# finmath/finmath-lib-cuda-extensions

Measured on AMD Instinct MI355X. Metric: Monte-Carlo path-ops/sec (fused RandomVariable stream), higher is better.
Workload: dtype f32

## Files before the change

### finmath-lib-cuda-extensions_amd/__init__.py

```python
from __future__ import annotations

import ctypes as _C

from . import _native
from ._native import FmhipError, Moments, PoolStats, ProgOp, build
from .random_variable import OP, DeviceVector, RandomVariableHip, RandomVariableHipFactory, quantiles, select_ranks_batch
from .brownian_motion import BrownianMotionHip, BrownianMotionFromMersenneRandomNumbers, TimeDiscretization, mersenne_increments
from .increments import (ExponentialLaw, GammaLaw, GammaProcess, IndependentIncrementsFromICDF, JumpProcessIncrements, NormalLaw, PoissonLaw,
                         UniformLaw, VarianceGammaProcess, host_increments, merton_increments)
from .sobol import BrownianMotionFromSobolSequence, SobolSequence, sobol_increments
from .program import Program
from .regression import MonteCarloConditionalExpectationRegression, covariance_matrix, cross_moments, solve_normal_equations
from .regression import MonteCarloConditionalExpectationLocalizedRegression, binned_cross_moments, binned_evaluate, quantile_bounds
from .regression import MonteCarloConditionalExpectationPolynomialRegression, polynomial_cross_moments, polynomial_evaluate
from .sorting import argsort, rank_scores, read_elements, sort_by_key, sorted_quantiles, spearman_matrix
from .prefix import cumulative_sums, expected_shortfall_curve, prefix_search, prefix_sums_at, prefix_sums_host, running_average
from .prefix import weighted_expected_shortfall, weighted_quantiles
from .resample import (bootstrap_resample, device_resample, effective_sample_size, multinomial_resample, resample, resample_host, stratified_resample,
                       systematic_resample)
from .selection import compress, compress_host, count_selected, device_select, expand, expand_host, gather, gather_host
from .tabulated import TabulatedFunction, table_apply, table_apply_host
from .analytic import NORMAL_CDF, NORMAL_DENSITY, NORMAL_QUANTILE, NamedFunction, function_apply, function_apply_host, normal_scores
from .analytic import bachelier_option_value, black_scholes_option_value, option_formula, option_formula_double, option_formula_host
from .analytic import (bachelier_implied_volatility, black_scholes_implied_volatility, convert_volatility, implied_volatility,
# ... 178 lines not shown
    prev = _C.c_int(0)
    _native.check(lib().fmhip_set_jit(int(mode), _C.byref(prev)))
    return prev.value


def jit_wait() -> None:
    _native.check(lib().fmhip_jit_wait())


def traffic_stats() -> tuple:
    b, l = _C.c_int64(0), _C.c_int64(0)
    _native.check(lib().fmhip_traffic_stats(_C.byref(b), _C.byref(l)))
    return b.value, l.value


def engine_stats() -> dict:
    st = _native.EngineStats()
    _native.check(lib().fmhip_engine_stats(_C.byref(st)))
    return {n: getattr(st, n) for n, _ in _native.EngineStats._fields_ if n != "size"}


def jit_stats() -> dict:
    c, f, p, s, d = _C.c_int64(0), _C.c_int64(0), _C.c_int64(0), _C.c_double(0), _C.c_int64(0)
    _native.check(lib().fmhip_jit_stats(_C.byref(c), _C.byref(f), _C.byref(p), _C.byref(s), _C.byref(d)))
    return {"compiled": c.value, "failed": f.value, "pending": p.value, "compile_seconds": s.value, "disk_cache_hits": d.value}


def graph_clone(roots, n_copies: int, leaf_from=(), leaf_to=(), scalars=None):
    import numpy as _np
    n_roots, n_map = len(roots), len(leaf_from)
    r = (_C.c_int64 * n_roots)(*[v.handle for v in roots])
    lf = (_C.c_int64 * max(1, n_map))(*[v.handle for v in leaf_from])
    lt = (_C.c_int64 * max(1, n_map * n_copies))(*[v.handle for row in leaf_to for v in row])
    sc, n_sc = None, 0
    if scalars is not None:
        a = _np.ascontiguousarray(scalars, dtype=_np.float64).reshape(n_copies, -1)
        n_sc = a.shape[1]
        sc = a.ctypes.data_as(_C.POINTER(_C.c_double))
    out = (_C.c_int64 * max(1, n_roots * n_copies))()
    _native.check(lib().fmhip_graph_clone(r, n_roots, n_copies, lf, lt, n_map, sc, n_sc, out))
    return [[DeviceVector(out[j * n_roots + k], roots[k].n) for k in range(n_roots)] for j in range(n_copies)]


def graph_scalars(roots):
    import numpy as _np
    r = (_C.c_int64 * len(roots))(*[v.handle for v in roots])
    n = _C.c_int(0)
    _native.check(lib().fmhip_graph_scalars(r, len(roots), None, 0, _C.byref(n)))
    out = _np.zeros(max(1, n.value), dtype=_np.float64)
    _native.check(lib().fmhip_graph_scalars(r, len(roots), out.ctypes.data_as(_C.POINTER(_C.c_double)), n.value, _C.byref(n)))
    return out[:n.value]


def flush() -> None:
    _native.check(lib().fmhip_flush())


def pool_stats() -> PoolStats:
    s = PoolStats()
    _native.check(lib().fmhip_pool_stats(_C.byref(s)))
    return s


def device_info():
    name = _C.create_string_buffer(256)
    cus, hbm = _C.c_int(0), _C.c_int64(0)
    _native.check(lib().fmhip_device_info(name, 256, _C.byref(cus), _C.byref(hbm)))
    return name.value.decode(), cus.value, hbm.value


def stream_ptr() -> int:
    p = _C.c_void_p(0)
    _native.check(lib().fmhip_get_stream(_C.byref(p)))
    return p.value or 0


def profile_enable(enabled: bool) -> None:
    _native.check(lib().fmhip_profile_enable(1 if enabled else 0))


def profile_read():
    ms, n = _C.c_double(0.0), _C.c_int64(0)
    _native.check(lib().fmhip_profile_read(_C.byref(ms), _C.byref(n)))
    return ms.value, n.value
```

### finmath-lib-cuda-extensions_amd/_native.py

```python
from __future__ import annotations

import ctypes as C
import os
import subprocess

_HERE = os.path.dirname(os.path.abspath(__file__))
LIB_PATH = os.path.join(_HERE, "lib", "libfmhip.so")
CSRC = os.path.join(_HERE, "csrc")

SYMBOLS = [
    "fmhip_init", "fmhip_init_devices", "fmhip_device_count", "fmhip_set_thread_engines", "fmhip_shutdown", "fmhip_is_initialized", "fmhip_abi_version", "fmhip_last_error",
    "fmhip_device_info", "fmhip_synchronize", "fmhip_get_stream",
    "fmhip_vec_create_from_double", "fmhip_vec_create_from_float", "fmhip_vec_create_filled",
    "fmhip_vec_create_uninitialized", "fmhip_vec_retain", "fmhip_vec_release", "fmhip_vec_size", "fmhip_vec_give_up_values",
    "fmhip_vec_read_double", "fmhip_vec_read_float", "fmhip_vec_device_ptr",
    "fmhip_call_v1s0", "fmhip_call_v1s1", "fmhip_call_v2s0", "fmhip_call_v2s1", "fmhip_call_v3s0",
    "fmhip_set_fusion", "fmhip_flush", "fmhip_fusion_hold", "fmhip_set_step_grouping", "fmhip_graph_clone", "fmhip_graph_scalars", "fmhip_set_math_mode",
    "fmhip_reduce_moments", "fmhip_reduce_moments_batch", "fmhip_reduce_moments_batch_device", "fmhip_reduce_moments_device",
    "fmhip_reduce_moments_batch_begin", "fmhip_reduce_moments_batch_end", "fmhip_reduce_moments_batch_devices", "fmhip_get_stream_of", "fmhip_expectation_collective",
    "fmhip_set_expectation_comm", "fmhip_expectation_world", "fmhip_expectation_combine",
    "fmhip_select_ranks_batch", "fmhip_rank_sums_batch", "fmhip_count_not_above", "fmhip_cross_moments", "fmhip_cross_moments_wide",
    "fmhip_binned_cross_moments", "fmhip_binned_cross_moments_host", "fmhip_binned_evaluate", "fmhip_binned_evaluate_host",
    "fmhip_polynomial_cross_moments", "fmhip_polynomial_evaluate", "fmhip_polynomial_cross_moments_host", "fmhip_polynomial_evaluate_host",
    "fmhip_sort_by_key", "fmhip_argsort", "fmhip_argsort_host", "fmhip_rank_scores", "fmhip_vec_read_elements",
    "fmhip_prefix_sums", "fmhip_prefix_sums_at", "fmhip_prefix_search", "fmhip_prefix_sums_host",
    "fmhip_resample", "fmhip_resample_host",
    "fmhip_compress", "fmhip_expand", "fmhip_gather", "fmhip_compress_host", "fmhip_expand_host", "fmhip_gather_host",
    "fmhip_table_build", "fmhip_table_apply", "fmhip_table_apply_host",
    "fmhip_function_apply", "fmhip_function_apply_host", "fmhip_option_formula", "fmhip_option_formula_host",
    "fmhip_implied_volatility", "fmhip_implied_volatility_host",
    "fmhip_block_moments", "fmhip_block_moments_host", "fmhip_vec_repeat",
    "fmhip_block_order_statistics", "fmhip_block_order_statistics_host", "fmhip_block_sort", "fmhip_block_sort_host",
    "fmhip_cross_order_statistics", "fmhip_cross_order_statistics_host", "fmhip_cross_select", "fmhip_cross_select_host",
    "fmhip_kernel_moments", "fmhip_kernel_moments_host",
    "fmhip_program_create", "fmhip_program_release", "fmhip_program_launch_count", "fmhip_program_shape",
    "fmhip_program_run", "fmhip_program_run_into",
    "fmhip_set_jit", "fmhip_jit_wait", "fmhip_jit_stats", "fmhip_program_tier", "fmhip_program_source",
    "fmhip_bm_generate", "fmhip_mersenne_increments", "fmhip_bm_generate_mersenne", "fmhip_bm_generate_mersenne_device", "fmhip_inverse_normal_cdf",
    "fmhip_increments_host", "fmhip_increments_generate_device",
    "fmhip_sobol_points_host", "fmhip_sobol_increments_host", "fmhip_bm_generate_sobol_device",
    "fmhip_pool_clean", "fmhip_pool_purge", "fmhip_pool_stats",
    "fmhip_profile_enable", "fmhip_profile_read", "fmhip_traffic_stats", "fmhip_engine_stats",
]

OK = 0
ERR_INVALID_HANDLE, ERR_SIZE_MISMATCH, ERR_OUT_OF_MEMORY, ERR_HIP = -1, -2, -3, -4
ERR_INVALID_ARGUMENT, ERR_NOT_INITIALIZED, ERR_UNSUPPORTED, ERR_PROGRAM_LIMIT = -5, -6, -7, -8


GATHER_FN = C.CFUNCTYPE(C.c_int, C.c_void_p, C.POINTER(C.c_double), C.c_int, C.POINTER(C.c_double))


class Moments(C.Structure):
    _fields_ = [("sum", C.c_double), ("sumsq", C.c_double), ("min", C.c_double), ("max", C.c_double)]


class ProgOp(C.Structure):
    _fields_ = [("opcode", C.c_int32), ("a", C.c_int32), ("b", C.c_int32), ("c", C.c_int32), ("scalar", C.c_double)]


class PoolStats(C.Structure):
    _fields_ = [(n, C.c_int64) for n in (
        "bytes_reserved", "bytes_in_use", "bytes_cached", "device_bytes_free", "device_bytes_total",
        "n_alloc_hits", "n_alloc_misses", "n_live_vectors", "n_kernel_launches", "n_ops_executed")]


class EngineStats(C.Structure):
    _fields_ = [(n, C.c_int64) for n in (
        "size", "kernel_launches", "specialised_launches", "interpreter_launches", "algorithmic_bytes", "algorithmic_bytes_written",
        "values_deferred", "values_deferred_now", "values_demanded", "pending_operations", "peak_bytes_reserved",
        "late_releases_while_waiting", "late_releases_at_once", "late_release_nanoseconds", "merged_launches", "merged_chains", "common_rows", "rolled_launches")]


class FmhipError(RuntimeError):
    def __init__(self, code: int, message: str):
        super().__init__(f"fmhip error {code}: {message}")
        self.code = code


def _source_hash() -> str:
    import hashlib
    h = hashlib.sha256()
    files = [os.path.join(CSRC, f) for f in sorted(os.listdir(CSRC))]
    files += [os.path.join(_HERE, "host", f) for f in sorted(os.listdir(os.path.join(_HERE, "host")))]
    files.append(os.path.join(os.path.dirname(_HERE), "include", "fmhip.h"))
    for f in files:
        if os.path.isfile(f):
            h.update(os.path.basename(f).encode())
            with open(f, "rb") as fh:
                h.update(fh.read())
    return h.hexdigest()


_HASH_PATH = LIB_PATH + ".srchash"


def build(force: bool = False) -> str:
    if force:
        subprocess.check_call(["make", "-C", CSRC, "clean"])
    subprocess.check_call(["make", "-C", CSRC, "-j4"], stdout=subprocess.DEVNULL)
    with open(_HASH_PATH, "w") as fh:
        fh.write(_source_hash())
    return LIB_PATH


def _stale() -> bool:
    if not os.path.exists(LIB_PATH):
        return True
    try:
        with open(_HASH_PATH) as fh:
            return fh.read().strip() != _source_hash()
    except OSError:
        return True


_lib = None


def lib():
    global _lib
    if _lib is not None:
        return _lib
    if _stale():
        import fcntl
        os.makedirs(os.path.dirname(LIB_PATH), exist_ok=True)
        with open(LIB_PATH + ".lock", "w") as lock:
            fcntl.flock(lock, fcntl.LOCK_EX)
            try:
                if _stale():
                    try:
                        build()
                    except Exception as e:
                        if not os.path.exists(LIB_PATH):
                            raise
                        import warnings
                        warnings.warn(f"libfmhip.so is older than its sources and rebuilding it failed ({e}); loading the existing library", RuntimeWarning)
            finally:
                fcntl.flock(lock, fcntl.LOCK_UN)
    if not os.path.exists(LIB_PATH):
        raise ImportError(f"{LIB_PATH} is missing — the HIP extension is required (no CPU fallback exists)")
    L = C.CDLL(LIB_PATH)
    vec, i64, i32, dbl, vp = C.c_int64, C.c_int64, C.c_int, C.c_double, C.c_void_p
    pv = C.POINTER(C.c_int64)
    sig = {
        "fmhip_init": [i32], "fmhip_init_devices": [C.POINTER(C.c_int), i32], "fmhip_device_count": [C.POINTER(C.c_int)], "fmhip_set_thread_engines": [i32, C.POINTER(C.c_int)], "fmhip_shutdown": [], "fmhip_is_initialized": [], "fmhip_abi_version": [],
        "fmhip_device_info": [C.c_char_p, i32, C.POINTER(i32), C.POINTER(i64)],
        "fmhip_synchronize": [], "fmhip_get_stream": [C.POINTER(vp)],
        "fmhip_vec_create_from_double": [C.POINTER(dbl), i64, pv],
        "fmhip_vec_create_from_float": [C.POINTER(C.c_float), i64, pv],
        "fmhip_vec_create_filled": [i64, dbl, pv], "fmhip_vec_create_uninitialized": [i64, pv],
        "fmhip_vec_retain": [vec], "fmhip_vec_release": [vec], "fmhip_vec_size": [vec, C.POINTER(i64)],
        "fmhip_vec_read_double": [vec, C.POINTER(dbl), i64], "fmhip_vec_read_float": [vec, C.POINTER(C.c_float), i64],
        "fmhip_vec_device_ptr": [vec, C.POINTER(vp)],
        "fmhip_call_v1s0": [i32, vec, pv], "fmhip_call_v1s1": [i32, vec, dbl, pv],
        "fmhip_call_v2s0": [i32, vec, vec, pv], "fmhip_call_v2s1": [i32, vec, vec, dbl, pv],
        "fmhip_call_v3s0": [i32, vec, vec, vec, pv],
        "fmhip_set_fusion": [i32, C.POINTER(i32)], "fmhip_flush": [], "fmhip_fusion_hold": [i32, C.POINTER(i32)], "fmhip_set_step_grouping": [i32, C.POINTER(i32)], "fmhip_set_math_mode": [i32, C.POINTER(i32)],
        "fmhip_graph_clone": [pv, i32, i32, pv, pv, i32, C.POINTER(dbl), i32, pv], "fmhip_graph_scalars": [pv, i32, C.POINTER(dbl), i32, C.POINTER(i32)],
        "fmhip_reduce_moments": [vec, dbl, C.POINTER(Moments)], "fmhip_reduce_moments_batch": [pv, i32, C.POINTER(dbl), C.POINTER(Moments)], "fmhip_reduce_moments_batch_device": [pv, i32, C.POINTER(dbl), vp], "fmhip_reduce_moments_device": [vec, dbl, vp],
        "fmhip_reduce_moments_batch_devices": [pv, i32, C.POINTER(dbl), C.POINTER(vp), i32], "fmhip_get_stream_of": [i32, C.POINTER(vp)], "fmhip_expectation_collective": [C.POINTER(i32), C.c_char_p, i32],
        "fmhip_reduce_moments_batch_begin": [pv, i32, C.POINTER(dbl), pv], "fmhip_vec_give_up_values": [pv, i32], "fmhip_reduce_moments_batch_end": [i64, C.POINTER(Moments), i32],
        "fmhip_select_ranks_batch": [pv, i32, C.POINTER(i64), i32, C.POINTER(dbl)], "fmhip_rank_sums_batch": [pv, i32, i64, i64, C.POINTER(dbl)], "fmhip_count_not_above": [vec, C.POINTER(dbl), i32, C.POINTER(i64)],
        "fmhip_cross_moments": [pv, i32, pv, i32, C.POINTER(dbl)],
        "fmhip_cross_moments_wide": [pv, i32, pv, i32, C.POINTER(dbl)],
        "fmhip_binned_cross_moments": [vec, C.POINTER(dbl), i32, pv, i32, pv, i32, C.POINTER(i64), C.POINTER(dbl)],
        "fmhip_binned_cross_moments_host": [vp, i64, C.POINTER(dbl), i32, C.POINTER(vp), i32, C.POINTER(vp), i32, C.POINTER(i64), C.POINTER(dbl)],
        "fmhip_binned_evaluate": [vec, C.POINTER(dbl), i32, pv, i32, C.POINTER(dbl), pv],
        "fmhip_binned_evaluate_host": [vp, i64, C.POINTER(dbl), i32, C.POINTER(vp), i32, C.POINTER(dbl), vp],
        "fmhip_polynomial_cross_moments": [pv, i32, C.POINTER(C.c_uint8), i32, pv, i32, pv, i32, C.POINTER(dbl)],
        "fmhip_polynomial_evaluate": [pv, i32, C.POINTER(C.c_uint8), i32, pv, i32, C.POINTER(dbl), pv],
        "fmhip_polynomial_cross_moments_host": [C.POINTER(vp), i64, i32, C.POINTER(C.c_uint8), i32, C.POINTER(vp), i32, C.POINTER(vp), i32, C.POINTER(dbl)],
        "fmhip_polynomial_evaluate_host": [C.POINTER(vp), i64, i32, C.POINTER(C.c_uint8), i32, C.POINTER(vp), i32, C.POINTER(dbl), vp],
        "fmhip_sort_by_key": [vec, pv, i32, pv, pv], "fmhip_argsort": [vec, C.POINTER(i64)], "fmhip_argsort_host": [vp, i64, C.POINTER(i64)],
        "fmhip_rank_scores": [vec, pv], "fmhip_vec_read_elements": [vec, C.POINTER(i64), i32, C.POINTER(dbl)],
        "fmhip_prefix_sums": [vec, i32, pv, C.POINTER(dbl)], "fmhip_prefix_sums_at": [vec, C.POINTER(i64), i32, C.POINTER(dbl)],
        "fmhip_prefix_search": [vec, C.POINTER(dbl), i32, i32, C.POINTER(i64), C.POINTER(dbl), C.POINTER(dbl)],
        "fmhip_prefix_sums_host": [vp, i64, C.POINTER(dbl)],
        "fmhip_resample": [vec, i32, i64, dbl, vec, pv, i32, pv, pv, C.POINTER(dbl)],
        "fmhip_resample_host": [vp, i64, i32, i64, dbl, vp, C.POINTER(vp), i32, C.POINTER(vp), C.POINTER(i64), C.POINTER(dbl)],
        "fmhip_compress": [vec, pv, i32, pv, pv, C.POINTER(i64)], "fmhip_expand": [vec, pv, i32, dbl, pv], "fmhip_gather": [vec, pv, i32, pv],
        "fmhip_compress_host": [vp, i64, C.POINTER(vp), i32, C.POINTER(vp), C.POINTER(i64), C.POINTER(i64)],
        "fmhip_expand_host": [vp, i64, C.POINTER(vp), i32, i64, dbl, C.POINTER(vp)],
        "fmhip_gather_host": [vp, i64, C.POINTER(vp), i32, i64, C.POINTER(vp)],
        "fmhip_table_build": [C.POINTER(dbl), C.POINTER(dbl), i32, i32, i32, i32, C.POINTER(dbl)],
        "fmhip_table_apply": [vec, C.POINTER(dbl), i32, C.POINTER(dbl), i32, pv],
        "fmhip_table_apply_host": [vp, i64, C.POINTER(dbl), i32, C.POINTER(dbl), i32, C.POINTER(vp)],
        "fmhip_function_apply": [vec, C.POINTER(i32), i32, pv], "fmhip_function_apply_host": [vp, i64, C.POINTER(i32), i32, C.POINTER(vp)],
        "fmhip_option_formula": [i32, vec, dbl, vec, dbl, vec, dbl, dbl, dbl, i32, pv],
        "fmhip_option_formula_host": [i32, vp, dbl, vp, dbl, vp, dbl, i64, dbl, dbl, i32, C.POINTER(vp)],
        "fmhip_implied_volatility": [i32, vec, dbl, vec, dbl, vec, dbl, dbl, dbl, i32, pv],
        "fmhip_implied_volatility_host": [i32, vp, dbl, vp, dbl, vp, dbl, i64, dbl, dbl, i32, C.POINTER(vp)],
        "fmhip_block_moments": [pv, i32, i64, C.c_uint32, pv], "fmhip_block_moments_host": [vp, i64, i64, C.c_uint32, vp],
        "fmhip_vec_repeat": [vec, i64, i64, pv],
        "fmhip_block_order_statistics": [pv, i32, i64, C.POINTER(i64), i32, C.POINTER(i64), C.POINTER(i64), i32, pv],
        "fmhip_block_order_statistics_host": [vp, i64, i64, C.POINTER(i64), i32, C.POINTER(i64), C.POINTER(i64), i32, vp],
        "fmhip_block_sort": [vec, i64, pv], "fmhip_block_sort_host": [vp, i64, i64, vp],
        "fmhip_cross_order_statistics": [pv, i32, C.POINTER(C.c_int32), i32, i32, pv],
        "fmhip_cross_order_statistics_host": [C.POINTER(vp), i32, i64, C.POINTER(C.c_int32), i32, i32, C.POINTER(vp)],
        "fmhip_cross_select": [vec, pv, i32, pv], "fmhip_cross_select_host": [vp, C.POINTER(vp), i32, i64, vp],
        "fmhip_kernel_moments": [vec, C.POINTER(dbl), C.POINTER(dbl), i32, i32, i32, pv, i32, C.POINTER(dbl)],
        "fmhip_kernel_moments_host": [vp, i64, C.POINTER(dbl), C.POINTER(dbl), i32, i32, i32, C.POINTER(vp), i32, C.POINTER(dbl)],
        "fmhip_program_create": [C.POINTER(ProgOp), i32, i32, C.POINTER(C.c_int32), i32, C.POINTER(C.c_int32), i32, pv],
        "fmhip_program_release": [i64], "fmhip_program_launch_count": [i64, C.POINTER(i32)],
        "fmhip_program_shape": [i64, C.POINTER(i32), C.POINTER(i32), C.POINTER(i32)],
        "fmhip_set_expectation_comm": [i32, i32, GATHER_FN, vp], "fmhip_expectation_world": [C.POINTER(i32), C.POINTER(i32)],
        "fmhip_expectation_combine": [C.POINTER(Moments), i32, i32, C.POINTER(Moments)],
        "fmhip_program_run": [i64, i32, pv, pv, C.POINTER(dbl), C.POINTER(Moments), vp],
        "fmhip_program_run_into": [i64, i32, pv, pv, C.POINTER(dbl), C.POINTER(Moments), vp],
        "fmhip_bm_generate": [i64, i32, i32, i64, i64, C.POINTER(dbl), pv],
        "fmhip_mersenne_increments": [C.c_int32, i32, i32, i64, C.POINTER(dbl), C.POINTER(dbl)],
        "fmhip_bm_generate_mersenne": [C.c_int32, i32, i32, i64, C.POINTER(dbl), pv],
# ... 31 lines not shown
```

### finmath-lib-cuda-extensions_amd/csrc/abi.cpp

```cpp
#include "runtime.hpp"
#include "sharded.hpp"
#include "order_stats.hpp"
#include <cmath>

#include <chrono>
#include <cstdlib>
#include <algorithm>
#include <cstring>
#include <functional>
#include <string>
#include <thread>
#include <vector>

namespace fm { void mersenne_increments(int32_t, int, int, int64_t, const double*, double*); double inverse_normal_cdf(double); }

using fm::Engine;
using fm::Error;

static thread_local std::string g_last_error;
namespace fm { void set_last_error(const std::string& message) { g_last_error = message; } }
namespace front = fm::front;
#define FRONT(call) do { if (fm::front_active()) return front::call; } while (0)

namespace te {
// ... 404 lines not shown
    return guarded([&] {
        Engine& e = Engine::get();
        e.require_init();
        if (previous) *previous = e.fusion ? 1 : 0;
        if (e.fusion && !enabled) e.flush_all();
        e.fusion = enabled != 0;
    });
}
int fmhip_fusion_hold(int hold, int* previous) {
    FRONT(set_int(1, hold, previous));
    return guarded([&] {
        Engine& e = Engine::get();
        e.require_init();
        if (previous) *previous = e.fusion_hold;
        e.fusion_hold = hold == 2 ? 2 : (hold != 0 ? 1 : 0);
    });
}
int fmhip_set_step_grouping(int steps, int* previous) {
    FRONT(set_int(2, steps, previous));
    TE_ALL(mine, fmhip_set_step_grouping(steps, mine ? previous : nullptr));
    return guarded([&] {
        Engine& e = Engine::get();
        e.require_init();
        if (steps < 0) throw Error(FMHIP_ERR_INVALID_ARGUMENT, "negative number of time steps");
        if (previous) *previous = e.group_steps;
        e.group_steps = steps;
    });
}
int fmhip_graph_clone(const fmhip_vec* roots, int n_roots, int n_copies, const fmhip_vec* leaf_from, const fmhip_vec* leaf_to, int n_map,
                      const double* scalars, int n_scalars, fmhip_vec* out) {
    FRONT(graph_clone(roots, n_roots, n_copies, leaf_from, leaf_to, n_map, scalars, n_scalars, out));
    if (te::active()) {
        const int te_rc = te::status_of([&]() -> int {
            te::ensure();
            bool any = false;
            for (int i = 0; leaf_from && i < n_map; ++i) any |= te::foreign(leaf_from[i]);
            for (int i = 0; leaf_to && i < n_map * n_copies; ++i) any |= te::foreign(leaf_to[i]);
            if (!any) return te::NOT_MINE_TO_HANDLE;
            te::Localized from(leaf_from, n_map), to(leaf_to, n_map * n_copies);
            te::Inside nested;
            return fmhip_graph_clone(roots, n_roots, n_copies, from.local.data(), to.local.data(), n_map, scalars, n_scalars, out);
        });
        if (te_rc != te::NOT_MINE_TO_HANDLE) return te_rc;
    }
    return guarded([&] { Engine::get().graph_clone(roots, n_roots, n_copies, leaf_from, leaf_to, n_map, scalars, n_scalars, out); });
}
int fmhip_graph_scalars(const fmhip_vec* roots, int n_roots, double* scalars_out, int capacity, int* n_scalars) {
    FRONT(graph_scalars(roots, n_roots, scalars_out, capacity, n_scalars));
    return guarded([&] {
        if (!n_scalars) throw Error(FMHIP_ERR_INVALID_ARGUMENT, "null count pointer");
        *n_scalars = Engine::get().graph_scalars(roots, n_roots, scalars_out, capacity);
    });
}
int fmhip_set_math_mode(int mode, int* previous) {
    FRONT(set_int(3, mode, previous));
    TE_ALL(mine, fmhip_set_math_mode(mode, mine ? previous : nullptr));
    return guarded([&] {
        Engine& e = Engine::get();
        e.require_init();
        if (mode != FMHIP_MATH_EXACT && mode != FMHIP_MATH_FAST) throw Error(FMHIP_ERR_INVALID_ARGUMENT, "unknown math mode");
        if (previous) *previous = e.math_mode;
        if (e.math_mode != mode) e.flush_all();
        e.math_mode = mode;
    });
}
int fmhip_flush(void) { FRONT(flush()); return guarded([&] { Engine::get().flush_all(); Engine::get().end_step_group(); }); }

static void combine_moments(const fmhip_moments* gathered, int world, int count, fmhip_moments* out) {
    for (int k = 0; k < count; ++k) {
        fmhip_moments m = gathered[k];
        for (int r = 1; r < world; ++r) {
            const fmhip_moments& g = gathered[(size_t)r * count + k];
            m.sum += g.sum; m.sumsq += g.sumsq;
            m.min = (m.min != m.min || g.min != g.min) ? std::nan("") : (g.min < m.min || (g.min == m.min && std::signbit(g.min))) ? g.min : m.min;
            m.max = (m.max != m.max || g.max != g.max) ? std::nan("") : (g.max > m.max || (g.max == m.max && !std::signbit(g.max))) ? g.max : m.max;
        }
        out[k] = m;
    }
}
static void exchange_moments(Engine& e, fmhip_moments* inout, int count) {
    if (e.comm_world <= 1 || !e.comm_gather) return;
    std::vector<fmhip_moments> all((size_t)e.comm_world * count);
    const int st = e.comm_gather(e.comm_context, reinterpret_cast<const double*>(inout), count * 4, reinterpret_cast<double*>(all.data()));
    if (st != 0) throw Error(FMHIP_ERR_HIP, "the expectation communicator's gather failed with status " + std::to_string(st));
    combine_moments(all.data(), e.comm_world, count, inout);
}
int fmhip_set_expectation_comm(int world, int rank, fmhip_gather_fn gather, void* context) {
    if (fm::front_active()) {
        if (world > 1) return front::unsupported("fmhip_set_expectation_comm");
        if (world < 1 || rank != 0) { g_last_error = "bad communicator: world " + std::to_string(world) + ", rank " + std::to_string(rank); return FMHIP_ERR_INVALID_ARGUMENT; }
        return FMHIP_OK;
    }
    return guarded([&] {
        Engine& e = Engine::get();
        if (world < 1 || rank < 0 || rank >= world) throw Error(FMHIP_ERR_INVALID_ARGUMENT, "bad communicator: world " + std::to_string(world) + ", rank " + std::to_string(rank));
        if (world > 1 && !gather) throw Error(FMHIP_ERR_INVALID_ARGUMENT, "a communicator of more than one rank needs a gather function");
        e.comm_world = gather ? world : 1; e.comm_rank = gather ? rank : 0; e.comm_gather = gather; e.comm_context = context;
    });
}
int fmhip_expectation_world(int* world, int* rank) {
    if (fm::front_active()) { if (world) *world = 1; if (rank) *rank = 0; return FMHIP_OK; }
    return guarded([&] { Engine& e = Engine::get(); if (world) *world = e.comm_world; if (rank) *rank = e.comm_rank; });
}
int fmhip_expectation_combine(const fmhip_moments* gathered, int world, int count, fmhip_moments* out) {
    return guarded([&] {
        need(gathered, "gathered"); need(out, "out");
// ... 754 lines not shown
```

### finmath-lib-cuda-extensions_amd/csrc/runtime.cpp

```cpp
#include "runtime.hpp"
#include "kernels.h"

#include <algorithm>
#include <cfloat>
#include <cmath>
#include <cstdio>
#include <cstdlib>
#include <cstring>
#include <array>
#include <functional>
#include <map>
#include <sstream>
#include <thread>
#include <chrono>
#include <unordered_set>
#if defined(__x86_64__)
#include <immintrin.h>
#endif

namespace fm {
static std::atomic<uint64_t> g_te_malloc_ns{ 0 }, g_te_malloc_calls{ 0 }, g_te_init_ns{ 0 };

void EngineMutex::lock_slow(uint64_t me) {
    for (unsigned spins = 0;; ++spins) {
// ... 117 lines not shown
        if (!all_free(sl)) { kept.push_back(sl); continue; }
        std::unordered_set<void*>& fs = free_set[sl.cap];
        for (size_t i = 0; i < sl.blocks; ++i) fs.erase((char*)sl.base + i * sl.cap);
        cached -= (int64_t)(sl.blocks * sl.cap);
        free_set[sl.parent_cap].insert(sl.base);
        cached += (int64_t)sl.parent_cap;
    }
    slabs_.swap(kept);
    kept.clear();
    size_t given_back = 0;
    for (size_t k = slabs_.size(); k-- > 0;) {
        const Slab& sl = slabs_[k];
        if (sl.parent_cap || given_back >= need || !all_free(sl)) { kept.push_back(sl); continue; }
        std::unordered_set<void*>& fs = free_set[sl.cap];
        for (size_t i = 0; i < sl.blocks; ++i) fs.erase((char*)sl.base + i * sl.cap);
        (void)hipFree(sl.base);
        reserved -= (int64_t)(sl.blocks * sl.cap); cached -= (int64_t)(sl.blocks * sl.cap);
        given_back += sl.blocks * sl.cap;
    }
    std::reverse(kept.begin(), kept.end());
    slabs_.swap(kept);
    free_.clear();
    for (auto& kv : free_set) if (!kv.second.empty()) free_[kv.first].assign(kv.second.begin(), kv.second.end());
    for (auto it = slab_blocks_.begin(); it != slab_blocks_.end();) {
        bool any = false;
        for (const Slab& sl : slabs_) any |= sl.cap == it->first && !sl.parent_cap;
        it = any ? std::next(it) : slab_blocks_.erase(it);
    }
}


static thread_local Engine* tls_engine = nullptr;
Engine& Engine::get() {
    if (tls_engine) { if (!tls_engine->retired.load(std::memory_order_acquire)) return *tls_engine; tls_engine = nullptr; }
    static Engine* e = new Engine();
    return *e;
}
Engine* Engine::create() { return new Engine(); }
void Engine::bind_thread(Engine* e) { tls_engine = e; }
bool Engine::thread_is_bound() { if (tls_engine && tls_engine->retired.load(std::memory_order_acquire)) tls_engine = nullptr; return tls_engine != nullptr; }

void Engine::require_init() const {
    if (!initialized_) throw Error(FMHIP_ERR_NOT_INITIALIZED, "fmhip_init has not been called");
    static thread_local int bound_device = -1;
    if (bound_device != device_) { hip_check(hipSetDevice(device_), "hipSetDevice"); bound_device = device_; }
}

void fusion_max_weight_override(int v);
HostProfile g_host_profile;
void HostProfile::report() const {
    static const char* names[N_SLOTS] = { "call (record one method)", "release", "flush_all (total)", "  build_dag", "  run_dags (total)", "    launch (total)",
                                          "      kernel launch API", "      row table upload", "reduce / reduce_batch (total)",
                                          "  flush: roots + components", "  build_big (walk, schedule, sign)", "  run_big_group (total)",
                                          "graph_clone (total)" };
    std::fprintf(stderr, "[fmhip host profile]\n");
    for (int i = 0; i < N_SLOTS; ++i)
        std::fprintf(stderr, "  %-32s %10lld calls %9.3f s %9.2f us/call\n", names[i], count[i], seconds[i], count[i] ? seconds[i] / count[i] * 1e6 : 0.0);
}

void Engine::init(int device_index) {
    const auto ti0 = std::chrono::steady_clock::now();
    struct Ti { std::chrono::steady_clock::time_point t0; ~Ti() { g_te_init_ns += (uint64_t)std::chrono::duration_cast<std::chrono::nanoseconds>(std::chrono::steady_clock::now() - t0).count(); } } ti{ ti0 };
    if (device_index < 0) {
        const char* e = std::getenv("FMHIP_DEVICE_INDEX");
        if (!e) e = std::getenv("LOCAL_RANK");
        device_index = e ? std::atoi(e) : 0;
    }
    int count = 0;
    hip_check(hipGetDeviceCount(&count), "hipGetDeviceCount");
    if (count <= 0) throw Error(FMHIP_ERR_HIP, "no HIP device visible");
    if (device_index >= count) device_index = device_index % count;
    if (initialized_) {
        if (device_index != device_) throw Error(FMHIP_ERR_INVALID_ARGUMENT, "already initialised on another device");
        return;
    }
    hip_check(hipSetDevice(device_index), "hipSetDevice");
    hip_check(hipStreamCreateWithFlags(&stream_, hipStreamNonBlocking), "hipStreamCreate");
    ring_cap_ = size_t(32) << 20;
    if (const char* e = std::getenv("FMHIP_RING_BYTES")) {
        const long long v = std::atoll(e);
        if (v >= 4096) ring_cap_ = ((size_t)v + 255) & ~size_t(255);
    }
    hip_check(hipHostMalloc(&ring_host_, ring_cap_, hipHostMallocDefault), "hipHostMalloc(ring)");
    hip_check(hipMalloc(&ring_dev_, ring_cap_ + 256), "hipMalloc(ring)");
    hip_check(hipMalloc(&dump_dev_, FM_DUMP_BYTES), "hipMalloc(dump)");
    hip_check(hipHostMalloc((void**)&result_slots_, (size_t)RESULT_SLOTS * 128, hipHostMallocDefault), "hipHostMalloc(result slots)");
    ARENA_BYTES = size_t(16) << 20;
    if (const char* e = std::getenv("FMHIP_ARENA_BYTES")) { const long long v = std::atoll(e); if (v >= 1024) ARENA_BYTES = ((size_t)v + 31) & ~size_t(31); }
    hip_check(hipHostMalloc((void**)&moments_arena_, ARENA_BYTES, hipHostMallocDefault), "hipHostMalloc(moments arena)");
    arena_off_ = 0; arena_outstanding_.clear();
    free_slots_.clear();
    for (int i = RESULT_SLOTS; i-- > 0;) free_slots_.push_back(i);
    { const char* e = std::getenv("FMHIP_UNIT_WORKGROUPS"); unit_workgroups_ = e ? std::atoll(e) : 512; }
    hip_check(hipMalloc((void**)&counters_dev_, FM_COUNTER_PLANES * FM_COUNTER_PLANE * sizeof(uint32_t)), "hipMalloc(counters)");
    hip_check(hipMemsetAsync(counters_dev_, 0, FM_COUNTER_PLANES * FM_COUNTER_PLANE * sizeof(uint32_t), stream_), "hipMemset(counters)");
    hip_check(hipStreamSynchronize(stream_), "init sync");
    hip_check(preload_kernels(), "loading the device code");
    ring_off_ = 0;
    device_ = device_index;
    if (const char* e = std::getenv("FMHIP_JIT")) {
        const std::string v(e);
        if (v == "off" || v == "0") jit_mode = FMHIP_JIT_OFF;
        else if (v == "sync" || v == "2") jit_mode = FMHIP_JIT_SYNC;
        else if (v == "auto" || v == "1") jit_mode = FMHIP_JIT_AUTO;
    }
    if (!jit_shared_) jit_.start(device_index);
    { static std::once_flag once; std::call_once(once, [] { g_host_profile.on = std::getenv("FMHIP_HOST_PROFILE") != nullptr; }); }
// ... 736 lines not shown
            throw;
        }
        return id;
    }
    return nd->id;
}

void Engine::step_boundary(const Node* inc) {
    if (group_last_by_bm_.size() > 64) group_last_by_bm_.clear();
    auto known = group_last_by_bm_.find(inc->bm_id);
    const int32_t last_of_this = known == group_last_by_bm_.end() ? -1 : known->second;
    if (inc->bm_step == last_of_this) { group_bm_id_ = inc->bm_id; group_last_step_ = inc->bm_step; return; }
    const bool restart = inc->bm_step == 0 || inc->bm_step < last_of_this;
    const bool same_time_index = !restart && inc->bm_id != group_bm_id_ && inc->bm_step == group_last_step_;
    group_last_by_bm_[inc->bm_id] = inc->bm_step;
    group_bm_id_ = inc->bm_id; group_last_step_ = inc->bm_step;
    if (same_time_index) return;
    ops_since_boundary_ = 0;
    if (restart) group_steps_pending_ = 0;
    if (group_steps_pending_ == 0) group_hold_ = true;
    if (++group_steps_pending_ > group_steps) { flush_all(); group_steps_pending_ = 1; }
    if (inc->bm_step == inc->bm_steps - 1) { group_steps_pending_ = 0; group_last_step_ = -1; group_bm_id_ = 0; group_hold_ = false; group_last_by_bm_.erase(inc->bm_id); }
}


void Engine::collect_pending(const fmhip_vec* roots, int n_roots, std::vector<Node*>& graph) {
    if (n_roots <= 0 || !roots) throw Error(FMHIP_ERR_INVALID_ARGUMENT, "no roots");
    if (!replicas_.empty())
        for (int r = 0; r < n_roots; ++r) { Node* root = node(roots[r]); if (!root->buf && root->rep_copy) if (ReplicaGroup* g = replica_of(root)) expand_replicas(g); }
    const uint64_t ep = ++epoch_;
    std::vector<Node*> stack;
    for (int r = 0; r < n_roots; ++r) {
        Node* root = node(roots[r]);
        if (root->buf || root->mark == ep) continue;
        root->mark = ep; stack.push_back(root);
        while (!stack.empty()) {
            Node* nd = stack.back(); stack.pop_back();
            graph.push_back(nd);
            for (int k = 0; k < nd->n_in; ++k) { Node* c = nd->in[k]; if (!c->buf && c->mark != ep) { c->mark = ep; stack.push_back(c); } }
        }
    }
    std::sort(graph.begin(), graph.end(), [](const Node* a, const Node* b) { return a->id < b->id; });
}

int Engine::graph_scalars(const fmhip_vec* roots, int n_roots, double* out, int capacity) {
    require_init();
    std::vector<Node*> graph;
    collect_pending(roots, n_roots, graph);
    int count = 0;
    for (Node* nd : graph) if (op_info(nd->opcode).scalar) { if (out && count < capacity) out[count] = nd->scalar; ++count; }
    return count;
}

template <class RootNode, class IdOf, class ScalarOf, class LeafTo>
static void clone_nodes_impl(std::vector<Node*>& graph, uint64_t ep_graph, uint64_t ep_leaf, int n_copies, RootNode root_node, IdOf id_of, ScalarOf scalar_of, LeafTo leaf_to,
                             std::vector<Node*>& node_pool, std::vector<std::vector<Node*>>& copies, const std::function<void(Node*)>& pend_insert)
{
    copies.assign((size_t)n_copies, std::vector<Node*>(graph.size(), nullptr));
    for (int j = 0; j < n_copies; ++j) {
        std::vector<Node*>& copy = copies[(size_t)j];
        for (size_t i = 0; i < graph.size(); ++i) {
            const Node* src = graph[i];
            Node* nd = root_node(j, i);
            const bool fresh = nd == nullptr;
            if (fresh) {
                if (!node_pool.empty()) { nd = node_pool.back(); node_pool.pop_back(); *nd = Node(); } else nd = new Node();
                nd->id = id_of(j, i); nd->n = src->n;
            }
            nd->opcode = src->opcode; nd->n_in = src->n_in; nd->weight = src->weight;
            nd->scalar = scalar_of(j, i, src);
            for (int k = 0; k < src->n_in; ++k) {
                Node* c = src->in[k];
                Node* m = c->mark == ep_graph ? copy[(size_t)c->tmp_id] : (c->mark == ep_leaf ? leaf_to(j, c->tmp_id) : c);
                nd->in[k] = m; m->refs_int++;
            }
            if (fresh) pend_insert(nd);
            copy[i] = nd;
        }
    }
}

static const bool REPLICAS = knob_on("FMHIP_REPLICAS");

void Engine::graph_clone(const fmhip_vec* roots, int n_roots, int n_copies, const fmhip_vec* leaf_from, const fmhip_vec* leaf_to, int n_map,
                         const double* scalars, int n_scalars, fmhip_vec* out) {
    HostTimer timer(HostProfile::CLONE);
    require_init();
    if (n_copies < 0 || n_map < 0 || !out || (n_map > 0 && (!leaf_from || !leaf_to))) throw Error(FMHIP_ERR_INVALID_ARGUMENT, "bad graph replication request");
    std::vector<Node*> graph;
    collect_pending(roots, n_roots, graph);
    const uint64_t ep_graph = ++epoch_;
    int count_scalars = 0;
    for (size_t i = 0; i < graph.size(); ++i) { graph[i]->mark = ep_graph; graph[i]->tmp_id = (int)i; count_scalars += op_info(graph[i]->opcode).scalar ? 1 : 0; }
    if (scalars && n_scalars != count_scalars)
        throw Error(FMHIP_ERR_INVALID_ARGUMENT, "the graph has " + std::to_string(count_scalars) + " scalar operands, the caller supplied " + std::to_string(n_scalars));
    const uint64_t ep_leaf = ++epoch_;
    std::vector<Node*> from((size_t)n_map);
    for (int i = 0; i < n_map; ++i) {
        Node* l = node(leaf_from[i]);
        touch(l);
        if (l->mark == ep_graph) throw Error(FMHIP_ERR_INVALID_ARGUMENT, "a substituted operand lies inside the graph to be replicated");
        l->mark = ep_leaf; l->tmp_id = i;
        from[(size_t)i] = l;
    }
    std::vector<Node*> root_nodes((size_t)n_roots);
    for (int r = 0; r < n_roots; ++r) { root_nodes[(size_t)r] = node(roots[r]); touch(root_nodes[(size_t)r]); }
// ... 1141 lines not shown
```

### finmath-lib-cuda-extensions_amd/csrc/runtime.hpp

```cpp
#pragma once
#include <hip/hip_runtime_api.h>
#include <array>
#include <atomic>
#include <chrono>
#include <cstdint>
#include <cstdlib>
#include <memory>
#include <mutex>
#include <stdexcept>
#include <string>
#include <unordered_map>
#include <unordered_set>
#include <vector>

#include "../../include/fmhip.h"
#include "fm_program.h"
#include "jit.hpp"

namespace fm {

struct Error : std::runtime_error {
    int code;
    Error(int c, const std::string& m) : std::runtime_error(m), code(c) {}
};
// ... 186 lines not shown
    std::vector<ForeignDone> take_foreign_done();
    void release_exported(fmhip_vec h, hipEvent_t done);
    static void bind_thread(Engine* e);
    static bool thread_is_bound();
    EngineMutex mu;
    static size_t late_eager() { static const size_t v = [] { const char* e = std::getenv("FMHIP_LATE_EAGER"); return e ? (size_t)std::atoll(e) : (size_t(1) << 17); }(); return v; }
    static size_t late_portion() { static const size_t v = [] { const char* e = std::getenv("FMHIP_LATE_PORTION"); return e ? (size_t)std::atoll(e) : (size_t)48; }(); return v; }
    void note_driver() { driver_seq_.store(driver_seq_.load(std::memory_order_relaxed) + 1, std::memory_order_relaxed); }
    uint64_t driver_seq() const { return driver_seq_.load(std::memory_order_relaxed); }
    void release_later(const fmhip_vec* hs, size_t count) {
        std::lock_guard<std::mutex> lock(late_mu_);
        late_.insert(late_.end(), hs, hs + count);
        late_count_.store(late_.size() - late_pos_, std::memory_order_release);
    }
    bool has_late() const { return late_count_.load(std::memory_order_acquire) != 0; }
    size_t late_count() const { return late_count_.load(std::memory_order_relaxed); }
    void drain_late(size_t at_most = ~size_t(0));
    std::atomic<int> waits_in_flight{ 0 };

    void init(int device_index);
    void shutdown();
    bool initialized() const { return initialized_; }
    int device_index() const { return device_; }
    void require_init() const;
    void synchronize();
    hipStream_t stream() const { return stream_; }
    void device_info(char* name, int len, int* cus, int64_t* hbm);

    Node* node(fmhip_vec h);
    fmhip_vec create_from_host(const void* src, bool is_double, int64_t n);
    fmhip_vec create_filled(int64_t n, float v);
    fmhip_vec create_uninitialized(int64_t n);
    void retain(fmhip_vec h);
    void release(fmhip_vec h);
    void read(fmhip_vec h, void* dst, bool as_double, int64_t n);
    void* device_ptr(fmhip_vec h);

    fmhip_vec call(int opcode, int n_in, const fmhip_vec* in, double scalar, bool has_scalar);
    bool fusion = false;
    int fusion_hold = 0;
    int math_mode = FMHIP_MATH_EXACT;
    int comm_world = 1, comm_rank = 0;
    fmhip_gather_fn comm_gather = nullptr;
    void* comm_context = nullptr;
    int group_steps = 4;
    int64_t unit_workgroups_ = 512;
    bool unit_launch(int64_t n, int64_t batch) const;
    void end_step_group() { group_hold_ = false; group_steps_pending_ = 0; }
    void flush_all();
    void materialize(const std::vector<Node*>& targets);
    void graph_clone(const fmhip_vec* roots, int n_roots, int n_copies, const fmhip_vec* leaf_from, const fmhip_vec* leaf_to, int n_map,
                     const double* scalars, int n_scalars, fmhip_vec* out);
    int graph_scalars(const fmhip_vec* roots, int n_roots, double* out, int capacity);

    struct RedLaunch { void* partials = nullptr; size_t partials_cap = 0; void* results = nullptr; size_t results_cap = 0; void* dev_moments = nullptr;
                       bool on_host = false; volatile uint64_t* poll_flag = nullptr; uint64_t done_value = 0; int slot = -1;
                       bool pending = false; int batch = 0, n_red = 0; fmhip_moments* host = nullptr; };
    void reduce(fmhip_vec h, double shift, fmhip_moments* host_out, void* dev_out, RedLaunch* hand_over = nullptr);
    static bool red_poll(const RedLaunch& red);
    void red_complete(RedLaunch& red, bool arrived);
    void reduce_batch(const fmhip_vec* hs, int count, const double* shifts, fmhip_moments* host_out, void* dev_out);
    struct MomentsTicket { void* host = nullptr; size_t cap = 0; hipEvent_t event = nullptr; int count = 0;
                           std::vector<volatile uint64_t*> slots; std::vector<fmhip_moments> ready; };
    int64_t reduce_batch_begin(const fmhip_vec* hs, int count, const double* shifts);
    int64_t reduce_batch_begin_from_launches(const fmhip_vec* hs, int count);
    void reduce_batch_device(const fmhip_vec* hs, int count, const double* shifts, void* dev_out);
    void reduce_batch_device_from_launches(const fmhip_vec* hs, int count, void* dev_out);
    void give_up_values(const fmhip_vec* hs, int count);
    MomentsTicket ticket_take(int64_t id);
    void ticket_retire(MomentsTicket& t);

    int64_t pass_size(const fmhip_vec* hs, int count, const char* what);
    int64_t os_size(const fmhip_vec* hs, int count);
    void os_hist_pass(const fmhip_vec* hs, int count, int S, const uint32_t* slots, uint32_t shift, uint64_t* hist_out);
    void os_sum_pass(const fmhip_vec* hs, int count, const uint32_t* keys, double* sums_out);
    void os_count_pass(fmhip_vec h, const double* ascending_bounds, int m, uint64_t* counts_out);

    void xmom_pass(const fmhip_vec* x, int n_x, const fmhip_vec* y, int n_y, double* sums_out);
    void xmom_wide_pass(const fmhip_vec* x, int n_x, const fmhip_vec* y, int n_y, double* sums_out);
    void xmom_poly_pass(const fmhip_vec* states, int n_states, const uint8_t* exponents, int n_terms, const fmhip_vec* extra_x, int n_extra, const fmhip_vec* y, int n_y, double* sums_out);
    void poly_eval(const fmhip_vec* states, int n_states, const uint8_t* exponents, int n_terms, const fmhip_vec* extra_x, int n_extra, const double* coefficients, fmhip_vec* out);

    void binned_xmom_pass(fmhip_vec key, const double* bounds, int n_bins, const fmhip_vec* x, int n_x, const fmhip_vec* y, int n_y, int64_t* counts_out, double* sums_out);
    void binned_eval(fmhip_vec key, const double* bounds, int n_bins, const fmhip_vec* x, int n_x, const double* coefficients, fmhip_vec* out);

    void sort_by_key(fmhip_vec key, const fmhip_vec* values, int n_values, fmhip_vec* sorted_key_out, fmhip_vec* sorted_values_out);
    void argsort(fmhip_vec key, int64_t* permutation_out);
    void rank_scores(fmhip_vec key, fmhip_vec* out);
    void read_elements(fmhip_vec v, const int64_t* positions, int count, double* out);

    void prefix_sums(fmhip_vec v, int mode, fmhip_vec* out, double* total_out);
    void prefix_sums_at(fmhip_vec v, const int64_t* positions, int count, double* sums_out);
    void prefix_search(fmhip_vec v, const double* thresholds, int count, int relative, int64_t* positions_out, double* sums_out, double* total_out);

    void resample(fmhip_vec weights, int scheme, int64_t m, double offset, fmhip_vec uniforms, const fmhip_vec* values, int n_values, fmhip_vec* values_out,
                  fmhip_vec* ancestors_out, double* total_out);

    void compress(fmhip_vec mask, const fmhip_vec* values, int n_values, fmhip_vec* values_out, fmhip_vec* positions_out, int64_t* count_out);
    void expand(fmhip_vec mask, const fmhip_vec* values, int n_values, double fill, fmhip_vec* values_out);
    void gather(fmhip_vec index, const fmhip_vec* values, int n_values, fmhip_vec* values_out);

    void table_apply(fmhip_vec x, const double* knots, int count, const double* coefficients, int n_tables, fmhip_vec* out);

    void function_apply(fmhip_vec x, const int* kinds, int n_functions, fmhip_vec* out);
    void option_formula(int model, fmhip_vec forward, double forward_scalar, fmhip_vec volatility, double volatility_scalar, fmhip_vec payoff_unit,
                        double payoff_unit_scalar, double maturity, double strike, int outputs, fmhip_vec* out);
// ... 296 lines not shown
    const SmallMatch* match_small(const Dag& d);
    int merge_shape_index(const std::string& desc);
    std::vector<std::string> merge_shapes_;
    std::vector<RolledBody> merge_shape_bodies_;
    std::unordered_map<std::string, SmallMatch> small_match_;
    std::unordered_map<std::string, std::shared_ptr<JitSlot>> merged_kernels_;
    int64_t n_merged_launches_ = 0, n_merged_chains_ = 0;
    std::unordered_map<uint32_t, ReplicaGroup*> replicas_;
    uint32_t next_replica_id_ = 1;
    uint32_t next_bm_id_ = 1, group_bm_id_ = 0;
    int32_t  group_last_step_ = -1;
    std::unordered_map<uint32_t, int32_t> group_last_by_bm_;
    int      group_steps_pending_ = 0;
    bool     group_hold_ = false;
    void step_boundary(const Node* increment);
    ReplicaGroup* replica_of(const Node* nd) const { if (!nd->rep_id) return nullptr; auto it = replicas_.find(nd->rep_id); return it == replicas_.end() ? nullptr : it->second; }
    void expand_replicas(ReplicaGroup* g);
    void expand_replicas_below(const std::vector<Node*>& targets);
    void replica_roots_done(ReplicaGroup* g, const std::vector<int>& roots);
    void destroy_replica_group(ReplicaGroup* g);
    void replicas_after_failure(const std::vector<std::pair<ReplicaGroup*, std::vector<int>>>& done);
    struct ReplicaView;
    std::unordered_map<uint64_t, BigPlan> plan_cache_;
    bool build_dag(const std::vector<Node*>& roots, Dag& dag);
    bool run_dags_plain(std::vector<Dag>& dags, const Dag* proto);
    bool run_dags(std::vector<Dag>& dags, const double* reduce_shift = nullptr, fmhip_moments* host_moments = nullptr, void* dev_moments = nullptr, const Dag* proto = nullptr);
    template <class K, class T> struct OrderedGroups {
        std::unordered_map<K, size_t> index; std::vector<std::vector<T>> lists;
        std::vector<T>& operator[](const K& key) { auto it = index.find(key); if (it == index.end()) { it = index.emplace(key, lists.size()).first; lists.emplace_back(); } return lists[it->second]; }
    };
    struct ReplicaLaunch;
    struct BigGroups;
    bool pending_roots(std::vector<Node*>& roots);
    Node* any_live_pending();
    void pending_components(const std::vector<Node*>& roots, OrderedGroups<int, Node*>& comps);
    bool small_groups(OrderedGroups<int, Node*>& comps, OrderedGroups<std::string, Dag>& groups, std::vector<Node*>& leftovers);
    void run_small_group(std::vector<Dag>& g, std::vector<SmallGroup>& waiting, std::vector<Node*>& leftovers);
    void run_small(SmallGroup& sg, std::vector<Node*>* leftovers);
    void run_parked(std::vector<SmallGroup>& waiting);
    bool big_groups(OrderedGroups<int, Node*>& comps, const std::vector<Node*>& leftovers, BigGroups& big);
    void run_big_groups(BigGroups& big, std::vector<SmallGroup>& waiting);
    bool expand_unless_whole(uint32_t rep_id, bool uniform, const std::vector<Node*>& nodes, const std::vector<char>* escapes, const std::vector<Node*>& roots);
    template <class D> void members_with_copies(std::vector<D>& originals, std::vector<D>& members, ReplicaLaunch& launch);
    std::vector<int> replicated_roots(Dag& d, ReplicaGroup* g);
    std::vector<int> replicated_roots(BigDag& b, ReplicaGroup* g);
    Dag replica_member(const Dag& d, ReplicaGroup* g, int copy);
    BigDag replica_member(const BigDag& b, ReplicaGroup* g, int copy);
    ReplicaGroup* clean_replica_group(uint32_t rep_id, bool uniform) const { if (!rep_id || !uniform) return nullptr; auto it = replicas_.find(rep_id); return it == replicas_.end() ? nullptr : it->second; }
};

void hip_check(hipError_t e, const char* what);

struct HostProfile {
    enum Slot { CALL, RELEASE, FLUSH, BUILD_DAG, RUN_DAGS, LAUNCH, LAUNCH_API, ROW_UPLOAD, REDUCE, FLUSH_COMPONENTS, BUILD_BIG, RUN_BIG, CLONE, N_SLOTS };
    bool on = false;
    double seconds[N_SLOTS] = { 0 };
    long long count[N_SLOTS] = { 0 };
    void report() const;
};
extern HostProfile g_host_profile;
struct HostTimer {
    HostProfile::Slot slot; bool on; std::chrono::steady_clock::time_point t0;
    explicit HostTimer(HostProfile::Slot s) : slot(s), on(g_host_profile.on) { if (on) t0 = std::chrono::steady_clock::now(); }
    ~HostTimer() { if (on) { g_host_profile.seconds[slot] += std::chrono::duration<double>(std::chrono::steady_clock::now() - t0).count(); g_host_profile.count[slot]++; } }
};

void xmom_check_counts(const fmhip_vec* x, int n_x, const fmhip_vec* y, int n_y, const double* sums_out);
void xmom_wide_check_counts(const fmhip_vec* x, int n_x, const fmhip_vec* y, int n_y, const double* sums_out);
void mt_bm_check(int n_steps, int n_factors, int64_t n_paths, int64_t path_offset, const double* dt, const fmhip_vec* out);
void mt_increments_check_only(int n_steps, int n_factors, int64_t n_paths, int64_t path_offset, const int32_t* kinds, const double* a, const double* b, const fmhip_vec* out);
void increments_host(int32_t seed, int n_steps, int n_factors, int64_t n_paths, const int32_t* kinds, const double* a, const double* b, double* host_out);
void sobol_check(int randomize, int construction, int n_steps, int n_factors, int64_t n_paths, int64_t path_offset, const double* dt, const fmhip_vec* out);
void sobol_increments_host(int32_t seed, int randomize, int construction, int n_steps, int n_factors, int64_t n_paths, int64_t path_offset, const double* dt, double* host_out);
void sobol_points_host(int n_dims, int64_t first_index, int64_t count, int32_t seed, int randomize, double* u_out);
void sort_check_by_key(fmhip_vec key, const fmhip_vec* values, int n_values, const fmhip_vec* sorted_key_out, const fmhip_vec* sorted_values_out);
void sort_check_read_elements(fmhip_vec v, const int64_t* positions, int count, const double* out);
void sort_argsort_host_checked(const float* key, int64_t n, int64_t* permutation_out);
void prefix_check_sums(fmhip_vec v, int mode, const fmhip_vec* out);
void prefix_check_queries(fmhip_vec v, const void* queries, int count, const void* sums_out, const char* what);
void prefix_sums_host_checked(const float* v, int64_t n, double* prefix_out);
void resample_check(fmhip_vec weights, int scheme, int64_t m, double offset, fmhip_vec uniforms, const fmhip_vec* values, int n_values, const fmhip_vec* values_out,
                    const fmhip_vec* ancestors_out);
void resample_check_sizes(int64_t n, int64_t m, int64_t n_uniforms, bool want_ancestors);
void resample_host_checked(const float* weights, int64_t n, int scheme, int64_t m, double offset, const float* uniforms, const float* const* values, int n_values,
                           float* const* values_out, int64_t* ancestors_out, double* total_out);
void select_check_compress(fmhip_vec mask, const fmhip_vec* values, int n_values, const fmhip_vec* values_out, const fmhip_vec* positions_out, const int64_t* count_out);
void select_check_expand(fmhip_vec mask, const fmhip_vec* values, int n_values, const fmhip_vec* values_out);
void select_check_gather(fmhip_vec index, const fmhip_vec* values, int n_values, const fmhip_vec* values_out);
void select_check_mask_size(const char* what, int64_t n, bool want_positions);
void compress_host_checked(const float* mask, int64_t n, const float* const* values, int n_values, float* const* values_out, int64_t* positions_out, int64_t* count_out);
void expand_host_checked(const float* mask, int64_t n, const float* const* values, int n_values, int64_t n_value_elements, double fill, float* const* values_out);
void gather_host_checked(const float* index, int64_t m, const float* const* values, int n_values, int64_t n, float* const* values_out);
void table_check_apply(fmhip_vec x, const double* knots, int count, const double* coefficients, int n_tables, const fmhip_vec* out);
void table_build_checked(const double* knots, const double* values, int count, int interpolation, int extrapolation, int derivative, double* coefficients_out);
void table_apply_host_checked(const float* x, int64_t n, const double* knots, int count, const double* coefficients, int n_tables, float* const* out);
void analytic_check_function(fmhip_vec x, const int* kinds, int n_functions, const fmhip_vec* out);
void analytic_check_formula(int model, fmhip_vec forward, fmhip_vec volatility, fmhip_vec payoff_unit, double maturity, double strike, int outputs, const fmhip_vec* out);
void function_apply_host_checked(const float* x, int64_t n, const int* kinds, int n_functions, float* const* out);
void option_formula_host_checked(int model, const float* forward, double forward_scalar, const float* volatility, double volatility_scalar, const float* payoff_unit,
                                 double payoff_unit_scalar, int64_t n, double maturity, double strike, int outputs, float* const* out);
void implied_check(int model, fmhip_vec price, fmhip_vec forward, fmhip_vec payoff_unit, double maturity, double strike, int outputs, const fmhip_vec* out);
void implied_volatility_host_checked(int model, const float* price, double price_scalar, const float* forward, double forward_scalar, const float* payoff_unit,
                                     double payoff_unit_scalar, int64_t n, double maturity, double strike, int outputs, float* const* out);
void nested_check_moments(const fmhip_vec* vs, int n_vs, int64_t block, uint32_t mask, const fmhip_vec* outs);
void nested_check_repeat(fmhip_vec v, int64_t each, int64_t times, const fmhip_vec* out);
void block_moments_host_checked(const float* v, int64_t n, int64_t block, uint32_t mask, float* outs);
void block_order_check_statistics(const fmhip_vec* vs, int n_vs, int64_t block, const int64_t* ranks, int n_ranks, const int64_t* range_from, const int64_t* range_to,
// ... 22 lines not shown
```

### finmath-lib-cuda-extensions_amd/csrc/sharded.cpp

```cpp
#include "sharded.hpp"
#include "runtime.hpp"
#include "kernels.h"
#include "order_stats.hpp"

#include <dlfcn.h>
#include <rccl/rccl.h>

#include <atomic>
#include <chrono>
#include <cmath>
#include <condition_variable>
#include <cstring>
#include <deque>
#include <functional>
#include <memory>
#include <mutex>
#include <string>
#include <thread>
#include <unordered_map>
#include <vector>

namespace fm {

void set_last_error(const std::string& message);
// ... 416 lines not shown
        Cmd& x = s.slot();
        x.kind = Cmd::CALL; x.has_scalar = has_scalar; x.last = false; x.target = -1; x.opcode = opcode; x.n_in = n_in; x.scalar = scalar;
        x.a0 = a[0]; x.a1 = a[1]; x.a2 = a[2]; x.id = id;
        s.pushed();
        *out = id;
    });
}

int set_int(int what, int value, int* previous) {
    return fronted([&](Shards& s) {
        int* mirror = what == 0 ? &s.fusion : what == 1 ? &s.hold : what == 2 ? &s.group_steps : what == 3 ? &s.math_mode : &s.jit_mode;
        if (what == 2 && value < 0) throw Error(FMHIP_ERR_INVALID_ARGUMENT, "negative number of time steps");
        if (what == 3 && value != FMHIP_MATH_EXACT && value != FMHIP_MATH_FAST) throw Error(FMHIP_ERR_INVALID_ARGUMENT, "unknown math mode");
        if (what == 4 && value != FMHIP_JIT_OFF && value != FMHIP_JIT_AUTO && value != FMHIP_JIT_SYNC) throw Error(FMHIP_ERR_INVALID_ARGUMENT, "unknown JIT mode");
        if (previous) *previous = *mirror;
        *mirror = what == 0 ? (value != 0) : what == 1 ? (value == 2 ? 2 : (value != 0 ? 1 : 0)) : value;
        s.post([=](Worker& w) {
            w.ok(what == 0 ? fmhip_set_fusion(value, nullptr) : what == 1 ? fmhip_fusion_hold(value, nullptr) : what == 2 ? fmhip_set_step_grouping(value, nullptr)
                 : what == 3 ? fmhip_set_math_mode(value, nullptr) : fmhip_set_jit(value, nullptr));
        });
    });
}

int flush() { return fronted([&](Shards& s) { s.post([](Worker& w) { w.ok(fmhip_flush()); }); s.check(); }); }

int graph_clone(const fmhip_vec* roots, int n_roots, int n_copies, const fmhip_vec* leaf_from, const fmhip_vec* leaf_to, int n_map, const double* scalars, int n_scalars, fmhip_vec* out) {
    return fronted([&](Shards& s) {
        if (n_roots <= 0 || !roots) throw Error(FMHIP_ERR_INVALID_ARGUMENT, "no roots");
        if (n_copies < 0 || n_map < 0 || !out || (n_map > 0 && (!leaf_from || !leaf_to))) throw Error(FMHIP_ERR_INVALID_ARGUMENT, "bad graph replication request");
        std::vector<int64_t> root_n;
        for (int r = 0; r < n_roots; ++r) root_n.push_back(s.vec(roots[r]).n);
        for (int i = 0; i < n_map; ++i) { const int64_t n = s.vec(leaf_from[i]).n; for (int j = 0; j < n_copies; ++j) if (s.vec(leaf_to[(size_t)j * n_map + i]).n != n) throw Error(FMHIP_ERR_SIZE_MISMATCH, "a substituted operand differs in size"); }
        auto r = std::make_shared<std::vector<fmhip_vec>>(roots, roots + n_roots);
        auto lf = std::make_shared<std::vector<fmhip_vec>>(leaf_from, leaf_from + n_map);
        auto lt = std::make_shared<std::vector<fmhip_vec>>(leaf_to, leaf_to + (size_t)n_map * n_copies);
        auto sc = std::make_shared<std::vector<double>>();
        if (scalars) sc->assign(scalars, scalars + (size_t)n_scalars * n_copies);
        const bool with_scalars = scalars != nullptr;
        std::vector<fmhip_vec> ids((size_t)n_roots * n_copies);
        for (int j = 0; j < n_copies; ++j) for (int k = 0; k < n_roots; ++k) ids[(size_t)j * n_roots + k] = s.fresh(root_n[(size_t)k]);
        auto idv = std::make_shared<std::vector<fmhip_vec>>(ids);
        s.post([=](Worker& w) {
            std::vector<fmhip_vec> lr, lfrom, lto, got(idv->size(), 0);
            for (fmhip_vec h : *r) lr.push_back(w.at(h));
            for (fmhip_vec h : *lf) lfrom.push_back(w.at(h));
            for (fmhip_vec h : *lt) lto.push_back(w.at(h));
            if (w.ok(fmhip_graph_clone(lr.data(), n_roots, n_copies, lfrom.data(), lto.data(), n_map, with_scalars ? sc->data() : nullptr, n_scalars, got.data())))
                for (size_t i = 0; i < got.size(); ++i) w.bind((*idv)[i], got[i]);
        });
        std::memcpy(out, ids.data(), ids.size() * sizeof(fmhip_vec));
    });
}

int graph_scalars(const fmhip_vec* roots, int n_roots, double* scalars_out, int capacity, int* n_scalars) {
    return fronted([&](Shards& s) {
        if (!n_scalars) throw Error(FMHIP_ERR_INVALID_ARGUMENT, "null count pointer");
        if (n_roots <= 0 || !roots) throw Error(FMHIP_ERR_INVALID_ARGUMENT, "no roots");
        for (int r = 0; r < n_roots; ++r) (void)s.vec(roots[r]);
        std::vector<fmhip_vec> r(roots, roots + n_roots);
        s.post([&](Worker& w) {
            std::vector<fmhip_vec> lr; for (fmhip_vec h : r) lr.push_back(w.at(h));
            w.ok(fmhip_graph_scalars(lr.data(), n_roots, scalars_out, capacity, n_scalars));
        }, 0);
        s.wait();
    });
}

int reduce_moments_batch(const fmhip_vec* vectors, int count, const double* shifts, fmhip_moments* out) {
    return fronted([&](Shards& s) {
        need(vectors, "vectors"); need(out, "out");
        if (count <= 0) throw Error(FMHIP_ERR_INVALID_ARGUMENT, "count must be positive");
        for (int i = 0; i < count; ++i) if (s.vec(vectors[i]).n != s.vec(vectors[0]).n) throw Error(FMHIP_ERR_SIZE_MISMATCH, "batched reduction over vectors of different size");
        std::vector<std::vector<fmhip_moments>> per((size_t)s.D(), std::vector<fmhip_moments>((size_t)count));
        s.post([&](Worker& w) {
            std::vector<fmhip_vec> l; for (int i = 0; i < count; ++i) l.push_back(w.at(vectors[i]));
            w.ok(count == 1 ? fmhip_reduce_moments(l[0], shifts ? shifts[0] : 0.0, per[(size_t)w.shard].data()) : fmhip_reduce_moments_batch(l.data(), count, shifts, per[(size_t)w.shard].data()));
        });
        s.wait();
        combine(per, count, out);
    });
}

int reduce_moments_batch_begin(const fmhip_vec* vectors, int count, const double* shifts, fmhip_ticket* ticket_out) {
    return fronted([&](Shards& s) {
        need(vectors, "vectors"); need(ticket_out, "ticket_out");
        if (count <= 0) throw Error(FMHIP_ERR_INVALID_ARGUMENT, "count must be positive");
        for (int i = 0; i < count; ++i) if (s.vec(vectors[i]).n != s.vec(vectors[0]).n) throw Error(FMHIP_ERR_SIZE_MISMATCH, "batched reduction over vectors of different size");
        auto v = std::make_shared<std::vector<fmhip_vec>>(vectors, vectors + count);
        auto sh = std::make_shared<std::vector<double>>();
        if (shifts) sh->assign(shifts, shifts + count);
        const bool shifted = shifts != nullptr;
        const int64_t id = s.next_other++;
        s.tickets[id] = count;
        s.post([=](Worker& w) {
            std::vector<fmhip_vec> l; for (fmhip_vec h : *v) l.push_back(w.at(h));
            fmhip_ticket t = 0;
            if (w.ok(fmhip_reduce_moments_batch_begin(l.data(), count, shifted ? sh->data() : nullptr, &t))) w.tickets[id] = t;
        });
        *ticket_out = id;
    });
}

int reduce_moments_batch_end(fmhip_ticket ticket, fmhip_moments* out, int count) {
    return fronted([&](Shards& s) {
        need(out, "out");
        auto it = s.tickets.find(ticket);
// ... 770 lines not shown
```

### finmath-lib-cuda-extensions_amd/csrc/sharded.hpp

```cpp
#pragma once
#include <cstdint>
#include <functional>
#include "../../include/fmhip.h"

namespace fm {
bool front_active();
void shard_range(int64_t n, int shards, int shard, int64_t* offset, int64_t* count);
int os_local_hist(const fmhip_vec* v, int count, int S, const uint32_t* slots, uint32_t shift, uint64_t* hist);
int os_local_sum(const fmhip_vec* v, int count, const uint32_t* keys, double* sums);
int os_local_count(fmhip_vec v, const double* ascending, int m, uint64_t* counts);
int xmom_local(const fmhip_vec* x, int n_x, const fmhip_vec* y, int n_y, double* sums);
int xmom_wide_local(const fmhip_vec* x, int n_x, const fmhip_vec* y, int n_y, double* sums);
int xmom_poly_local(const fmhip_vec* states, int n_states, const uint8_t* exponents, int n_terms, const fmhip_vec* extra_x, int n_extra, const fmhip_vec* y, int n_y, double* sums);
int binned_xmom_local(fmhip_vec key, const double* bounds, int n_bins, const fmhip_vec* x, int n_x, const fmhip_vec* y, int n_y, int64_t* counts, double* sums);
int kernel_moments_local(fmhip_vec key, const double* points, const double* bandwidths, int n_points, int kernel, int order, const fmhip_vec* y, int n_y, double* sums);
void os_counts_from_passes(const double* bounds, int n_bounds, int64_t* counts_out, const std::function<void(const double*, int, uint64_t*)>& pass);
namespace front {
int init_devices(const int* devices, int count);
int shutdown();
int device_info(char* name_buf, int name_buf_len, int* n_compute_units, int64_t* hbm_bytes);
int device_count(int* count);
int synchronize();
int vec_create_from_host(const void* host_values, bool is_double, int64_t n, fmhip_vec* out);
int vec_create_filled(int64_t n, double value, bool initialised, fmhip_vec* out);
int vec_retain(fmhip_vec v);
int vec_release(fmhip_vec v);
int vec_size(fmhip_vec v, int64_t* n_out);
int vec_read(fmhip_vec v, void* host_out, bool as_double, int64_t n);
int call(int opcode, int n_in, const fmhip_vec* in, double scalar, bool has_scalar, fmhip_vec* out);
int set_int(int what, int value, int* previous);
int flush();
int graph_clone(const fmhip_vec* roots, int n_roots, int n_copies, const fmhip_vec* leaf_from, const fmhip_vec* leaf_to, int n_map, const double* scalars, int n_scalars, fmhip_vec* out);
int graph_scalars(const fmhip_vec* roots, int n_roots, double* scalars_out, int capacity, int* n_scalars);
int reduce_moments_batch(const fmhip_vec* vectors, int count, const double* shifts, fmhip_moments* out);
int reduce_moments_batch_begin(const fmhip_vec* vectors, int count, const double* shifts, fmhip_ticket* ticket_out);
int reduce_moments_batch_end(fmhip_ticket ticket, fmhip_moments* out, int count);
int reduce_moments_batch_devices(const fmhip_vec* vectors, int count, const double* shifts, void* const* device_out, int n_devices);
int get_stream_of(int shard, void** stream_out);
int expectation_collective(int* kind, char* why, int why_len);
int vec_give_up_values(const fmhip_vec* vectors, int count);
int select_ranks_batch(const fmhip_vec* vectors, int count, const int64_t* ranks, int n_ranks, double* values_out);
int rank_sums_batch(const fmhip_vec* vectors, int count, int64_t rank_from, int64_t rank_to, double* sums_out);
int count_not_above(fmhip_vec v, const double* bounds, int n_bounds, int64_t* counts_out);
int cross_moments(const fmhip_vec* x, int n_x, const fmhip_vec* y, int n_y, double* sums_out);
int cross_moments_wide(const fmhip_vec* x, int n_x, const fmhip_vec* y, int n_y, double* sums_out);
int binned_cross_moments(fmhip_vec key, const double* bounds, int n_bins, const fmhip_vec* x, int n_x, const fmhip_vec* y, int n_y, int64_t* counts_out, double* sums_out);
int binned_evaluate(fmhip_vec key, const double* bounds, int n_bins, const fmhip_vec* x, int n_x, const double* coefficients, fmhip_vec* out);
int sort_by_key(fmhip_vec key, const fmhip_vec* values, int n_values, fmhip_vec* sorted_key_out, fmhip_vec* sorted_values_out);
int argsort(fmhip_vec key, int64_t* permutation_out);
int rank_scores(fmhip_vec key, fmhip_vec* out);
int vec_read_elements(fmhip_vec v, const int64_t* positions, int count, double* out);
int prefix_sums(fmhip_vec v, int mode, fmhip_vec* out, double* total_out);
int prefix_sums_at(fmhip_vec v, const int64_t* positions, int count, double* sums_out);
int resample(fmhip_vec weights, int scheme, int64_t m, double offset, fmhip_vec uniforms, const fmhip_vec* values, int n_values, fmhip_vec* values_out,
             fmhip_vec* ancestors_out, double* total_out);
int compress(fmhip_vec mask, const fmhip_vec* values, int n_values, fmhip_vec* values_out, fmhip_vec* positions_out, int64_t* count_out);
int expand(fmhip_vec mask, const fmhip_vec* values, int n_values, double fill, fmhip_vec* values_out);
int gather(fmhip_vec index, const fmhip_vec* values, int n_values, fmhip_vec* values_out);
int table_apply(fmhip_vec x, const double* knots, int count, const double* coefficients, int n_tables, fmhip_vec* out);
int function_apply(fmhip_vec x, const int* kinds, int n_functions, fmhip_vec* out);
int option_formula(int model, fmhip_vec forward, double forward_scalar, fmhip_vec volatility, double volatility_scalar, fmhip_vec payoff_unit,
                   double payoff_unit_scalar, double maturity, double strike, int outputs, fmhip_vec* out);
int implied_volatility(int model, fmhip_vec price, double price_scalar, fmhip_vec forward, double forward_scalar, fmhip_vec payoff_unit,
                       double payoff_unit_scalar, double maturity, double strike, int outputs, fmhip_vec* out);
int prefix_search(fmhip_vec v, const double* thresholds, int count, int relative, int64_t* positions_out, double* sums_out, double* total_out);
int block_moments(const fmhip_vec* vs, int n_vs, int64_t block, uint32_t mask, fmhip_vec* outs);
int vec_repeat(fmhip_vec v, int64_t each, int64_t times, fmhip_vec* out);
int block_order_statistics(const fmhip_vec* vs, int n_vs, int64_t block, const int64_t* ranks, int n_ranks, const int64_t* range_from, const int64_t* range_to,
                           int n_ranges, fmhip_vec* outs);
int block_sort(fmhip_vec v, int64_t block, fmhip_vec* out);
int cross_order_statistics(const fmhip_vec* vs, int n_vs, const int* ranks, int n_ranks, int outputs, fmhip_vec* outs);
int cross_select(fmhip_vec index, const fmhip_vec* vs, int n_vs, fmhip_vec* out);
int kernel_moments(fmhip_vec key, const double* points, const double* bandwidths, int n_points, int kernel, int order, const fmhip_vec* y, int n_y, double* sums_out);
int polynomial_cross_moments(const fmhip_vec* states, int n_states, const uint8_t* exponents, int n_terms, const fmhip_vec* extra_x, int n_extra, const fmhip_vec* y, int n_y, double* sums_out);
int polynomial_evaluate(const fmhip_vec* states, int n_states, const uint8_t* exponents, int n_terms, const fmhip_vec* extra_x, int n_extra, const double* coefficients, fmhip_vec* out);
int program_create(const fmhip_prog_op* ops, int n_ops, int n_inputs, const int32_t* out_values, int n_outputs, const int32_t* reduce_values, int n_reduce, fmhip_program* out);
int program_release(fmhip_program p);
int program_shape(fmhip_program p, int* n_inputs, int* n_outputs, int* n_reduce);
int program_tier(fmhip_program p, int* tier, int* vgprs);
int program_run(fmhip_program p, int batch, const fmhip_vec* inputs, fmhip_vec* outputs, bool into, const double* reduce_shift, fmhip_moments* moments);
int jit_wait();
int jit_stats(int64_t* compiled, int64_t* failed, int64_t* pending, double* compile_seconds, int64_t* disk_cache_hits);
int bm_generate(int64_t seed, int n_steps, int n_factors, int64_t n_paths, int64_t path_offset, const double* dt, fmhip_vec* out);
int bm_generate_mersenne_device(int32_t seed, int n_steps, int n_factors, int64_t n_paths, int64_t path_offset, const double* dt, fmhip_vec* out);
int increments_generate_device(int32_t seed, int n_steps, int n_factors, int64_t n_paths, int64_t path_offset, const int32_t* kinds, const double* a, const double* b, fmhip_vec* out);
int bm_generate_sobol_device(int32_t seed, int randomize, int construction, int n_steps, int n_factors, int64_t n_paths, int64_t path_offset, const double* dt, fmhip_vec* out);
// ... 10 lines not shown
```

### finmath-lib-cuda-extensions_amd/host/hip_backend.hpp

```cpp
#pragma once
#include <cstdlib>
#include <cstring>
#include <memory>
#include "lmm.hpp"

namespace fmhost {

class BrownianMotionFromMersenneRandomNumbersHip final : public BrownianMotion {
public:
    BrownianMotionFromMersenneRandomNumbersHip(TimeDiscretization td, int numberOfFactors, int64_t numberOfPaths, int seed, int64_t pathOffset = 0)
        : td_(std::move(td)), factors_(numberOfFactors), paths_(numberOfPaths), offset_(pathOffset), seed_(seed) {}
    RV getBrownianIncrement(int timeIndex, int factor) const override {
        std::call_once(generated_, [this] { generate(); });
        return inc_.at((size_t)timeIndex * factors_ + factor);
    }
    const TimeDiscretization& getTimeDiscretization() const override { return td_; }
    int getNumberOfFactors() const override { return factors_; }
    int64_t getNumberOfPaths() const override { return paths_; }
    int getSeed() const { return seed_; }
    RV getRandomVariableForConstant(double value) const override { return RandomVariableHip::of(-std::numeric_limits<double>::infinity(), value); }
private:
    void generate() const {
        const int steps = td_.getNumberOfTimeSteps();
        std::vector<double> dt((size_t)steps);
        for (int i = 0; i < steps; ++i) dt[(size_t)i] = td_.getTimeStep(i);
        std::vector<fmhip_vec> h((size_t)steps * factors_);
        check(fmhip_bm_generate_mersenne_device(seed_, steps, factors_, paths_, offset_, dt.data(), h.data()));
        inc_.reserve(h.size());
        for (int i = 0; i < steps; ++i)
            for (int f = 0; f < factors_; ++f)
                inc_.push_back(RandomVariableHip::of(td_.getTime(i + 1), DeviceVector(h[(size_t)i * factors_ + f]), paths_));
    }
    TimeDiscretization td_;
    int factors_;
    int64_t paths_, offset_;
    int seed_;
    mutable std::vector<RV> inc_;
    mutable std::once_flag generated_;
};

inline lmm::Backend makeHipBackend(const RandomVariableFactory* factory, const BrownianMotion* brownianMotion, int chunk = 0, int stepsPerLaunch = 0, int jacobianBatch = 0) {
    lmm::Backend be;
    be.factory = factory;
    be.brownianMotion = brownianMotion;
    if (!(std::getenv("FMHIP_LMM_FLUSH") && std::getenv("FMHIP_LMM_FLUSH")[0] == '0'))
        be.flush = [] { check(fmhip_flush()); };
    if (!(std::getenv("FMHIP_LMM_HOLD") && std::getenv("FMHIP_LMM_HOLD")[0] == '0'))
        be.hold = [](bool h) { check(fmhip_fusion_hold(h ? 1 : 0, nullptr)); };
    if (chunk > 0) be.chunk = chunk;
    if (stepsPerLaunch > 0) be.stepsPerLaunch = stepsPerLaunch;
    be.jacobianBatch = jacobianBatch > 0 ? jacobianBatch : 8;
    if (!(std::getenv("FMHIP_LMM_CLONE") && std::getenv("FMHIP_LMM_CLONE")[0] == '0')) {
        auto handleOf = [](const RV& x) {
            auto p = dynamic_cast<const RandomVariableHip*>(x.get());
            if (!p || p->isDeterministic()) throw std::runtime_error("graph replication over a value that is not a device vector");
            return p->deviceVector().handle();
        };
        be.clone = [handleOf](const std::vector<RV>& roots, const std::vector<RV>& leafFrom, const std::vector<std::vector<RV>>& leafTo,
                              const std::vector<std::vector<double>>* scalars) {
            const int nRoots = (int)roots.size(), nMap = (int)leafFrom.size(), nCopies = (int)leafTo.size();
            std::vector<fmhip_vec> r, lf, lt, out((size_t)nRoots * nCopies);
            for (const RV& x : roots) r.push_back(handleOf(x));
            for (const RV& x : leafFrom) lf.push_back(handleOf(x));
            for (const auto& row : leafTo) { if ((int)row.size() != nMap) throw std::runtime_error("graph replication: ragged operand map"); for (const RV& x : row) lt.push_back(handleOf(x)); }
            std::vector<double> sc;
            int nScalars = 0;
            if (scalars) { nScalars = (int)(*scalars)[0].size(); for (const auto& row : *scalars) { if ((int)row.size() != nScalars) throw std::runtime_error("graph replication: ragged scalar lists"); sc.insert(sc.end(), row.begin(), row.end()); } }
            check(fmhip_graph_clone(r.data(), nRoots, nCopies, lf.data(), lt.data(), nMap, scalars ? sc.data() : nullptr, nScalars, out.data()));
            std::vector<std::vector<RV>> copies((size_t)nCopies);
            for (int c = 0; c < nCopies; ++c)
                for (int k = 0; k < nRoots; ++k)
                    copies[(size_t)c].push_back(RandomVariableHip::of(roots[(size_t)k]->getFiltrationTime(), DeviceVector(out[(size_t)c * nRoots + k]), roots[(size_t)k]->size()));
            return copies;
        };
        be.recordedScalars = [handleOf](const std::vector<RV>& roots) {
            std::vector<fmhip_vec> r;
            for (const RV& x : roots) r.push_back(handleOf(x));
            int n = 0;
            check(fmhip_graph_scalars(r.data(), (int)r.size(), nullptr, 0, &n));
            std::vector<double> sc((size_t)n);
            check(fmhip_graph_scalars(r.data(), (int)r.size(), sc.data(), n, &n));
            return sc;
        };
    }
    if (!(std::getenv("FMHIP_LMM_DISCARD") && std::getenv("FMHIP_LMM_DISCARD")[0] == '0'))
        be.valuesNotNeeded = [](const std::vector<RV>& v) {
            std::vector<fmhip_vec> h;
            for (const RV& x : v) { auto p = dynamic_cast<const RandomVariableHip*>(x.get()); if (p && !p->isDeterministic()) h.push_back(p->deviceVector().handle()); }
            if (!h.empty()) check(fmhip_vec_give_up_values(h.data(), (int)h.size()));
        };
    be.launches = [] { fmhip_engine_stats_t s; check(fmhip_engine_stats(&s)); return (long long)s.kernel_launches; };
    be.averages = [](const std::vector<RV>& v) { return getAverages(v); };
    if (!(std::getenv("FMHIP_LMM_ASYNC") && std::getenv("FMHIP_LMM_ASYNC")[0] == '0'))
        be.expectationsRunPending = true;
    if (!(std::getenv("FMHIP_LMM_ASYNC") && std::getenv("FMHIP_LMM_ASYNC")[0] == '0'))
        be.averagesAsync = [](const std::vector<RV>& v) -> std::function<std::vector<double>()> {
            std::vector<fmhip_vec> h;
            int64_t n = 0;
            for (const RV& x : v) {
                auto p = dynamic_cast<const RandomVariableHip*>(x.get());
                if (!p || p->isDeterministic()) { const std::vector<double> now = getAverages(v); return [now] { return now; }; }
                h.push_back(p->deviceVector().handle()); n = p->size();
            }
            const int count = (int)h.size();
            fmhip_ticket ticket = 0;
            check(fmhip_reduce_moments_batch_begin(h.data(), count, nullptr, &ticket));
            struct Owner { fmhip_ticket t = 0; int count = 0; bool ended = false;
                           Owner() = default; Owner(const Owner&) = delete; Owner& operator=(const Owner&) = delete;
                           ~Owner() { if (!ended && t) { std::vector<fmhip_moments> drop((size_t)count); (void)fmhip_reduce_moments_batch_end(t, drop.data(), count); } } };
            auto owner = std::make_shared<Owner>();
            owner->t = ticket; owner->count = count;
            return [owner, count, n] {
                std::vector<fmhip_moments> m((size_t)count);
                owner->ended = true;
                check(fmhip_reduce_moments_batch_end(owner->t, m.data(), count));
                std::vector<double> out((size_t)count);
                for (int k = 0; k < count; ++k) out[(size_t)k] = m[(size_t)k].sum / (double)n;
                return out;
            };
        };
    return be;
}

}
```

### finmath-lib-cuda-extensions_amd/host/lmm.hpp

```cpp
#pragma once
#include <algorithm>
#include <chrono>
#include <cmath>
#include <cstdio>
#include <atomic>
#include <thread>
#include <cstdlib>
#include <functional>
#include <string>
#include <vector>

#include "random_variable.hpp"

namespace fmhost { namespace lmm {


inline const std::vector<double>& atmNormalVolatilities() {
    static const std::vector<double> v = {
        0.00151, 0.00169, 0.0021, 0.00248, 0.00291, 0.00329, 0.00365, 0.004, 0.00437, 0.00466, 0.00527, 0.00571,
        0.00604, 0.00625, 0.0016, 0.00174, 0.00217, 0.00264, 0.00314, 0.00355, 0.00398, 0.00433, 0.00469,
        0.00493, 0.00569, 0.00607, 0.00627, 0.00645, 0.00182, 0.00204, 0.00238, 0.00286, 0.00339, 0.00384,
        0.00424, 0.00456, 0.00488, 0.0052, 0.0059, 0.00623, 0.0064, 0.00654, 0.00205, 0.00235, 0.00272, 0.0032,
        0.00368, 0.00406, 0.00447, 0.00484, 0.00515, 0.00544, 0.00602, 0.00629, 0.0064, 0.00646, 0.00279,
        0.00319, 0.0036, 0.00396, 0.00436, 0.00469, 0.00503, 0.0053, 0.00557, 0.00582, 0.00616, 0.00628,
        0.00638, 0.00641, 0.00379, 0.00406, 0.00439, 0.00472, 0.00504, 0.00532, 0.0056, 0.00582, 0.00602,
        0.00617, 0.0063, 0.00636, 0.00638, 0.00639, 0.00471, 0.00489, 0.00511, 0.00539, 0.00563, 0.00583, 0.006,
        0.00618, 0.0063, 0.00644, 0.00641, 0.00638, 0.00635, 0.00634, 0.00544, 0.00557, 0.00572, 0.00591,
        0.00604, 0.00617, 0.0063, 0.00641, 0.00651, 0.00661, 0.00645, 0.00634, 0.00627, 0.00624, 0.00625,
        0.00632, 0.00638, 0.00644, 0.0065, 0.00655, 0.00661, 0.00667, 0.00672, 0.00673, 0.00634, 0.00614,
        0.00599, 0.00593, 0.00664, 0.00671, 0.00675, 0.00676, 0.00676, 0.00675, 0.00676, 0.00674, 0.00672,
        0.00669, 0.00616, 0.00586, 0.00569, 0.00558, 0.00647, 0.00651, 0.00651, 0.00651, 0.00652, 0.00649,
        0.00645, 0.0064, 0.00637, 0.00631, 0.00576, 0.00534, 0.00512, 0.00495, 0.00615, 0.0062, 0.00618,
        0.00613, 0.0061, 0.00607, 0.00602, 0.00596, 0.00591, 0.00586, 0.00536, 0.00491, 0.00469, 0.0045,
        0.00578, 0.00583, 0.00579, 0.00574, 0.00567, 0.00562, 0.00556, 0.00549, 0.00545, 0.00538, 0.00493,
        0.00453, 0.00435, 0.0042, 0.00542, 0.00547, 0.00539, 0.00532, 0.00522, 0.00516, 0.0051, 0.00504, 0.005,
        0.00495, 0.00454, 0.00418, 0.00404, 0.00394 };
    return v;
}
inline const std::vector<double>& atmExpiryYears() { static const std::vector<double> v = { 1.0 / 12, 0.25, 0.5, 1, 2, 3, 4, 5, 7, 10, 15, 20, 25, 30 }; return v; }
inline const std::vector<double>& atmTenorYears()  { static const std::vector<double> v = { 1, 2, 3, 4, 5, 6, 7, 8, 9, 10, 15, 20, 25, 30 }; return v; }

struct DiscountCurve {
    std::vector<double> t{ 0.0 }, logdf{ 0.0 };
    double df(double time) const {
        if (time <= 0.0) return 1.0;
        if (time >= t.back()) return std::exp(logdf.back());
        const size_t k = (size_t)(std::upper_bound(t.begin(), t.end(), time) - t.begin());
        const double w = (time - t[k - 1]) / (t[k] - t[k - 1]);
        return std::exp(logdf[k - 1] + w * (logdf[k] - logdf[k - 1]));
    }
    double forward(double fixing, double period) const { return (df(fixing) / df(fixing + period) - 1.0) / period; }
    static DiscountCurve bootstrap() {
        const double maturities[] = { 0.5, 1, 2, 3, 4, 5, 6, 7, 8, 9, 10, 11, 12, 15, 20, 25, 30, 35, 40, 45, 50 };
        const double rates[] = { -0.00216, -0.00208, -0.00222, -0.00216, -0.0019, -0.0014, -0.00072, 0.00011, 0.00103, 0.00196, 0.00285,
                                 0.00367, 0.0044, 0.00604, 0.00733, 0.00767, 0.00773, 0.00765, 0.00752, 0.007138, 0.007 };
        DiscountCurve c;
        for (int i = 0; i < 21; ++i) {
            const double M = maturities[i], r = rates[i];
            c.t.push_back(M); c.logdf.push_back(c.logdf.back());
            auto swapValue = [&](double ld) {
                c.logdf.back() = ld;
// ... 32 lines not shown
                for (int p = 0; p <= s.numberOfPeriods; ++p) s.swapTenor.push_back(exercise + p * 0.5);
                double floating = 0.0, annuity = 0.0;
                for (int p = 0; p < s.numberOfPeriods; ++p) {
                    const double d = curve.df(s.swapTenor[p + 1]);
                    floating += curve.forward(s.swapTenor[p], 0.5) * 0.5 * d; annuity += 0.5 * d;
                }
                s.swaprate = floating / annuity; s.annuity = annuity;
                s.targetVolatility = vols[e * atmTenorYears().size() + k];
                swaptions.push_back(std::move(s));
            }
    }
    int numberOfLibors() const { return timeDiscretization.getNumberOfTimeSteps(); }
};

struct VolatilityModel {
    std::vector<double> grid{ 0.0, 1.0, 2.0, 5.0, 10.0, 20.0, 30.0, 40.0 };
    std::vector<double> parameter = std::vector<double>(64, 0.50 / 100);
    int bin(double x) const { int k = 0; while (k < 7 && grid[(size_t)k] < x - 1e-12) ++k; return k; }
    int parameterIndex(double time, double maturity) const { return bin(time) * 8 + bin(maturity - time); }
    double volatility(double time, double maturity) const { return maturity <= time + 1e-12 ? 0.0 : parameter[(size_t)parameterIndex(time, maturity)]; }
    std::vector<int> activeParameters(const Market& m) const {
        std::vector<char> used(64, 0);
        const auto& td = m.timeDiscretization;
        for (int i = 0; i < td.getNumberOfTimeSteps(); ++i)
            for (int j = i + 1; j < m.numberOfLibors(); ++j) used[(size_t)parameterIndex(td.getTime(i), td.getTime(j))] = 1;
        std::vector<int> idx;
        for (int k = 0; k < 64; ++k) if (used[(size_t)k]) idx.push_back(k);
        return idx;
    }
};


struct Simulation {
    std::vector<std::vector<RV>> libor;
    std::vector<RV> numeraire;
};

struct Backend {
    const RandomVariableFactory* factory = nullptr;
    const BrownianMotion* brownianMotion = nullptr;
    std::function<void()> flush = [] {};
    std::function<void(bool)> hold = [](bool) {};
    std::function<long long()> launches = [] { return 0LL; };
    std::function<std::vector<double>(const std::vector<RV>&)> averages = [](const std::vector<RV>& v) {
        std::vector<double> a; for (const RV& x : v) a.push_back(x->getAverage()); return a; };
    std::function<std::function<std::vector<double>()>(const std::vector<RV>&)> averagesAsync;
    bool expectationsRunPending = false;
    std::function<void(const std::vector<RV>&)> valuesNotNeeded;
    int chunk = 7;
    int stepsPerLaunch = 4;
    std::function<std::vector<std::vector<RV>>(const std::vector<RV>& roots, const std::vector<RV>& leafFrom, const std::vector<std::vector<RV>>& leafTo,
                                               const std::vector<std::vector<double>>* scalars)> clone;
    std::function<std::vector<double>(const std::vector<RV>& roots)> recordedScalars;
    int jacobianBatch = 1;
    bool keepAllStates = false;
    int threads = 1;
};

inline std::vector<Simulation> simulateMany(const Market& m, const std::vector<const VolatilityModel*>& vols, const Backend& be, int lastTimeIndex,
                                            const std::vector<char>* keep = nullptr) {
    const auto& td = m.timeDiscretization;
    const int n = m.numberOfLibors();
    const double delta = m.dt;
    const size_t K = vols.size();
    std::vector<Simulation> sims(K);
    for (Simulation& sim : sims) {
        sim.libor.resize((size_t)lastTimeIndex + 1);
        sim.numeraire.resize((size_t)lastTimeIndex + 1);
        sim.libor[0].resize((size_t)n);
        for (int j = 0; j < n; ++j) sim.libor[0][(size_t)j] = be.factory->createRandomVariable(0.0, m.curve.forward(td.getTime(j), delta));
        sim.numeraire[0] = be.factory->createRandomVariable(0.0, 1.0);
    }
    std::vector<RV> factorSum(K);
    const int S = std::max(1, be.stepsPerLaunch);
    static int cloneChecks = 0;
    for (int i0 = 0; i0 < lastTimeIndex;) {
        int i1 = std::min(i0 + S, lastTimeIndex);
        static const bool endAtKept = std::getenv("FMHIP_LMM_GROUPS_END_AT_KEPT") && std::getenv("FMHIP_LMM_GROUPS_END_AT_KEPT")[0] == '1';
        if (keep && endAtKept) for (int s2 = i0 + 1; s2 < i1; ++s2) if ((*keep)[(size_t)s2]) { i1 = s2; break; }
        const bool cloning = K > 1 && S > 1 && keep && be.clone && i0 >= 2;
        const size_t Krec = cloning ? 1 : K;
        if (S > 1) be.hold(true);
        for (int i = i0; i < i1; ++i) {
            const double t = td.getTime(i), dt = td.getTimeStep(i);
            const RV dW = be.brownianMotion->getBrownianIncrement(i, 0);
            for (size_t k = 0; k < Krec; ++k) {
                auto& cur = sims[k].libor[(size_t)i];
                auto& nxt = sims[k].libor[(size_t)i + 1];
                nxt.resize((size_t)n);
                for (int j = 0; j <= i && j < n; ++j) nxt[(size_t)j] = cur[(size_t)j];
                factorSum[k] = nullptr;
            }
            for (int j0 = i + 1; j0 < n; j0 += be.chunk) {
                const int j1 = std::min(n, j0 + be.chunk);
                for (size_t k = 0; k < Krec; ++k) {
                    auto& cur = sims[k].libor[(size_t)i];
                    auto& nxt = sims[k].libor[(size_t)i + 1];
                    for (int j = j0; j < j1; ++j) {
                        const double lambda = vols[k]->volatility(t, td.getTime(j));
                        const RV& L = cur[(size_t)j];
                        const RV transform = be.factory->createRandomVariable(lambda * delta)->discount(L, delta);
                        factorSum[k] = factorSum[k] ? factorSum[k]->add(transform) : transform;
                        const RV drift = factorSum[k]->mult(lambda);
                        nxt[(size_t)j] = L->addProduct(drift, dt)->addProduct(dW, lambda);
                    }
                }
                if (S == 1 && j1 - j0 == be.chunk) be.flush();
            }
            for (size_t k = 0; k < Krec; ++k)
                sims[k].numeraire[(size_t)i + 1] = sims[k].numeraire[(size_t)i]->accrue(sims[k].libor[(size_t)i][(size_t)i], delta);
            for (size_t k = 0; k < Krec; ++k) factorSum[k] = nullptr;
        }
        if (cloning) {
            std::vector<RV> roots, leafFrom;
            for (int j = i0 + 1; j < n; ++j) roots.push_back(sims[0].libor[(size_t)i1][(size_t)j]);
            for (int i = i0; i < i1; ++i) roots.push_back(sims[0].numeraire[(size_t)i + 1]);
            for (int s2 = i0 + 1; s2 < i1; ++s2)
                if (!keep || (*keep)[(size_t)s2]) for (int j = s2; j < n; ++j) roots.push_back(sims[0].libor[(size_t)s2][(size_t)j]);
            for (int j = i0; j < n; ++j) leafFrom.push_back(sims[0].libor[(size_t)i0][(size_t)j]);
            leafFrom.push_back(sims[0].numeraire[(size_t)i0]);
            auto scalarsOf = [&](const VolatilityModel& vol) {
                std::vector<double> sc;
                for (int i = i0; i < i1; ++i) {
                    const double t = td.getTime(i), dt = td.getTimeStep(i);
                    for (int j = i + 1; j < n; ++j) {
                        const double lambda = vol.volatility(t, td.getTime(j));
                        sc.push_back(delta); sc.push_back(1.0); sc.push_back(lambda * delta); sc.push_back(lambda); sc.push_back(dt); sc.push_back(lambda);
                    }
                    sc.push_back(delta);
                }
                return sc;
            };
            if (cloneChecks < 64 && be.recordedScalars) {
                ++cloneChecks;
                if (be.recordedScalars(roots) != scalarsOf(*vols[0])) throw std::runtime_error("lmm: the scalar list of the replicated Euler steps does not match the recording");
            }
            std::vector<std::vector<RV>> leafTo(K - 1);
            std::vector<std::vector<double>> scalars(K - 1);
            for (size_t k = 1; k < K; ++k) {
                for (int j = i0; j < n; ++j) leafTo[k - 1].push_back(sims[k].libor[(size_t)i0][(size_t)j]);
                leafTo[k - 1].push_back(sims[k].numeraire[(size_t)i0]);
                scalars[k - 1] = scalarsOf(*vols[k]);
            }
            const std::vector<std::vector<RV>> copies = be.clone(roots, leafFrom, leafTo, &scalars);
            for (size_t k = 1; k < K; ++k) {
                auto& nxt = sims[k].libor[(size_t)i1];
                nxt.resize((size_t)n);
                for (int j = 0; j <= i0 && j < n; ++j) nxt[(size_t)j] = sims[k].libor[(size_t)i0][(size_t)j];
                size_t r = 0;
                for (int j = i0 + 1; j < n; ++j) nxt[(size_t)j] = copies[k - 1][r++];
                for (int i = i0; i < i1; ++i) sims[k].numeraire[(size_t)i + 1] = copies[k - 1][r++];
                for (int s2 = i0 + 1; s2 < i1; ++s2)
                    if (!keep || (*keep)[(size_t)s2]) { auto& mid = sims[k].libor[(size_t)s2]; mid.resize((size_t)n); for (int j = s2; j < n; ++j) mid[(size_t)j] = copies[k - 1][r++]; }
            }
        }
        if (keep)
            for (int i = i0; i < i1; ++i)
                if (!(*keep)[(size_t)i])
                    for (size_t k = 0; k < K; ++k) { sims[k].libor[(size_t)i].clear(); sims[k].libor[(size_t)i].shrink_to_fit(); }
        if (S > 1) be.hold(false);
        be.flush();
        i0 = i1;
    }
    return sims;
}

inline Simulation simulate(const Market& m, const VolatilityModel& vol, const Backend& be, int lastTimeIndex) {
    return std::move(simulateMany(m, { &vol }, be, lastTimeIndex)[0]);
}

inline RV swaptionValue(const Market& m, const Simulation& sim, const Swaption& s) {
    const auto& td = m.timeDiscretization;
    const int exerciseIndex = td.getTimeIndex(s.exercise);
    RV value;
    for (int p = s.numberOfPeriods - 1; p >= 0; --p) {
        const int j = td.getTimeIndex(s.swapTenor[(size_t)p]);
        const RV& libor = sim.libor[(size_t)exerciseIndex][(size_t)j];
        const RV payoff = libor->sub(s.swaprate)->mult(s.swapPeriodLength);
        value = (value ? value->add(payoff) : payoff)->discount(libor, s.swapPeriodLength);
    }
    return value->floor(0.0)->div(sim.numeraire[(size_t)exerciseIndex]);
}
inline double bachelierAtmImpliedVolatility(double optionValue, double optionMaturity, double annuity) {
    return optionValue * std::sqrt(2.0 * 3.14159265358979323846) / (annuity * std::sqrt(optionMaturity));
}

struct Valuation { std::vector<double> modelVolatility; double seconds_simulation = 0, seconds_valuation = 0; long long launches_simulation = 0, launches_valuation = 0; };

struct PendingValuations {
    std::vector<std::function<std::vector<double>()>> expectations;
    std::vector<Valuation> out;
};

inline std::vector<Valuation> evaluateManyFinish(const Market& m, PendingValuations& p) {
    for (size_t k = 0; k < p.out.size(); ++k) {
        const std::vector<double> optionValues = p.expectations[k]();
        for (size_t q = 0; q < m.swaptions.size(); ++q)
            p.out[k].modelVolatility.push_back(bachelierAtmImpliedVolatility(optionValues[q], m.swaptions[q].exercise, m.swaptions[q].annuity));
    }
    return std::move(p.out);
}

inline PendingValuations evaluateManyBegin(const Market& m, const std::vector<const VolatilityModel*>& vols, const Backend& be) {
    using clk = std::chrono::steady_clock;
    const size_t K = vols.size();
    PendingValuations pending;
    std::vector<Valuation>& out = pending.out;
    out.resize(K);
    int lastIndex = 0;
    for (const Swaption& s : m.swaptions) lastIndex = std::max(lastIndex, m.timeDiscretization.getTimeIndex(s.exercise));
    const auto t0 = clk::now();
    const long long l0 = be.launches();
    std::vector<char> keep((size_t)lastIndex + 1, 0);
    for (const Swaption& s : m.swaptions) keep[(size_t)m.timeDiscretization.getTimeIndex(s.exercise)] = 1;
    const std::vector<Simulation> sims = simulateMany(m, vols, be, lastIndex, be.keepAllStates ? nullptr : &keep);
    const auto t1 = clk::now();
    const long long l1 = be.launches();
    std::vector<std::vector<RV>> values(K);
    if (K > 1 && be.clone) {
        be.hold(true);
        values[0].reserve(m.swaptions.size());
        for (const Swaption& s : m.swaptions) values[0].push_back(swaptionValue(m, sims[0], s));
        std::vector<RV> leafFrom;
        std::vector<std::vector<RV>> leafTo(K - 1);
        for (int e = 0; e <= lastIndex; ++e) {
            if (!keep[(size_t)e]) continue;
            for (size_t k = 0; k < K; ++k) {
                std::vector<RV>& dst = k == 0 ? leafFrom : leafTo[k - 1];
                for (int j = e; j < m.numberOfLibors(); ++j) dst.push_back(sims[k].libor[(size_t)e][(size_t)j]);
                dst.push_back(sims[k].numeraire[(size_t)e]);
            }
        }
        const std::vector<std::vector<RV>> copies = be.clone(values[0], leafFrom, leafTo, nullptr);
        for (size_t k = 1; k < K; ++k) values[k] = copies[k - 1];
        be.hold(false);
        if (!(be.averagesAsync && be.expectationsRunPending)) be.flush();
    } else
    for (size_t k = 0; k < K; ++k) {
        be.hold(true);
        values[k].reserve(m.swaptions.size());
        for (const Swaption& s : m.swaptions) values[k].push_back(swaptionValue(m, sims[k], s));
        be.hold(false);
        if (!(be.averagesAsync && be.expectationsRunPending)) be.flush();
    }
    if (be.valuesNotNeeded) for (size_t k = 0; k < K; ++k) be.valuesNotNeeded(values[k]);
    for (size_t k = 0; k < K; ++k) {
        if (be.averagesAsync) pending.expectations.push_back(be.averagesAsync(values[k]));
        else { const std::vector<double> now = be.averages(values[k]); pending.expectations.push_back([now] { return now; }); }
    }
    const auto t2 = clk::now();
    for (size_t k = 0; k < K; ++k) {
        out[k].launches_simulation = (l1 - l0) / (long long)K; out[k].launches_valuation = (be.launches() - l1) / (long long)K;
        out[k].seconds_simulation = std::chrono::duration<double>(t1 - t0).count() / (double)K;
        out[k].seconds_valuation = std::chrono::duration<double>(t2 - t1).count() / (double)K;
    }
    return pending;
}

inline std::vector<Valuation> evaluateMany(const Market& m, const std::vector<const VolatilityModel*>& vols, const Backend& be) {
    PendingValuations p = evaluateManyBegin(m, vols, be);
    return evaluateManyFinish(m, p);
}

inline Valuation evaluate(const Market& m, const VolatilityModel& vol, const Backend& be) {
    return std::move(evaluateMany(m, { &vol }, be)[0]);
}


struct CalibrationResult {
    VolatilityModel model; int iterations = 0, evaluations = 0;
    double meanDeviation = 0, rmsDeviation = 0, initialRms = 0, seconds = 0, seconds_simulation = 0, seconds_valuation = 0;
    std::vector<double> modelVolatility;
};

inline bool solveSymmetric(std::vector<double> A, std::vector<double> b, int n, std::vector<double>& x) {
    for (int c = 0; c < n; ++c) {
        int piv = c;
        for (int r = c + 1; r < n; ++r) if (std::fabs(A[(size_t)r * n + c]) > std::fabs(A[(size_t)piv * n + c])) piv = r;
        if (std::fabs(A[(size_t)piv * n + c]) < 1e-300) return false;
        if (piv != c) { for (int k = 0; k < n; ++k) std::swap(A[(size_t)c * n + k], A[(size_t)piv * n + k]); std::swap(b[(size_t)c], b[(size_t)piv]); }
        for (int r = c + 1; r < n; ++r) {
            const double f = A[(size_t)r * n + c] / A[(size_t)c * n + c];
            for (int k = c; k < n; ++k) A[(size_t)r * n + k] -= f * A[(size_t)c * n + k];
            b[(size_t)r] -= f * b[(size_t)c];
        }
    }
    x.assign((size_t)n, 0.0);
    for (int r = n - 1; r >= 0; --r) { double s = b[(size_t)r]; for (int k = r + 1; k < n; ++k) s -= A[(size_t)r * n + k] * x[(size_t)k]; x[(size_t)r] = s / A[(size_t)r * n + r]; }
    return true;
}

inline CalibrationResult calibrate(const Market& m, const Backend& be, int maxIterations = 200, double accuracy = 1e-7,
                                   double lambda = 0.1, double parameterStep = 1e-4, bool verbose = false) {
    using clk = std::chrono::steady_clock;
// ... 122 lines not shown
```

### finmath-lib-cuda-extensions_amd/host/lmm_hip_main.cpp

```cpp
#include <fstream>
#include <thread>
#include <csignal>
#include <execinfo.h>
#include <unistd.h>
#include <rccl/rccl.h>
#include "lmm_main_common.hpp"
#include "hip_backend.hpp"
using namespace fmhost;

static void ncclCheck(ncclResult_t r, const char* what) {
    if (r != ncclSuccess) throw std::runtime_error(std::string(what) + ": " + ncclGetErrorString(r));
}

static void fatalSignal(int sig) {
    void* frames[64];
    const int n = backtrace(frames, 64);
    const char msg[] = "lmm_hip: fatal signal, call stack:\n";
    (void)!write(2, msg, sizeof msg - 1);
    backtrace_symbols_fd(frames, n, 2);
    signal(sig, SIG_DFL);
    raise(sig);
}

int main(int argc, char** argv) {
    if (std::getenv("FMHIP_BACKTRACE")) { signal(SIGABRT, fatalSignal); signal(SIGSEGV, fatalSignal); signal(SIGBUS, fatalSignal); }
    const lmm::Options o = lmm::parseOptions(argc, argv);
    try {
        if (!o.devices.empty()) check(fmhip_init_devices(o.devices.data(), (int)o.devices.size()));
        else check(fmhip_init(-1));
        check(fmhip_set_fusion(1, nullptr));
        RandomVariableHipFactory factory;
        lmm::Market m;
        const int64_t pathOffset = o.pathOffset + (int64_t)o.rank * o.paths;
        BrownianMotionHip philox(m.timeDiscretization, 1, o.paths, o.seed, pathOffset);
        BrownianMotionFromMersenneRandomNumbers mersenne(m.timeDiscretization, 1, o.paths, (int)o.seed, &factory);
        if (o.brownian == "mersenne" && o.world > 1) throw std::runtime_error("--brownian mersenne is a sequential stream: not available with --world > 1 (mersenne-device is)");
        BrownianMotionFromMersenneRandomNumbersHip mersenneDevice(m.timeDiscretization, 1, o.paths, (int)o.seed, pathOffset);
        lmm::Backend be = makeHipBackend(&factory, (o.brownian == "mersenne") ? static_cast<const BrownianMotion*>(&mersenne)
                                                 : (o.brownian == "mersenne-device") ? static_cast<const BrownianMotion*>(&mersenneDevice) : &philox,
                                         o.chunk, o.stepsPerLaunch, o.jacobianBatch);

        if (o.finmathLike) {
            be.flush = [] {}; be.hold = [](bool) {}; be.clone = nullptr; be.recordedScalars = nullptr; be.averagesAsync = nullptr; be.expectationsRunPending = false;
            be.averages = [](const std::vector<RV>& v) { std::vector<double> a; for (const RV& x : v) a.push_back(x->getAverage()); return a; };
            be.jacobianBatch = 1; be.stepsPerLaunch = 1; be.chunk = 1 << 30; be.keepAllStates = true;
            if (o.threads > 1) {
                if (!o.devices.empty() || o.world > 1) throw std::runtime_error("--threads: one device, one process");
                check(fmhip_set_thread_engines(1, nullptr));
                be.threads = o.threads;
            }
        } else if (o.threads > 1) throw std::runtime_error("--threads belongs to --finmath-like (the native driver batches its Jacobian columns instead)");
        if (o.releaseLagMs > 0.0 || o.releaseLagBytes > 0) ReleaseLag::instance().start(o.releaseLagMs, (size_t)o.releaseLagBytes);
        ncclComm_t comm = nullptr;
        std::vector<std::pair<double*, hipEvent_t>> sparePinned;
        fmhip_vec sums = 0;
        long long collectives = 0;
        double collective_seconds = 0.0;
        if (o.world > 1 || !o.ncclIdFile.empty()) {
            if (o.ncclIdFile.empty()) throw std::runtime_error("--world needs --nccl-id-file");
            struct IdFile { uint64_t magic, nonce; ncclUniqueId id; } rec{};
            const uint64_t MAGIC = 0x464d4e43434c4944ull;
            if (o.rank == 0) {
                std::remove(o.ncclIdFile.c_str());
                rec.magic = MAGIC; rec.nonce = (uint64_t)o.ncclNonce;
                ncclCheck(ncclGetUniqueId(&rec.id), "ncclGetUniqueId");
                { std::ofstream f(o.ncclIdFile + ".tmp", std::ios::binary); f.write((const char*)&rec, sizeof rec); }
                std::rename((o.ncclIdFile + ".tmp").c_str(), o.ncclIdFile.c_str());
            } else {
                for (int tries = 0; ; ++tries) {
                    std::ifstream f(o.ncclIdFile, std::ios::binary);
                    if (f && f.read((char*)&rec, sizeof rec) && f.gcount() == (std::streamsize)sizeof rec && rec.magic == MAGIC && rec.nonce == (uint64_t)o.ncclNonce) break;
                    if (tries > 6000) throw std::runtime_error("timed out waiting for " + o.ncclIdFile);
                    std::this_thread::sleep_for(std::chrono::milliseconds(10));
                }
            }
            const ncclUniqueId id = rec.id;
            ncclCheck(ncclCommInitRank(&comm, o.world, id, o.rank), "ncclCommInitRank");
            if (o.rank == 0) std::remove(o.ncclIdFile.c_str());
            const int count = (int)m.swaptions.size();
            check(fmhip_vec_create_uninitialized((int64_t)count * 8 * o.world, &sums));
            void* stream = nullptr; check(fmhip_get_stream(&stream));
            const int64_t totalPaths = (int64_t)o.world * o.paths;
            const int world = o.world, rank = o.rank;
            struct Flight {
                fmhip_vec dev = 0; double* host = nullptr; hipEvent_t ev = nullptr;
                std::vector<std::pair<double*, hipEvent_t>>* spare = nullptr;
                ~Flight() { if (dev) fmhip_vec_release(dev); if (host && ev && spare) spare->push_back({ host, ev }); }
            };
            std::vector<std::pair<double*, hipEvent_t>>* const spare = &sparePinned;
            { const char* e = std::getenv("FMHIP_LMM_SHARDED_FROM_LAUNCHES"); be.expectationsRunPending = !(e && e[0] == '0'); }
            be.averagesAsync = [=, &collectives, &collective_seconds](const std::vector<RV>& v) -> std::function<std::vector<double>()> {
                std::vector<fmhip_vec> h;
                for (const RV& x : v) {
                    auto p = dynamic_cast<const RandomVariableHip*>(x.get());
                    if (!p || p->isDeterministic()) throw std::runtime_error("sharded expectation of a non-device value");
                    h.push_back(p->deviceVector().handle());
                }
                if ((int)h.size() != count) throw std::runtime_error("sharded expectation: unexpected product count");
                auto f = std::make_shared<Flight>();
                const size_t doubles = (size_t)count * 4 * (size_t)world;
                check(fmhip_vec_create_uninitialized((int64_t)doubles * 2, &f->dev));
                f->spare = spare;
                if (!spare->empty()) { f->host = spare->back().first; f->ev = spare->back().second; spare->pop_back(); }
                else if (hipHostMalloc((void**)&f->host, doubles * 8, hipHostMallocDefault) != hipSuccess || hipEventCreateWithFlags(&f->ev, hipEventDisableTiming) != hipSuccess)
                    throw std::runtime_error("pinned memory / event for a sharded expectation");
// ... 40 lines not shown
                    for (int r = 0; r < world; ++r) { double s; std::memcpy(&s, &raw[((size_t)r * count + k) * 8], 8); total += s; }
                    out[(size_t)k] = total / (double)totalPaths;
                }
                return out;
            };
        }

        if (o.mode == "evaluate" && o.warmupEvaluations > 0) {
            lmm::VolatilityModel vol;
            (void)lmm::evaluateMany(m, std::vector<const lmm::VolatilityModel*>((size_t)o.warmupEvaluations, &vol), be);
            check(fmhip_jit_wait());
        }
        fmhip_pool_stats_t s0; check(fmhip_pool_stats(&s0));
        int64_t bytes0 = 0; check(fmhip_traffic_stats(&bytes0, nullptr));
        if (o.profile) check(fmhip_profile_enable(1));
        auto extra = [&] {
            fmhip_pool_stats_t s; check(fmhip_pool_stats(&s));
            char name[128] = { 0 }; int cus = 0; int64_t hbm = 0; fmhip_device_info(name, 128, &cus, &hbm);
            int64_t jc = 0, jf = 0, jp = 0, jd = 0; double js = 0.0; fmhip_jit_stats(&jc, &jf, &jp, &js, &jd);
            int64_t bytes1 = 0, jl = 0; fmhip_traffic_stats(&bytes1, &jl);
            std::string prof;
            if (o.profile) {
                double ms = 0.0; int64_t nl = 0; fmhip_profile_read(&ms, &nl);
                char pb[256];
                std::snprintf(pb, sizeof pb, ", \"profiled_launches\": %lld, \"kernel_ms_total\": %.3f, \"achieved_GBps\": %.1f",
                              (long long)nl, ms, ms > 0 ? (double)(bytes1 - bytes0) / (ms * 1e-3) / 1e9 : 0.0);
                prof = pb;
            }
            char buf[768];
            std::snprintf(buf, sizeof buf, ", \"kernel_launches\": %lld, \"path_ops\": %.6e, \"device_bytes_reserved\": %lld, \"device\": \"%s\", "
                          "\"world\": %d, \"rank\": %d, \"total_paths\": %lld, \"rccl_collectives\": %lld, \"rccl_collective_seconds\": %.6f, "
                          "\"specialised_kernels\": %lld, \"specialisations_from_disk_cache\": %lld, \"specialisations_pending\": %lld, \"specialisation_seconds\": %.3f, "
                          "\"algorithmic_bytes\": %lld, \"specialised_launches\": %lld",
                          (long long)(s.n_kernel_launches - s0.n_kernel_launches), (double)(s.n_ops_executed - s0.n_ops_executed) * (double)o.paths,
                          (long long)s.bytes_reserved, name, o.world, o.rank, (long long)o.world * (long long)o.paths, collectives, collective_seconds,
                          (long long)jc, (long long)jd, (long long)jp, js, (long long)(bytes1 - bytes0), (long long)jl);
            std::string lag;
            if (ReleaseLag::instance().on()) {
                const ReleaseLag::Stats ls = ReleaseLag::instance().stats();
                char lb[384];
                std::snprintf(lb, sizeof lb, ", \"release_lag\": {\"collect_every_ms\": %.3f, \"collect_at_bytes\": %lld, \"handles_queued\": %lld, \"handles_released\": %lld, "
                              "\"collections\": %lld, \"collections_forced_by_out_of_memory\": %lld, \"peak_dead_handles\": %lld}",
                              o.releaseLagMs, o.releaseLagBytes, ls.queued, ls.released, ls.collections, ls.forcedCollections, ls.peakQueue);
                lag = lb;
            }
            fmhip_engine_stats_t es; check(fmhip_engine_stats(&es));
            char eb[768];
            std::snprintf(eb, sizeof eb, ", \"engine\": {\"interpreter_launches\": %lld, \"algorithmic_bytes_written\": %lld, \"values_deferred\": %lld, \"values_deferred_now\": %lld, "
                          "\"values_demanded\": %lld, \"peak_bytes_reserved\": %lld, \"late_releases_while_waiting\": %lld, \"late_releases_at_once\": %lld, \"late_release_seconds\": %.3f, "
                          "\"merged_launches\": %lld, \"merged_chains\": %lld, \"common_rows\": %lld, \"rolled_launches\": %lld}",
                          (long long)es.interpreter_launches, (long long)es.algorithmic_bytes_written, (long long)es.values_deferred, (long long)es.values_deferred_now,
                          (long long)es.values_demanded, (long long)es.peak_bytes_reserved, (long long)es.late_releases_while_waiting, (long long)es.late_releases_at_once, (double)es.late_release_nanoseconds * 1e-9,
                          (long long)es.merged_launches, (long long)es.merged_chains, (long long)es.common_rows, (long long)es.rolled_launches);
            return std::string(buf) + prof + lag + eb;
        };
        if (o.rank == 0) lmm::runAndReport(o, be, "hip", extra);
        else { lmm::Options quiet = o; quiet.verbose = false; lmm::runAndReport(quiet, be, "hip", extra); }
        if (sums) fmhip_vec_release(sums);
        ReleaseLag::instance().stop();
        be = lmm::Backend();
        for (auto& pe : sparePinned) { (void)hipHostFree(pe.first); (void)hipEventDestroy(pe.second); }
        if (comm) ncclCommDestroy(comm);
        check(fmhip_shutdown());
    } catch (const std::exception& e) { std::fprintf(stderr, "lmm_hip[rank %d]: %s\n", o.rank, e.what()); return 1; }
    return 0;
}
```

### include/fmhip.h

```cpp
#ifndef FMHIP_H
#define FMHIP_H

#include <stdint.h>
#include <stddef.h>

#ifdef __cplusplus
extern "C" {
#endif

#define FMHIP_ABI_VERSION 1

typedef int64_t fmhip_vec;
typedef int64_t fmhip_program;

typedef enum fmhip_status {
    FMHIP_OK                  =  0,
    FMHIP_ERR_INVALID_HANDLE  = -1,
    FMHIP_ERR_SIZE_MISMATCH   = -2,
    FMHIP_ERR_OUT_OF_MEMORY   = -3,
    FMHIP_ERR_HIP             = -4,
    FMHIP_ERR_INVALID_ARGUMENT= -5,
    FMHIP_ERR_NOT_INITIALIZED = -6,
    FMHIP_ERR_UNSUPPORTED     = -7,
    FMHIP_ERR_PROGRAM_LIMIT   = -8
// ... 44 lines not shown
typedef struct fmhip_pool_stats_t {
    int64_t bytes_reserved;
    int64_t bytes_in_use;
    int64_t bytes_cached;
    int64_t device_bytes_free;
    int64_t device_bytes_total;
    int64_t n_alloc_hits;
    int64_t n_alloc_misses;
    int64_t n_live_vectors;
    int64_t n_kernel_launches;
    int64_t n_ops_executed;
} fmhip_pool_stats_t;


int fmhip_init(int device_index);
int fmhip_init_devices(const int* devices, int count);
int fmhip_device_count(int* count);
int fmhip_set_thread_engines(int enabled, int* previous);
int fmhip_shutdown(void);
int fmhip_is_initialized(void);
int fmhip_abi_version(void);
const char* fmhip_last_error(void);
int fmhip_device_info(char* name_buf, int name_buf_len, int* n_compute_units, int64_t* hbm_bytes);
int fmhip_synchronize(void);
int fmhip_get_stream(void** stream_out);


int fmhip_vec_create_from_double(const double* host_values, int64_t n, fmhip_vec* out);
int fmhip_vec_create_from_float(const float* host_values, int64_t n, fmhip_vec* out);
int fmhip_vec_create_filled(int64_t n, double value, fmhip_vec* out);
int fmhip_vec_create_uninitialized(int64_t n, fmhip_vec* out);
int fmhip_vec_retain(fmhip_vec v);
int fmhip_vec_release(fmhip_vec v);
int fmhip_vec_size(fmhip_vec v, int64_t* n_out);
int fmhip_vec_read_double(fmhip_vec v, double* host_out, int64_t n);
int fmhip_vec_read_float(fmhip_vec v, float* host_out, int64_t n);
int fmhip_vec_device_ptr(fmhip_vec v, void** device_ptr_out);


int fmhip_call_v1s0(int opcode, fmhip_vec a, fmhip_vec* out);
int fmhip_call_v1s1(int opcode, fmhip_vec a, double s, fmhip_vec* out);
int fmhip_call_v2s0(int opcode, fmhip_vec a, fmhip_vec b, fmhip_vec* out);
int fmhip_call_v2s1(int opcode, fmhip_vec a, fmhip_vec b, double s, fmhip_vec* out);
int fmhip_call_v3s0(int opcode, fmhip_vec a, fmhip_vec b, fmhip_vec c, fmhip_vec* out);

int fmhip_set_fusion(int enabled, int* previous);
int fmhip_flush(void);
int fmhip_fusion_hold(int hold, int* previous);
int fmhip_set_step_grouping(int steps, int* previous);
int fmhip_graph_clone(const fmhip_vec* roots, int n_roots, int n_copies,
                      const fmhip_vec* leaf_from, const fmhip_vec* leaf_to, int n_map,
                      const double* scalars, int n_scalars, fmhip_vec* out);
int fmhip_graph_scalars(const fmhip_vec* roots, int n_roots, double* scalars_out, int capacity, int* n_scalars);

#define FMHIP_MATH_EXACT 0
#define FMHIP_MATH_FAST  1
int fmhip_set_math_mode(int mode, int* previous);


int fmhip_reduce_moments(fmhip_vec v, double shift, fmhip_moments* out);
int fmhip_reduce_moments_device(fmhip_vec v, double shift, void* device_out_4_doubles);

int fmhip_reduce_moments_batch(const fmhip_vec* vectors, int count, const double* shifts, fmhip_moments* out);
int fmhip_reduce_moments_batch_device(const fmhip_vec* vectors, int count, const double* shifts, void* device_out);
int fmhip_reduce_moments_batch_devices(const fmhip_vec* vectors, int count, const double* shifts, void* const* device_out, int n_devices);
int fmhip_get_stream_of(int shard, void** stream_out);
int fmhip_expectation_collective(int* kind, char* why, int why_len);
typedef int64_t fmhip_ticket;
int fmhip_reduce_moments_batch_begin(const fmhip_vec* vectors, int count, const double* shifts, fmhip_ticket* ticket_out);
int fmhip_reduce_moments_batch_end(fmhip_ticket ticket, fmhip_moments* out, int count);
int fmhip_vec_give_up_values(const fmhip_vec* vectors, int count);

int fmhip_select_ranks_batch(const fmhip_vec* vectors, int count, const int64_t* ranks, int n_ranks, double* values_out);
int fmhip_rank_sums_batch(const fmhip_vec* vectors, int count, int64_t rank_from, int64_t rank_to, double* sums_out);
int fmhip_count_not_above(fmhip_vec v, const double* bounds, int n_bounds, int64_t* counts_out);

int fmhip_cross_moments(const fmhip_vec* x, int n_x, const fmhip_vec* y, int n_y, double* sums_out);

int fmhip_cross_moments_wide(const fmhip_vec* x, int n_x, const fmhip_vec* y, int n_y, double* sums_out);

int fmhip_binned_cross_moments(fmhip_vec key, const double* bounds, int n_bins, const fmhip_vec* x, int n_x, const fmhip_vec* y, int n_y,
                               int64_t* counts_out, double* sums_out);
int fmhip_binned_cross_moments_host(const float* key, int64_t n, const double* bounds, int n_bins, const float* const* x, int n_x,
                                    const float* const* y, int n_y, int64_t* counts_out, double* sums_out);
int fmhip_binned_evaluate(fmhip_vec key, const double* bounds, int n_bins, const fmhip_vec* x, int n_x, const double* coefficients, fmhip_vec* out);
int fmhip_binned_evaluate_host(const float* key, int64_t n, const double* bounds, int n_bins, const float* const* x, int n_x,
                               const double* coefficients, float* out);

int fmhip_sort_by_key(fmhip_vec key, const fmhip_vec* values, int n_values, fmhip_vec* sorted_key_out, fmhip_vec* sorted_values_out);
int fmhip_argsort(fmhip_vec key, int64_t* permutation_out);
int fmhip_argsort_host(const float* key, int64_t n, int64_t* permutation_out);
int fmhip_rank_scores(fmhip_vec key, fmhip_vec* out);
int fmhip_vec_read_elements(fmhip_vec v, const int64_t* positions, int count, double* out);

#define FMHIP_PREFIX_SUM  0
#define FMHIP_PREFIX_MEAN 1
int fmhip_prefix_sums(fmhip_vec v, int mode, fmhip_vec* out, double* total_out);
int fmhip_prefix_sums_at(fmhip_vec v, const int64_t* positions, int count, double* sums_out);
int fmhip_prefix_search(fmhip_vec v, const double* thresholds, int count, int relative,
                        int64_t* positions_out, double* sums_out, double* total_out);
int fmhip_prefix_sums_host(const float* v, int64_t n, double* prefix_out);

#define FMHIP_RESAMPLE_SYSTEMATIC  0
#define FMHIP_RESAMPLE_STRATIFIED  1
#define FMHIP_RESAMPLE_MULTINOMIAL 2
int fmhip_resample(fmhip_vec weights , int scheme, int64_t m, double offset,
// ... 186 lines not shown
```

### java/net/finmath/hip/Native.java

```java
package net.finmath.hip;

final class Native {

	static {
		System.loadLibrary("fmhip_jni");
	}

	private Native() { }

	static native int init(int deviceIndex);
	static native int initDevices(int[] devices);
	static native int deviceCount(int[] count);
	static native int    setThreadEngines(int enabled, int[] previous);
	static native int shutdown();
	static native int isInitialized();
	static native int abiVersion();
	static native String lastError();
	static native int deviceInfo(String[] name, int[] computeUnits, long[] hbmBytes);
	static native int synchronize();
	static native int getStream(long[] stream);

	static native long vecCreateFromDouble(double[] values);
	static native long vecCreateFromFloat(float[] values);
	static native long vecCreateFilled(long n, double value);
	static native long vecCreateUninitialized(long n);
	static native int vecRetain(long vector);
	static native int vecRelease(long vector);
	static native int vecSize(long vector, long[] size);
	static native int vecReadDouble(long vector, double[] out);
	static native int vecReadFloat(long vector, float[] out);
	static native int vecDevicePtr(long vector, long[] devicePointer);

	static native long callV1s0(int opcode, long a);
	static native long callV1s1(int opcode, long a, double s);
	static native long callV2s0(int opcode, long a, long b);
	static native long callV2s1(int opcode, long a, long b, double s);
	static native long callV3s0(int opcode, long a, long b, long c);

	static native int setFusion(int enabled, int[] previous);
	static native int flush();
	static native int fusionHold(int hold, int[] previous);
	static native int setStepGrouping(int steps, int[] previous);
	static native int graphClone(long[] roots, int nCopies, long[] leafFrom, long[] leafTo, double[] scalarsOrNull, int nScalars, long[] out);
	static native int graphScalars(long[] roots, double[] scalarsOutOrNull, int[] count);
	static native int setMathMode(int mode, int[] previous);

	static native int reduceMoments(long vector, double shift, double[] moments4);
	static native int reduceMomentsDevice(long vector, double shift, long deviceOut4Doubles);
	static native int reduceMomentsBatch(long[] vectors, double[] shiftsOrNull, double[] moments4PerVector);
	static native int reduceMomentsBatchDevice(long[] vectors, double[] shiftsOrNull, long deviceOut);
	static native int selectRanksBatch(long[] vectors, long[] ranks, double[] valuesOut);
	static native int rankSumsBatch(long[] vectors, long rankFrom, long rankTo, double[] sumsOut);
	static native int countNotAbove(long vector, double[] bounds, long[] countsOut);
	static native int crossMoments(long[] x, long[] y, double[] sumsOut);
	static native int crossMomentsWide(long[] x, long[] y, double[] sumsOut);
	static native int binnedCrossMoments(long key, double[] bounds, long[] x, long[] y, long[] countsOut, double[] sumsOut);
	static native int binnedCrossMomentsHost(float[] key, double[] bounds, float[] xColumns, int nX, int onesMask, float[] yColumns, int nY, long[] countsOut, double[] sumsOut);
	static native int binnedEvaluate(long key, double[] bounds, long[] x, double[] coefficients, long[] out);
	static native int binnedEvaluateHost(float[] key, double[] bounds, float[] xColumns, int nX, int onesMask, double[] coefficients, float[] out);
	static native int sortByKey(long key, long[] values, long[] sortedKeyOut, long[] sortedValuesOut);
	static native int argsort(long key, long[] permutationOut);
	static native int argsortHost(float[] key, long[] permutationOut);
	static native int rankScores(long key, long[] out);
	static native int vecReadElements(long v, long[] positions, double[] out);
	static native int prefixSums(long v, int mode, long[] out, double[] totalOutOrNull);
	static native int prefixSumsAt(long v, long[] positions, double[] sumsOut);
	static native int prefixSearch(long v, double[] thresholds, boolean relative, long[] positionsOut, double[] sumsOut, double[] totalOutOrNull);
	static native int prefixSumsHost(float[] v, double[] prefixOut);
	static native int resample(long weights, int scheme, long m, double offset, long uniforms, long[] values, long[] valuesOut, long[] ancestorsOutOrNull, double[] totalOutOrNull);
	static native int resampleHost(float[] weightsOrNull, long n, int scheme, long m, double offset, float[] uniformsOrNull, float[] valueColumns, int nValues, float[] outColumns, long[] ancestorsOutOrNull, double[] totalOutOrNull);
	static native int compress(long mask, long[] valuesOrNull, long[] valuesOutOrNull, long[] positionsOutOrNull, long[] countOutOrNull);
	static native int expand(long mask, long[] values, double fill, long[] valuesOut);
	static native int gather(long index, long[] values, long[] valuesOut);
	static native int compressHost(float[] mask, float[] valueColumns, int nValues, float[] outColumns, long[] positionsOutOrNull, long[] countOutOrNull);
	static native int expandHost(float[] mask, float[] valueColumns, int nValues, long nValueElements, double fill, float[] outColumns);
	static native int gatherHost(float[] index, float[] valueColumns, int nValues, long n, float[] outColumns);
	static native int tableBuild(double[] knots, double[] values, int interpolation, int extrapolation, int derivative, double[] coefficientsOut);
	static native int tableApply(long x, double[] knots, double[] coefficients, int nTables, long[] out);
	static native int tableApplyHost(float[] x, double[] knots, double[] coefficients, int nTables, float[] outColumns);
	static native int functionApply(long x, int[] kinds, long[] out);
	static native int functionApplyHost(float[] x, int[] kinds, float[] outColumns);
	static native int optionFormula(int model, long forward, double forwardScalar, long volatility, double volatilityScalar, long payoffUnit, double payoffUnitScalar, double maturity, double strike, int outputs, long[] out);
	static native int optionFormulaHost(int model, float[] forwardOrNull, double forwardScalar, float[] volatilityOrNull, double volatilityScalar, float[] payoffUnitOrNull, double payoffUnitScalar, int n, double maturity, double strike, int outputs, float[] outColumns);
	static native int impliedVolatility(int model, long price, double priceScalar, long forward, double forwardScalar, long payoffUnit, double payoffUnitScalar, double maturity, double strike, int outputs, long[] out);
	static native int impliedVolatilityHost(int model, float[] priceOrNull, double priceScalar, float[] forwardOrNull, double forwardScalar, float[] payoffUnitOrNull, double payoffUnitScalar, int n, double maturity, double strike, int outputs, float[] outColumns);
	static native int blockMoments(long[] vs, long block, int mask, long[] outs);
	static native int blockMomentsHost(float[] v, long block, int mask, float[] outColumns);
	static native int vecRepeat(long v, long each, long times, long[] out);
	static native int blockOrderStatistics(long[] vs, long block, long[] ranks, long[] rangeFrom, long[] rangeTo, long[] outs);
	static native int blockOrderStatisticsHost(float[] v, long block, long[] ranks, long[] rangeFrom, long[] rangeTo, float[] outColumns);
	static native int blockSort(long v, long block, long[] out);
	static native int blockSortHost(float[] v, long block, float[] out);
	static native int crossOrderStatistics(long[] vs, int[] ranks, int outputs, long[] outs);
	static native int crossOrderStatisticsHost(float[] vsColumns, int nVs, int[] ranks, int outputs, float[] outColumns);
	static native int crossSelect(long index, long[] vs, long[] out);
	static native int crossSelectHost(float[] index, float[] vsColumns, int nVs, float[] out);
	static native int kernelMoments(long key, double[] points, double[] bandwidths, int kernel, int order, long[] y, double[] sumsOut);
// ... 70 lines not shown
```

### src/jni/fmhip_jni.cpp

```cpp
#include <jni.h>
#include <cstdint>
#include <string>
#include <vector>
#include "fmhip.h"

namespace {

template <typename T> struct ArrayOps;
template <> struct ArrayOps<jint>    { static jint*    get(JNIEnv* e, jarray a) { return e->GetIntArrayElements((jintArray)a, nullptr); }       static void put(JNIEnv* e, jarray a, jint* p, jint m)    { e->ReleaseIntArrayElements((jintArray)a, p, m); } };
template <> struct ArrayOps<jlong>   { static jlong*   get(JNIEnv* e, jarray a) { return e->GetLongArrayElements((jlongArray)a, nullptr); }     static void put(JNIEnv* e, jarray a, jlong* p, jint m)   { e->ReleaseLongArrayElements((jlongArray)a, p, m); } };
template <> struct ArrayOps<jdouble> { static jdouble* get(JNIEnv* e, jarray a) { return e->GetDoubleArrayElements((jdoubleArray)a, nullptr); } static void put(JNIEnv* e, jarray a, jdouble* p, jint m) { e->ReleaseDoubleArrayElements((jdoubleArray)a, p, m); } };
template <> struct ArrayOps<jfloat>  { static jfloat*  get(JNIEnv* e, jarray a) { return e->GetFloatArrayElements((jfloatArray)a, nullptr); }   static void put(JNIEnv* e, jarray a, jfloat* p, jint m)  { e->ReleaseFloatArrayElements((jfloatArray)a, p, m); } };
template <typename T>
struct Pin {
    JNIEnv* env; jarray arr; T* p; jint mode; jsize len;
    Pin(JNIEnv* e, jarray a, jint release_mode = 0) : env(e), arr(a), p(nullptr), mode(release_mode), len(a ? e->GetArrayLength(a) : 0) { if (a) p = ArrayOps<T>::get(e, a); }
    ~Pin() { if (arr && p) ArrayOps<T>::put(env, arr, p, mode); }
    jsize length() const { return len; }
};
bool program_ops(JNIEnv* env, jintArray opcode, jintArray a, jintArray b, jintArray c, jdoubleArray scalar, std::vector<fmhip_prog_op>& ops) {
    const jsize n = opcode ? env->GetArrayLength(opcode) : 0;
    ops.assign((size_t)n, fmhip_prog_op{});
    if (n == 0) return true;
    Pin<jint> po(env, opcode, JNI_ABORT), pa(env, a, JNI_ABORT), pb(env, b, JNI_ABORT), pc(env, c, JNI_ABORT);
    Pin<jdouble> ps(env, scalar, JNI_ABORT);
    if (!po.p || !pa.p || !pb.p || !pc.p || pa.length() < n || pb.length() < n || pc.length() < n || (ps.p && ps.length() < n)) return false;
    for (jsize i = 0; i < n; ++i) ops[(size_t)i] = { po.p[i], pa.p[i], pb.p[i], pc.p[i], ps.p ? ps.p[i] : 0.0 };
    return true;
}

inline void set1(JNIEnv* env, jintArray arr, jint v) { if (arr && env->GetArrayLength(arr) > 0) env->SetIntArrayRegion(arr, 0, 1, &v); }
inline void set1(JNIEnv* env, jlongArray arr, jlong v) { if (arr && env->GetArrayLength(arr) > 0) env->SetLongArrayRegion(arr, 0, 1, &v); }

}

#define FMJ(ret, name) extern "C" JNIEXPORT ret JNICALL Java_net_finmath_hip_Native_##name

FMJ(jint, init)(JNIEnv*, jclass, jint deviceIndex) { return fmhip_init(deviceIndex); }
FMJ(jint, initDevices)(JNIEnv* env, jclass, jintArray devices) {
    Pin<jint> pd(env, devices, JNI_ABORT);
    if (!pd.p) return FMHIP_ERR_INVALID_ARGUMENT;
    return fmhip_init_devices((const int*)pd.p, pd.length());
}
FMJ(jint, deviceCount)(JNIEnv* env, jclass, jintArray count) {
    if (!count || env->GetArrayLength(count) < 1) return FMHIP_ERR_INVALID_ARGUMENT;
    int c = 0;
    const int st = fmhip_device_count(&c);
    if (st == FMHIP_OK) { const jint v = c; env->SetIntArrayRegion(count, 0, 1, &v); }
    return st;
}
FMJ(jint, setThreadEngines)(JNIEnv* env, jclass, jint enabled, jintArray previous) {
    int prev = 0;
    const int st = fmhip_set_thread_engines(enabled, &prev);
// ... 22 lines not shown
}

FMJ(jlong, vecCreateFromDouble)(JNIEnv* env, jclass, jdoubleArray values) {
    Pin<jdouble> p(env, values, JNI_ABORT);
    fmhip_vec out = 0;
    return fmhip_vec_create_from_double(p.p, p.length(), &out) == FMHIP_OK ? (jlong)out : 0;
}
FMJ(jlong, vecCreateFromFloat)(JNIEnv* env, jclass, jfloatArray values) {
    Pin<jfloat> p(env, values, JNI_ABORT);
    fmhip_vec out = 0;
    return fmhip_vec_create_from_float(p.p, p.length(), &out) == FMHIP_OK ? (jlong)out : 0;
}
FMJ(jlong, vecCreateFilled)(JNIEnv*, jclass, jlong n, jdouble value) { fmhip_vec out = 0; return fmhip_vec_create_filled(n, value, &out) == FMHIP_OK ? (jlong)out : 0; }
FMJ(jlong, vecCreateUninitialized)(JNIEnv*, jclass, jlong n) { fmhip_vec out = 0; return fmhip_vec_create_uninitialized(n, &out) == FMHIP_OK ? (jlong)out : 0; }
FMJ(jint, vecRetain)(JNIEnv*, jclass, jlong v) { return fmhip_vec_retain(v); }
FMJ(jint, vecRelease)(JNIEnv*, jclass, jlong v) { return fmhip_vec_release(v); }
FMJ(jint, vecSize)(JNIEnv* env, jclass, jlong v, jlongArray size) {
    int64_t n = 0;
    const int st = fmhip_vec_size(v, &n);
    if (st == FMHIP_OK) set1(env, size, (jlong)n);
    return st;
}
FMJ(jint, vecReadDouble)(JNIEnv* env, jclass, jlong v, jdoubleArray out) { Pin<jdouble> p(env, out); return fmhip_vec_read_double(v, p.p, p.length()); }
FMJ(jint, vecReadFloat)(JNIEnv* env, jclass, jlong v, jfloatArray out) { Pin<jfloat> p(env, out); return fmhip_vec_read_float(v, p.p, p.length()); }
FMJ(jint, vecDevicePtr)(JNIEnv* env, jclass, jlong v, jlongArray devicePointer) {
    void* ptr = nullptr;
    const int st = fmhip_vec_device_ptr(v, &ptr);
    if (st == FMHIP_OK) set1(env, devicePointer, (jlong)(intptr_t)ptr);
    return st;
}

FMJ(jlong, callV1s0)(JNIEnv*, jclass, jint opcode, jlong a) { fmhip_vec out = 0; return fmhip_call_v1s0(opcode, a, &out) == FMHIP_OK ? (jlong)out : 0; }
FMJ(jlong, callV1s1)(JNIEnv*, jclass, jint opcode, jlong a, jdouble s) { fmhip_vec out = 0; return fmhip_call_v1s1(opcode, a, s, &out) == FMHIP_OK ? (jlong)out : 0; }
FMJ(jlong, callV2s0)(JNIEnv*, jclass, jint opcode, jlong a, jlong b) { fmhip_vec out = 0; return fmhip_call_v2s0(opcode, a, b, &out) == FMHIP_OK ? (jlong)out : 0; }
FMJ(jlong, callV2s1)(JNIEnv*, jclass, jint opcode, jlong a, jlong b, jdouble s) { fmhip_vec out = 0; return fmhip_call_v2s1(opcode, a, b, s, &out) == FMHIP_OK ? (jlong)out : 0; }
FMJ(jlong, callV3s0)(JNIEnv*, jclass, jint opcode, jlong a, jlong b, jlong c) { fmhip_vec out = 0; return fmhip_call_v3s0(opcode, a, b, c, &out) == FMHIP_OK ? (jlong)out : 0; }

FMJ(jint, setFusion)(JNIEnv* env, jclass, jint enabled, jintArray previous) { int prev = 0; const int st = fmhip_set_fusion(enabled, &prev); if (st == FMHIP_OK) set1(env, previous, prev); return st; }
FMJ(jint, flush)(JNIEnv*, jclass) { return fmhip_flush(); }
FMJ(jint, setStepGrouping)(JNIEnv* env, jclass, jint steps, jintArray previous) { int prev = 0; const int st = fmhip_set_step_grouping(steps, &prev); if (st == FMHIP_OK) set1(env, previous, prev); return st; }
FMJ(jint, fusionHold)(JNIEnv* env, jclass, jint hold, jintArray previous) { int prev = 0; const int st = fmhip_fusion_hold(hold, &prev); if (st == FMHIP_OK) set1(env, previous, prev); return st; }
FMJ(jint, graphClone)(JNIEnv* env, jclass, jlongArray roots, jint nCopies, jlongArray leafFrom, jlongArray leafTo, jdoubleArray scalars, jint nScalars, jlongArray out) {
    Pin<jlong> pr(env, roots, JNI_ABORT), pf(env, leafFrom, JNI_ABORT), pt(env, leafTo, JNI_ABORT), po(env, out); Pin<jdouble> ps(env, scalars, JNI_ABORT);
    if (nCopies < 0 || nScalars < 0 || !pr.p || !po.p || (int64_t)pt.length() < (int64_t)pf.length() * nCopies || (int64_t)po.length() < (int64_t)pr.length() * nCopies ||
        (ps.p && (int64_t)ps.length() < (int64_t)nScalars * nCopies)) return FMHIP_ERR_INVALID_ARGUMENT;
    return fmhip_graph_clone((const fmhip_vec*)pr.p, pr.length(), nCopies, (const fmhip_vec*)pf.p, (const fmhip_vec*)pt.p, pf.length(), ps.p, nScalars, (fmhip_vec*)po.p);
}
FMJ(jint, graphScalars)(JNIEnv* env, jclass, jlongArray roots, jdoubleArray scalarsOut, jintArray count) {
    int n = 0, st;
    { Pin<jlong> pr(env, roots, JNI_ABORT); Pin<jdouble> ps(env, scalarsOut); st = fmhip_graph_scalars((const fmhip_vec*)pr.p, pr.length(), ps.p, ps.length(), &n); }
    if (st == FMHIP_OK) set1(env, count, n);
    return st;
}
FMJ(jint, setMathMode)(JNIEnv* env, jclass, jint mode, jintArray previous) { int prev = 0; const int st = fmhip_set_math_mode(mode, &prev); if (st == FMHIP_OK) set1(env, previous, prev); return st; }

FMJ(jint, reduceMoments)(JNIEnv* env, jclass, jlong v, jdouble shift, jdoubleArray moments4) {
    fmhip_moments m;
    const int st = fmhip_reduce_moments(v, shift, &m);
    if (st == FMHIP_OK && moments4 && env->GetArrayLength(moments4) >= 4) { const jdouble d[4] = { m.sum, m.sumsq, m.min, m.max }; env->SetDoubleArrayRegion(moments4, 0, 4, d); }
    return st;
}
FMJ(jint, reduceMomentsDevice)(JNIEnv*, jclass, jlong v, jdouble shift, jlong deviceOut) { return fmhip_reduce_moments_device(v, shift, (void*)(intptr_t)deviceOut); }
FMJ(jint, reduceMomentsBatch)(JNIEnv* env, jclass, jlongArray vectors, jdoubleArray shifts, jdoubleArray moments4PerVector) {
    Pin<jlong> pv(env, vectors, JNI_ABORT); Pin<jdouble> ps(env, shifts, JNI_ABORT); Pin<jdouble> pm(env, moments4PerVector);
    static_assert(sizeof(fmhip_moments) == 4 * sizeof(double), "moments travel as 4 doubles");
    if (!pv.p || !pm.p || (int64_t)pm.length() < 4 * (int64_t)pv.length() || (ps.p && ps.length() < pv.length())) return FMHIP_ERR_INVALID_ARGUMENT;
    return fmhip_reduce_moments_batch((const fmhip_vec*)pv.p, pv.length(), ps.p, (fmhip_moments*)pm.p);
}
FMJ(jint, selectRanksBatch)(JNIEnv* env, jclass, jlongArray vectors, jlongArray ranks, jdoubleArray valuesOut) {
    Pin<jlong> pv(env, vectors, JNI_ABORT); Pin<jlong> pr(env, ranks, JNI_ABORT); Pin<jdouble> po(env, valuesOut);
    static_assert(sizeof(jlong) == sizeof(int64_t), "ranks travel as 64-bit integers");
    if (!pv.p || !pr.p || !po.p || (int64_t)po.length() < (int64_t)pv.length() * (int64_t)pr.length()) return FMHIP_ERR_INVALID_ARGUMENT;
    return fmhip_select_ranks_batch((const fmhip_vec*)pv.p, pv.length(), (const int64_t*)pr.p, pr.length(), po.p);
}
FMJ(jint, rankSumsBatch)(JNIEnv* env, jclass, jlongArray vectors, jlong rankFrom, jlong rankTo, jdoubleArray sumsOut) {
    Pin<jlong> pv(env, vectors, JNI_ABORT); Pin<jdouble> po(env, sumsOut);
    if (!pv.p || !po.p || po.length() < pv.length()) return FMHIP_ERR_INVALID_ARGUMENT;
    return fmhip_rank_sums_batch((const fmhip_vec*)pv.p, pv.length(), rankFrom, rankTo, po.p);
}
FMJ(jint, countNotAbove)(JNIEnv* env, jclass, jlong v, jdoubleArray bounds, jlongArray countsOut) {
    Pin<jdouble> pb(env, bounds, JNI_ABORT); Pin<jlong> po(env, countsOut);
    if (!pb.p || !po.p || po.length() < pb.length()) return FMHIP_ERR_INVALID_ARGUMENT;
    return fmhip_count_not_above(v, pb.p, pb.length(), (int64_t*)po.p);
}
FMJ(jint, crossMoments)(JNIEnv* env, jclass, jlongArray x, jlongArray y, jdoubleArray sumsOut) {
    Pin<jlong> px(env, x, JNI_ABORT); Pin<jlong> py(env, y, JNI_ABORT); Pin<jdouble> po(env, sumsOut);
    if (!px.p || !po.p) return FMHIP_ERR_INVALID_ARGUMENT;
    const int64_t nx = px.length(), ny = py.p ? py.length() : 0;
    if ((int64_t)po.length() < nx * (nx + 1) / 2 + nx * ny) return FMHIP_ERR_INVALID_ARGUMENT;
    return fmhip_cross_moments((const fmhip_vec*)px.p, (int)nx, ny ? (const fmhip_vec*)py.p : nullptr, (int)ny, po.p);
}
FMJ(jint, crossMomentsWide)(JNIEnv* env, jclass, jlongArray x, jlongArray y, jdoubleArray sumsOut) {
    Pin<jlong> px(env, x, JNI_ABORT); Pin<jlong> py(env, y, JNI_ABORT); Pin<jdouble> po(env, sumsOut);
    if (!px.p || !po.p) return FMHIP_ERR_INVALID_ARGUMENT;
    const int64_t nx = px.length(), ny = py.p ? py.length() : 0;
    if ((int64_t)po.length() < nx * (nx + 1) / 2 + nx * ny) return FMHIP_ERR_INVALID_ARGUMENT;
    return fmhip_cross_moments_wide((const fmhip_vec*)px.p, (int)nx, ny ? (const fmhip_vec*)py.p : nullptr, (int)ny, po.p);
}
FMJ(jint, binnedCrossMoments)(JNIEnv* env, jclass, jlong key, jdoubleArray bounds, jlongArray x, jlongArray y, jlongArray countsOut, jdoubleArray sumsOut) {
    Pin<jdouble> pb(env, bounds, JNI_ABORT); Pin<jlong> px(env, x, JNI_ABORT); Pin<jlong> py(env, y, JNI_ABORT); Pin<jlong> pc(env, countsOut); Pin<jdouble> po(env, sumsOut);
    if (!px.p || !pc.p || !po.p) return FMHIP_ERR_INVALID_ARGUMENT;
    const int64_t nb = (pb.p ? pb.length() : 0) + 1, nx = px.length(), ny = py.p ? py.length() : 0;
    if ((int64_t)pc.length() < nb || (int64_t)po.length() < nb * (nx * (nx + 1) / 2 + nx * ny)) return FMHIP_ERR_INVALID_ARGUMENT;
    return fmhip_binned_cross_moments(key, pb.p, (int)nb, (const fmhip_vec*)px.p, (int)nx, ny ? (const fmhip_vec*)py.p : nullptr, (int)ny, (int64_t*)pc.p, po.p);
}
static bool binned_columns(const jfloat* flat, int64_t flatLength, int64_t n, int count, int onesMask, std::vector<const float*>& out) {
// ... 664 lines not shown
```

Baseline: 4242 billion.

## Record whole operation lists in one call instead of per-method calls

Adds fmhip_record_ops, which takes a topologically ordered list of operations over leaves and inserts all of the nodes into the pending fusion graph in one batch. It also adds fmhip_graph_ops to capture an existing graph as such a list. The LMM host driver records swaption product graphs via captured lists and replays them per simulation. The aim is to cut the per-operation host cost of calling, handle allocation and bookkeeping when building large fused graphs, at the price of extra validation code and a second path that has to match the per-call semantics.

```diff
diff --git a/finmath-lib-cuda-extensions_amd/__init__.py b/finmath-lib-cuda-extensions_amd/__init__.py
--- a/finmath-lib-cuda-extensions_amd/__init__.py
+++ b/finmath-lib-cuda-extensions_amd/__init__.py
@@ -254,6 +254,35 @@
     return out[:n.value]
 
 
+def record_ops(ops, leaves, wanted):
+    arr = (_native.Op * max(1, len(ops)))()
+    for i, (opcode, operands, scalar) in enumerate(ops):
+        arr[i].opcode, arr[i].n_in, arr[i].scalar = int(opcode), len(operands), float(scalar)
+        for k, r in enumerate(operands[:3]):
+            arr[i].operands[k] = int(r)
+    lv = (_C.c_int64 * max(1, len(leaves)))(*[v.handle for v in leaves])
+    w = (_C.c_int32 * max(1, len(wanted)))(*[int(x) for x in wanted])
+    out = (_C.c_int64 * max(1, len(wanted)))()
+    _native.check(lib().fmhip_record_ops(arr, len(ops), lv, len(leaves), w, len(wanted), out))
+    sizes = []
+    for opcode, operands, _ in ops:
+        r = operands[0]
+        sizes.append(sizes[r] if r >= 0 else leaves[-1 - r].n)
+    return [DeviceVector(out[k], sizes[wanted[k]]) for k in range(len(wanted))]
+
+
+def graph_ops(roots):
+    r = (_C.c_int64 * len(roots))(*[v.handle for v in roots])
+    n, nl = _C.c_int(0), _C.c_int(0)
+    _native.check(lib().fmhip_graph_ops(r, len(roots), None, 0, _C.byref(n), None, 0, _C.byref(nl), None))
+    arr = (_native.Op * max(1, n.value))()
+    lv = (_C.c_int64 * max(1, nl.value))()
+    entry = (_C.c_int32 * len(roots))()
+    _native.check(lib().fmhip_graph_ops(r, len(roots), arr, n.value, _C.byref(n), lv, nl.value, _C.byref(nl), entry))
+    ops = [(arr[i].opcode, [arr[i].operands[k] for k in range(arr[i].n_in)], arr[i].scalar) for i in range(n.value)]
+    return ops, [lv[i] for i in range(nl.value)], [entry[i] for i in range(len(roots))]
+
+
 def flush() -> None:
     _native.check(lib().fmhip_flush())
 
diff --git a/finmath-lib-cuda-extensions_amd/_native.py b/finmath-lib-cuda-extensions_amd/_native.py
--- a/finmath-lib-cuda-extensions_amd/_native.py
+++ b/finmath-lib-cuda-extensions_amd/_native.py
@@ -15,7 +15,7 @@
     "fmhip_vec_create_uninitialized", "fmhip_vec_retain", "fmhip_vec_release", "fmhip_vec_size", "fmhip_vec_give_up_values",
     "fmhip_vec_read_double", "fmhip_vec_read_float", "fmhip_vec_device_ptr",
     "fmhip_call_v1s0", "fmhip_call_v1s1", "fmhip_call_v2s0", "fmhip_call_v2s1", "fmhip_call_v3s0",
-    "fmhip_set_fusion", "fmhip_flush", "fmhip_fusion_hold", "fmhip_set_step_grouping", "fmhip_graph_clone", "fmhip_graph_scalars", "fmhip_set_math_mode",
+    "fmhip_set_fusion", "fmhip_flush", "fmhip_fusion_hold", "fmhip_set_step_grouping", "fmhip_graph_clone", "fmhip_graph_scalars", "fmhip_record_ops", "fmhip_graph_ops", "fmhip_set_math_mode",
     "fmhip_reduce_moments", "fmhip_reduce_moments_batch", "fmhip_reduce_moments_batch_device", "fmhip_reduce_moments_device",
     "fmhip_reduce_moments_batch_begin", "fmhip_reduce_moments_batch_end", "fmhip_reduce_moments_batch_devices", "fmhip_get_stream_of", "fmhip_expectation_collective",
     "fmhip_set_expectation_comm", "fmhip_expectation_world", "fmhip_expectation_combine",
@@ -57,6 +57,10 @@
 
 class ProgOp(C.Structure):
     _fields_ = [("opcode", C.c_int32), ("a", C.c_int32), ("b", C.c_int32), ("c", C.c_int32), ("scalar", C.c_double)]
+
+
+class Op(C.Structure):
+    _fields_ = [("opcode", C.c_int32), ("n_in", C.c_int32), ("operands", C.c_int32 * 3), ("reserved", C.c_int32), ("scalar", C.c_double)]
 
 
 class PoolStats(C.Structure):
@@ -157,6 +161,8 @@
         "fmhip_call_v3s0": [i32, vec, vec, vec, pv],
         "fmhip_set_fusion": [i32, C.POINTER(i32)], "fmhip_flush": [], "fmhip_fusion_hold": [i32, C.POINTER(i32)], "fmhip_set_step_grouping": [i32, C.POINTER(i32)], "fmhip_set_math_mode": [i32, C.POINTER(i32)],
         "fmhip_graph_clone": [pv, i32, i32, pv, pv, i32, C.POINTER(dbl), i32, pv], "fmhip_graph_scalars": [pv, i32, C.POINTER(dbl), i32, C.POINTER(i32)],
+        "fmhip_record_ops": [C.POINTER(Op), i32, pv, i32, C.POINTER(C.c_int32), i32, pv],
+        "fmhip_graph_ops": [pv, i32, C.POINTER(Op), i32, C.POINTER(i32), pv, i32, C.POINTER(i32), C.POINTER(C.c_int32)],
         "fmhip_reduce_moments": [vec, dbl, C.POINTER(Moments)], "fmhip_reduce_moments_batch": [pv, i32, C.POINTER(dbl), C.POINTER(Moments)], "fmhip_reduce_moments_batch_device": [pv, i32, C.POINTER(dbl), vp], "fmhip_reduce_moments_device": [vec, dbl, vp],
         "fmhip_reduce_moments_batch_devices": [pv, i32, C.POINTER(dbl), C.POINTER(vp), i32], "fmhip_get_stream_of": [i32, C.POINTER(vp)], "fmhip_expectation_collective": [C.POINTER(i32), C.c_char_p, i32],
         "fmhip_reduce_moments_batch_begin": [pv, i32, C.POINTER(dbl), pv], "fmhip_vec_give_up_values": [pv, i32], "fmhip_reduce_moments_batch_end": [i64, C.POINTER(Moments), i32],
diff --git a/finmath-lib-cuda-extensions_amd/csrc/abi.cpp b/finmath-lib-cuda-extensions_amd/csrc/abi.cpp
--- a/finmath-lib-cuda-extensions_amd/csrc/abi.cpp
+++ b/finmath-lib-cuda-extensions_amd/csrc/abi.cpp
@@ -480,6 +480,19 @@
         *n_scalars = Engine::get().graph_scalars(roots, n_roots, scalars_out, capacity);
     });
 }
+int fmhip_record_ops(const fmhip_op* ops, int n_ops, const fmhip_vec* leaves, int n_leaves, const int32_t* wanted, int n_wanted, fmhip_vec* out) {
+    FRONT(record_ops(ops, n_ops, leaves, n_leaves, wanted, n_wanted, out));
+    TE_LOCAL(leaves, n_leaves, L, fmhip_record_ops(ops, n_ops, L, n_leaves, wanted, n_wanted, out));
+    return guarded([&] { Engine::get().record_ops(ops, n_ops, leaves, n_leaves, wanted, n_wanted, out); });
+}
+int fmhip_graph_ops(const fmhip_vec* roots, int n_roots, fmhip_op* ops_out, int capacity, int* n_ops, fmhip_vec* leaves_out, int leaf_capacity, int* n_leaves, int32_t* root_entry_out) {
+    FRONT(unsupported("fmhip_graph_ops"));
+    return guarded([&] {
+        need(n_ops, "n_ops"); need(n_leaves, "n_leaves");
+        if (capacity < 0 || leaf_capacity < 0) throw Error(FMHIP_ERR_INVALID_ARGUMENT, "negative capacity");
+        Engine::get().graph_ops(roots, n_roots, ops_out, capacity, n_ops, leaves_out, leaf_capacity, n_leaves, root_entry_out);
+    });
+}
 int fmhip_set_math_mode(int mode, int* previous) {
     FRONT(set_int(3, mode, previous));
     TE_ALL(mine, fmhip_set_math_mode(mode, mine ? previous : nullptr));
diff --git a/finmath-lib-cuda-extensions_amd/csrc/runtime.cpp b/finmath-lib-cuda-extensions_amd/csrc/runtime.cpp
--- a/finmath-lib-cuda-extensions_amd/csrc/runtime.cpp
+++ b/finmath-lib-cuda-extensions_amd/csrc/runtime.cpp
@@ -193,7 +193,7 @@
     static const char* names[N_SLOTS] = { "call (record one method)", "release", "flush_all (total)", "  build_dag", "  run_dags (total)", "    launch (total)",
                                           "      kernel launch API", "      row table upload", "reduce / reduce_batch (total)",
                                           "  flush: roots + components", "  build_big (walk, schedule, sign)", "  run_big_group (total)",
-                                          "graph_clone (total)" };
+                                          "graph_clone (total)", "record_ops (a list of methods)" };
     std::fprintf(stderr, "[fmhip host profile]\n");
     for (int i = 0; i < N_SLOTS; ++i)
         std::fprintf(stderr, "  %-32s %10lld calls %9.3f s %9.2f us/call\n", names[i], count[i], seconds[i], count[i] ? seconds[i] / count[i] * 1e6 : 0.0);
@@ -1036,6 +1036,145 @@
     return count;
 }
 
+
+void Engine::graph_ops(const fmhip_vec* roots, int n_roots, fmhip_op* ops_out, int capacity, int* n_ops, fmhip_vec* leaves_out, int leaf_capacity, int* n_leaves,
+                       int32_t* root_entry_out) {
+    require_init();
+    std::vector<Node*> graph;
+    collect_pending(roots, n_roots, graph);
+    const uint64_t ep_graph = ++epoch_;
+    for (size_t i = 0; i < graph.size(); ++i) { graph[i]->mark = ep_graph; graph[i]->tmp_id = (int)i; }
+    const uint64_t ep_leaf = ++epoch_;
+    int leaves = 0;
+    auto leaf_index = [&](Node* l) {
+        if (l->mark != ep_leaf) { l->mark = ep_leaf; l->tmp_id = leaves; if (leaves_out && leaves < leaf_capacity) leaves_out[leaves] = l->id; ++leaves; }
+        return l->tmp_id;
+    };
+    for (size_t i = 0; i < graph.size(); ++i) {
+        const Node* nd = graph[i];
+        fmhip_op op{};
+        op.opcode = nd->opcode; op.n_in = nd->n_in; op.scalar = op_info(nd->opcode).scalar ? nd->scalar : 0.0;
+        for (int k = 0; k < nd->n_in; ++k) { Node* c = nd->in[k]; op.in[k] = c->mark == ep_graph ? c->tmp_id : -1 - leaf_index(c); }
+        if (ops_out && (int)i < capacity) ops_out[i] = op;
+    }
+    if (root_entry_out)
+        for (int r = 0; r < n_roots; ++r) { Node* root = node(roots[r]); root_entry_out[r] = root->mark == ep_graph ? root->tmp_id : -1 - leaf_index(root); }
+    if (n_ops) *n_ops = (int)graph.size();
+    if (n_leaves) *n_leaves = leaves;
+}
+
+void Engine::record_ops(const fmhip_op* ops, int n_ops, const fmhip_vec* leaves, int n_leaves, const int32_t* wanted, int n_wanted, fmhip_vec* out) {
+    HostTimer timer(HostProfile::RECORD_OPS);
+    require_init();
+    if (n_ops < 0 || n_leaves < 0 || n_wanted < 0 || (n_ops > 0 && !ops) || (n_leaves > 0 && !leaves) || (n_wanted > 0 && (!wanted || !out)))
+        throw Error(FMHIP_ERR_INVALID_ARGUMENT, "bad operation list");
+    std::vector<Node*> lf((size_t)n_leaves);
+    for (int i = 0; i < n_leaves; ++i) lf[(size_t)i] = node(leaves[i]);
+    std::vector<int64_t> size((size_t)n_ops);
+    std::vector<char> leaf_used((size_t)n_leaves, 0);
+    for (int i = 0; i < n_ops; ++i) {
+        const fmhip_op& op = ops[i];
+        const OpInfo inf = op_info(op.opcode);
+        if (inf.n_vec == 0) throw Error(FMHIP_ERR_INVALID_ARGUMENT, "entry " + std::to_string(i) + ": unknown opcode " + std::to_string(op.opcode));
+        if (inf.n_vec != op.n_in) throw Error(FMHIP_ERR_INVALID_ARGUMENT, "entry " + std::to_string(i) + ": opcode " + std::to_string(op.opcode) + " does not take " + std::to_string(op.n_in) + " operands");
+        for (int k = 0; k < op.n_in; ++k) {
+            const int32_t r = op.in[k];
+            int64_t n;
+            if (r >= 0) {
+                if (r >= i) throw Error(FMHIP_ERR_INVALID_ARGUMENT, "entry " + std::to_string(i) + " refers to entry " + std::to_string(r) + ", which is not before it");
+                n = size[(size_t)r];
+            } else {
+                const int64_t l = -1 - (int64_t)r;
+                if (l >= n_leaves) throw Error(FMHIP_ERR_INVALID_ARGUMENT, "entry " + std::to_string(i) + " refers to leaf " + std::to_string(l) + " of " + std::to_string(n_leaves));
+                const Node* leaf = lf[(size_t)l];
+                if (leaf->discarded && !leaf->buf) throw Error(FMHIP_ERR_INVALID_ARGUMENT, "the value of an operand does not exist: it was given up (fmhip_vec_give_up_values), or lost in a launch that failed");
+                leaf_used[(size_t)l] = 1;
+                n = leaf->n;
+            }
+            if (k == 0) size[(size_t)i] = n;
+            else if (n != size[(size_t)i]) throw Error(FMHIP_ERR_SIZE_MISMATCH, "operand sizes differ: " + std::to_string(size[(size_t)i]) + " vs " + std::to_string(n));
+        }
+    }
+    for (int w = 0; w < n_wanted; ++w)
+        if (wanted[w] < 0 || wanted[w] >= n_ops) throw Error(FMHIP_ERR_INVALID_ARGUMENT, "wanted result " + std::to_string(wanted[w]) + " is no entry of the list");
+
+    if (!(fusion && fusion_hold == 1)) {
+        std::vector<fmhip_vec> h((size_t)n_ops, 0);
+        int made = 0;
+        auto give_back = [&] { for (int i = made - 1; i >= 0; --i) { try { release(h[(size_t)i]); } catch (...) {} } };
+        try {
+            for (int i = 0; i < n_ops; ++i) {
+                const fmhip_op& op = ops[i];
+                fmhip_vec in[3] = { 0, 0, 0 };
+                for (int k = 0; k < op.n_in; ++k) in[k] = op.in[k] >= 0 ? h[(size_t)op.in[k]] : leaves[-1 - op.in[k]];
+                h[(size_t)i] = call(op.opcode, op.n_in, in, op.scalar, op_info(op.opcode).scalar);
+                made = i + 1;
+            }
+            for (int w = 0; w < n_wanted; ++w) node(h[(size_t)wanted[w]]);
+        } catch (...) { give_back(); throw; }
+        for (int w = 0; w < n_wanted; ++w) { node(h[(size_t)wanted[w]])->refs_ext++; out[w] = h[(size_t)wanted[w]]; }
+        give_back();
+        return;
+    }
+
+    if (!replicas_.empty())
+        for (int l = 0; l < n_leaves; ++l) if (leaf_used[(size_t)l] && !lf[(size_t)l]->buf && lf[(size_t)l]->rep_copy) if (ReplicaGroup* g = replica_of(lf[(size_t)l])) expand_replicas(g);
+    for (int l = 0; l < n_leaves; ++l) if (leaf_used[(size_t)l] && (lf[(size_t)l]->watch || lf[(size_t)l]->deferred)) demand(lf[(size_t)l]);
+    std::vector<char> alive((size_t)n_ops, 0);
+    for (int w = 0; w < n_wanted; ++w) alive[(size_t)wanted[w]] = 1;
+    for (int i = n_ops - 1; i >= 0; --i)
+        if (alive[(size_t)i]) for (int k = 0; k < ops[i].n_in; ++k) if (ops[i].in[k] >= 0) alive[(size_t)ops[i].in[k]] = 1;
+    std::vector<Node*> made((size_t)n_ops, nullptr);
+    try {
+        for (int i = 0; i < n_ops; ++i) {
+            if (!alive[(size_t)i]) continue;
+            Node* nd;
+            if (!node_pool_.empty()) { nd = node_pool_.back(); node_pool_.pop_back(); *nd = Node(); } else nd = new Node();
+            made[(size_t)i] = nd;
+        }
+    } catch (...) {
+        for (Node* nd : made) if (nd) node_pool_.push_back(nd);
+        throw;
+    }
+    const int64_t id_base = next_id_;
+    next_id_ += n_ops;
+    for (int i = 0; i < n_ops; ++i) {
+        Node* nd = made[(size_t)i];
+        if (!nd) continue;
+        const fmhip_op& op = ops[i];
+        nd->id = id_base + i; nd->n = size[(size_t)i];
+        nd->opcode = op.opcode; nd->n_in = op.n_in; nd->scalar = op.scalar;
+        int w = 1;
+        for (int k = 0; k < op.n_in; ++k) {
+            Node* in = op.in[k] >= 0 ? made[(size_t)op.in[k]] : lf[(size_t)(-1 - op.in[k])];
+            nd->in[k] = in; in->refs_int++; w += in->buf ? 0 : in->weight;
+        }
+        nd->weight = w;
+        pend_insert(nd);
+    }
+    ops_since_boundary_ += (size_t)n_ops;
+    int handed = 0;
+    try {
+        for (; handed < n_wanted; ++handed) {
+            Node* nd = made[(size_t)wanted[handed]];
+            if (++nd->refs_ext == 1) nodes_.put(nd->id, nd);
+            out[handed] = nd->id;
+        }
+    } catch (...) {
+        for (int w = 0; w < handed; ++w) { Node* nd = made[(size_t)wanted[w]]; if (--nd->refs_ext == 0) nodes_.erase(nd->id); }
+        for (int i = n_ops - 1; i >= 0; --i) {
+            Node* nd = made[(size_t)i];
+            if (!nd) continue;
+            nd->refs_ext = 0;
+            for (int k = 0; k < nd->n_in; ++k) nd->in[k]->refs_int--;
+            nd->n_in = 0;
+            pend_erase(nd);
+            node_pool_.push_back(nd);
+        }
+        throw;
+    }
+}
+
 template <class RootNode, class IdOf, class ScalarOf, class LeafTo>
 static void clone_nodes_impl(std::vector<Node*>& graph, uint64_t ep_graph, uint64_t ep_leaf, int n_copies, RootNode root_node, IdOf id_of, ScalarOf scalar_of, LeafTo leaf_to,
                              std::vector<Node*>& node_pool, std::vector<std::vector<Node*>>& copies, const std::function<void(Node*)>& pend_insert)
diff --git a/finmath-lib-cuda-extensions_amd/csrc/runtime.hpp b/finmath-lib-cuda-extensions_amd/csrc/runtime.hpp
--- a/finmath-lib-cuda-extensions_amd/csrc/runtime.hpp
+++ b/finmath-lib-cuda-extensions_amd/csrc/runtime.hpp
@@ -262,6 +262,8 @@
     void graph_clone(const fmhip_vec* roots, int n_roots, int n_copies, const fmhip_vec* leaf_from, const fmhip_vec* leaf_to, int n_map,
                      const double* scalars, int n_scalars, fmhip_vec* out);
     int graph_scalars(const fmhip_vec* roots, int n_roots, double* out, int capacity);
+    void record_ops(const fmhip_op* ops, int n_ops, const fmhip_vec* leaves, int n_leaves, const int32_t* wanted, int n_wanted, fmhip_vec* out);
+    void graph_ops(const fmhip_vec* roots, int n_roots, fmhip_op* ops_out, int capacity, int* n_ops, fmhip_vec* leaves_out, int leaf_capacity, int* n_leaves, int32_t* root_entry_out);
 
     struct RedLaunch { void* partials = nullptr; size_t partials_cap = 0; void* results = nullptr; size_t results_cap = 0; void* dev_moments = nullptr;
                        bool on_host = false; volatile uint64_t* poll_flag = nullptr; uint64_t done_value = 0; int slot = -1;
@@ -664,7 +666,7 @@
 void hip_check(hipError_t e, const char* what);
 
 struct HostProfile {
-    enum Slot { CALL, RELEASE, FLUSH, BUILD_DAG, RUN_DAGS, LAUNCH, LAUNCH_API, ROW_UPLOAD, REDUCE, FLUSH_COMPONENTS, BUILD_BIG, RUN_BIG, CLONE, N_SLOTS };
+    enum Slot { CALL, RELEASE, FLUSH, BUILD_DAG, RUN_DAGS, LAUNCH, LAUNCH_API, ROW_UPLOAD, REDUCE, FLUSH_COMPONENTS, BUILD_BIG, RUN_BIG, CLONE, RECORD_OPS, N_SLOTS };
     bool on = false;
     double seconds[N_SLOTS] = { 0 };
     long long count[N_SLOTS] = { 0 };
diff --git a/finmath-lib-cuda-extensions_amd/csrc/sharded.cpp b/finmath-lib-cuda-extensions_amd/csrc/sharded.cpp
--- a/finmath-lib-cuda-extensions_amd/csrc/sharded.cpp
+++ b/finmath-lib-cuda-extensions_amd/csrc/sharded.cpp
@@ -492,6 +492,43 @@
     });
 }
 
+int record_ops(const fmhip_op* ops, int n_ops, const fmhip_vec* leaves, int n_leaves, const int32_t* wanted, int n_wanted, fmhip_vec* out) {
+    return fronted([&](Shards& s) {
+        if (n_ops < 0 || n_leaves < 0 || n_wanted < 0 || (n_ops > 0 && !ops) || (n_leaves > 0 && !leaves) || (n_wanted > 0 && (!wanted || !out)))
+            throw Error(FMHIP_ERR_INVALID_ARGUMENT, "bad operation list");
+        std::vector<int64_t> leaf_n((size_t)n_leaves), size((size_t)n_ops);
+        for (int i = 0; i < n_leaves; ++i) leaf_n[(size_t)i] = s.vec(leaves[i]).n;
+        for (int i = 0; i < n_ops; ++i) {
+            const fmhip_op& op = ops[i];
+            const OpShape shape = op_shape(op.opcode);
+            if (shape.n_vec == 0) throw Error(FMHIP_ERR_INVALID_ARGUMENT, "entry " + std::to_string(i) + ": unknown opcode " + std::to_string(op.opcode));
+            if (shape.n_vec != op.n_in) throw Error(FMHIP_ERR_INVALID_ARGUMENT, "entry " + std::to_string(i) + ": opcode " + std::to_string(op.opcode) + " does not take " + std::to_string(op.n_in) + " operands");
+            for (int k = 0; k < op.n_in; ++k) {
+                const int32_t r = op.in[k];
+                if (r >= i) throw Error(FMHIP_ERR_INVALID_ARGUMENT, "entry " + std::to_string(i) + " refers to entry " + std::to_string(r) + ", which is not before it");
+                if (r < 0 && -1 - (int64_t)r >= n_leaves) throw Error(FMHIP_ERR_INVALID_ARGUMENT, "entry " + std::to_string(i) + " refers to a leaf that is not there");
+                const int64_t n = r >= 0 ? size[(size_t)r] : leaf_n[(size_t)(-1 - r)];
+                if (k == 0) size[(size_t)i] = n;
+                else if (n != size[(size_t)i]) throw Error(FMHIP_ERR_SIZE_MISMATCH, "operand sizes differ: " + std::to_string(size[(size_t)i]) + " vs " + std::to_string(n));
+            }
+        }
+        for (int w = 0; w < n_wanted; ++w)
+            if (wanted[w] < 0 || wanted[w] >= n_ops) throw Error(FMHIP_ERR_INVALID_ARGUMENT, "wanted result " + std::to_string(wanted[w]) + " is no entry of the list");
+        auto o = std::make_shared<std::vector<fmhip_op>>(ops, ops + n_ops);
+        auto lv = std::make_shared<std::vector<fmhip_vec>>(leaves, leaves + n_leaves);
+        auto wt = std::make_shared<std::vector<int32_t>>(wanted, wanted + n_wanted);
+        auto ids = std::make_shared<std::vector<fmhip_vec>>((size_t)n_wanted);
+        for (int w = 0; w < n_wanted; ++w) (*ids)[(size_t)w] = s.fresh(size[(size_t)wanted[w]]);
+        s.post([=](Worker& w) {
+            std::vector<fmhip_vec> local, got(ids->size(), 0);
+            for (fmhip_vec h : *lv) local.push_back(w.at(h));
+            if (w.ok(fmhip_record_ops(o->data(), (int)o->size(), local.data(), (int)local.size(), wt->data(), (int)wt->size(), got.data())))
+                for (size_t i = 0; i < got.size(); ++i) w.bind((*ids)[i], got[i]);
+        });
+        if (n_wanted > 0) std::memcpy(out, ids->data(), ids->size() * sizeof(fmhip_vec));
+    });
+}
+
 int graph_scalars(const fmhip_vec* roots, int n_roots, double* scalars_out, int capacity, int* n_scalars) {
     return fronted([&](Shards& s) {
         if (!n_scalars) throw Error(FMHIP_ERR_INVALID_ARGUMENT, "null count pointer");
diff --git a/finmath-lib-cuda-extensions_amd/csrc/sharded.hpp b/finmath-lib-cuda-extensions_amd/csrc/sharded.hpp
--- a/finmath-lib-cuda-extensions_amd/csrc/sharded.hpp
+++ b/finmath-lib-cuda-extensions_amd/csrc/sharded.hpp
@@ -32,6 +32,7 @@
 int flush();
 int graph_clone(const fmhip_vec* roots, int n_roots, int n_copies, const fmhip_vec* leaf_from, const fmhip_vec* leaf_to, int n_map, const double* scalars, int n_scalars, fmhip_vec* out);
 int graph_scalars(const fmhip_vec* roots, int n_roots, double* scalars_out, int capacity, int* n_scalars);
+int record_ops(const fmhip_op* ops, int n_ops, const fmhip_vec* leaves, int n_leaves, const int32_t* wanted, int n_wanted, fmhip_vec* out);
 int reduce_moments_batch(const fmhip_vec* vectors, int count, const double* shifts, fmhip_moments* out);
 int reduce_moments_batch_begin(const fmhip_vec* vectors, int count, const double* shifts, fmhip_ticket* ticket_out);
 int reduce_moments_batch_end(fmhip_ticket ticket, fmhip_moments* out, int count);
diff --git a/finmath-lib-cuda-extensions_amd/host/hip_backend.hpp b/finmath-lib-cuda-extensions_amd/host/hip_backend.hpp
--- a/finmath-lib-cuda-extensions_amd/host/hip_backend.hpp
+++ b/finmath-lib-cuda-extensions_amd/host/hip_backend.hpp
@@ -2,6 +2,7 @@
 #include <cstdlib>
 #include <cstring>
 #include <memory>
+#include <unordered_map>
 #include "lmm.hpp"
 
 namespace fmhost {
@@ -83,6 +84,77 @@
             return sc;
         };
     }
+    if (!(std::getenv("FMHIP_LMM_RECORD_OPS") && std::getenv("FMHIP_LMM_RECORD_OPS")[0] == '0')) {
+        auto handleOf = [](const RV& x) {
+            auto p = dynamic_cast<const RandomVariableHip*>(x.get());
+            if (!p || p->isDeterministic()) throw std::runtime_error("a list of operations over a value that is not a device vector");
+            return p->deviceVector().handle();
+        };
+        struct NativeList { std::vector<fmhip_op> ops; std::vector<int32_t> scalarOp, wanted; std::vector<size_t> rootSlot; };
+        be.captureOps = [handleOf](const std::vector<RV>& roots, const std::vector<RV>& leaves) -> std::shared_ptr<lmm::Backend::OpList> {
+            std::vector<fmhip_vec> r;
+            for (const RV& x : roots) { auto p = dynamic_cast<const RandomVariableHip*>(x.get()); if (!p || p->isDeterministic()) return nullptr; r.push_back(p->deviceVector().handle()); }
+            int nOps = 0, nLeaves = 0;
+            if (r.empty() || fmhip_graph_ops(r.data(), (int)r.size(), nullptr, 0, &nOps, nullptr, 0, &nLeaves, nullptr) != FMHIP_OK || nOps == 0) return nullptr;
+            auto native = std::make_shared<NativeList>();
+            native->ops.resize((size_t)nOps);
+            std::vector<fmhip_vec> graphLeaves((size_t)nLeaves);
+            std::vector<int32_t> entry(r.size());
+            check(fmhip_graph_ops(r.data(), (int)r.size(), native->ops.data(), nOps, &nOps, graphLeaves.data(), nLeaves, &nLeaves, entry.data()));
+            if ((size_t)nOps != native->ops.size() || (size_t)nLeaves != graphLeaves.size()) return nullptr;
+            std::vector<int32_t> position((size_t)nLeaves, -1);
+            std::unordered_map<fmhip_vec, int32_t> named;
+            for (size_t q = 0; q < leaves.size(); ++q) named.emplace(handleOf(leaves[q]), (int32_t)q);
+            for (size_t l = 0; l < graphLeaves.size(); ++l) {
+                const auto at = named.find(graphLeaves[l]);
+                if (at == named.end()) return nullptr;
+                position[l] = at->second;
+            }
+            auto list = std::make_shared<lmm::Backend::OpList>();
+            list->ops.resize((size_t)nOps);
+            for (int i = 0; i < nOps; ++i) {
+                fmhip_op& op = native->ops[(size_t)i];
+                lmm::Backend::OpList::Op& o = list->ops[(size_t)i];
+                o.opcode = op.opcode; o.nIn = op.n_in;
+                for (int k = 0; k < op.n_in; ++k) { if (op.in[k] < 0) op.in[k] = -1 - position[(size_t)(-1 - op.in[k])]; o.in[k] = op.in[k]; }
+                const bool carriesScalar = (op.opcode >= FMHIP_OP_CAP_S && op.opcode <= FMHIP_OP_POW_S) || (op.opcode >= FMHIP_OP_ACCRUE && op.opcode <= FMHIP_OP_ADDPRODUCT_VS);
+                if (carriesScalar) { native->scalarOp.push_back(i); list->scalars.push_back(op.scalar); }
+            }
+            for (size_t k = 0; k < r.size(); ++k) {
+                if (entry[k] < 0) return nullptr;
+                size_t slot = 0;
+                while (slot < native->wanted.size() && native->wanted[slot] != entry[k]) ++slot;
+                if (slot == native->wanted.size()) native->wanted.push_back(entry[k]);
+                native->rootSlot.push_back(slot);
+                list->rootEntry.push_back(entry[k]);
+                list->rootTime.push_back(roots[k]->getFiltrationTime());
+            }
+            list->numberOfLeaves = leaves.size();
+            list->native = native;
+            return list;
+        };
+        be.recordOps = [handleOf](const lmm::Backend::OpList& list, const std::vector<double>& scalars, const std::vector<RV>& leaves) {
+            NativeList& native = *static_cast<NativeList*>(list.native.get());
+            if (scalars.size() != native.scalarOp.size()) throw std::runtime_error("a list of operations: ragged scalar list");
+            for (size_t k = 0; k < scalars.size(); ++k) native.ops[(size_t)native.scalarOp[k]].scalar = scalars[k];
+            std::vector<fmhip_vec> lv, out(native.wanted.size(), 0);
+            lv.reserve(leaves.size());
+            for (const RV& x : leaves) lv.push_back(handleOf(x));
+            check(fmhip_record_ops(native.ops.data(), (int)native.ops.size(), lv.data(), (int)lv.size(), native.wanted.data(), (int)native.wanted.size(), out.data()));
+            const int64_t n = leaves.empty() ? 0 : leaves[0]->size();
+            std::vector<RV> unique(native.wanted.size()), roots;
+            std::vector<DeviceVector> owned;
+            owned.reserve(out.size());
+            for (fmhip_vec h : out) owned.emplace_back(h);
+            roots.reserve(native.rootSlot.size());
+            for (size_t k = 0; k < native.rootSlot.size(); ++k) {
+                RV& u = unique[native.rootSlot[k]];
+                if (!u) u = RandomVariableHip::of(list.rootTime[k], std::move(owned[native.rootSlot[k]]), n);
+                roots.push_back(u);
+            }
+            return roots;
+        };
+    }
     if (!(std::getenv("FMHIP_LMM_DISCARD") && std::getenv("FMHIP_LMM_DISCARD")[0] == '0'))
         be.valuesNotNeeded = [](const std::vector<RV>& v) {
             std::vector<fmhip_vec> h;
diff --git a/finmath-lib-cuda-extensions_amd/host/lmm.hpp b/finmath-lib-cuda-extensions_amd/host/lmm.hpp
--- a/finmath-lib-cuda-extensions_amd/host/lmm.hpp
+++ b/finmath-lib-cuda-extensions_amd/host/lmm.hpp
@@ -7,6 +7,8 @@
 #include <thread>
 #include <cstdlib>
 #include <functional>
+#include <map>
+#include <memory>
 #include <string>
 #include <vector>
 
@@ -145,10 +147,60 @@
     std::function<std::vector<std::vector<RV>>(const std::vector<RV>& roots, const std::vector<RV>& leafFrom, const std::vector<std::vector<RV>>& leafTo,
                                                const std::vector<std::vector<double>>* scalars)> clone;
     std::function<std::vector<double>(const std::vector<RV>& roots)> recordedScalars;
+    struct OpList {
+        struct Op { int opcode = 0, nIn = 0; int in[3] = { 0, 0, 0 }; };
+        std::vector<Op> ops;
+        std::vector<double> scalars;
+        std::vector<int> rootEntry;
+        std::vector<double> rootTime;
+        size_t numberOfLeaves = 0;
+        bool verified = false;
+        std::shared_ptr<void> native;
+    };
+    std::function<std::shared_ptr<OpList>(const std::vector<RV>& roots, const std::vector<RV>& leaves)> captureOps;
+    std::function<std::vector<RV>(const OpList& list, const std::vector<double>& scalars, const std::vector<RV>& leaves)> recordOps;
     int jacobianBatch = 1;
     bool keepAllStates = false;
     int threads = 1;
 };
+
+struct OpLists {
+    std::map<std::string, std::shared_ptr<Backend::OpList>> byKey;
+    long long recordings = 0, operations = 0;
+};
+inline OpLists& opLists() { static OpLists lists; return lists; }
+
+inline bool sameOperations(const Backend::OpList& a, const Backend::OpList& b) {
+    if (a.ops.size() != b.ops.size() || a.rootEntry != b.rootEntry || a.numberOfLeaves != b.numberOfLeaves) return false;
+    for (size_t i = 0; i < a.ops.size(); ++i) {
+        const Backend::OpList::Op& x = a.ops[i]; const Backend::OpList::Op& y = b.ops[i];
+        if (x.opcode != y.opcode || x.nIn != y.nIn) return false;
+        for (int k = 0; k < x.nIn; ++k) if (x.in[k] != y.in[k]) return false;
+    }
+    return true;
+}
+
+inline std::vector<RV> recordListed(const Backend& be, const std::string& key, const std::vector<double>* scalars, const std::vector<RV>& leaves) {
+    const auto it = opLists().byKey.find(key);
+    if (it == opLists().byKey.end() || !it->second) return {};
+    Backend::OpList& list = *it->second;
+    const std::vector<double>& sc = scalars ? *scalars : list.scalars;
+    if (sc.size() != list.scalars.size() || leaves.size() != list.numberOfLeaves) throw std::runtime_error("lmm: the list \"" + key + "\" was captured with other operands than it is recorded with");
+    std::vector<RV> roots = be.recordOps(list, sc, leaves);
+    if (!list.verified) {
+        const std::shared_ptr<Backend::OpList> again = be.captureOps(roots, leaves);
+        if (!again || !sameOperations(*again, list) || again->scalars != sc) throw std::runtime_error("lmm: the operations recorded as the list \"" + key + "\" differ from the hand recording");
+        list.verified = true;
+    }
+    ++opLists().recordings; opLists().operations += (long long)list.ops.size();
+    return roots;
+}
+inline void captureListed(const Backend& be, const std::string& key, const std::vector<RV>& roots, const std::vector<RV>& leaves, const std::vector<double>* expected) {
+    if (opLists().byKey.count(key)) return;
+    std::shared_ptr<Backend::OpList> list = be.captureOps(roots, leaves);
+    if (list && expected && list->scalars != *expected) throw std::runtime_error("lmm: the scalar list of \"" + key + "\" does not match the recording");
+    opLists().byKey[key] = list;
+}
 
 inline std::vector<Simulation> simulateMany(const Market& m, const std::vector<const VolatilityModel*>& vols, const Backend& be, int lastTimeIndex,
                                             const std::vector<char>* keep = nullptr) {
@@ -173,7 +225,57 @@
         if (keep && endAtKept) for (int s2 = i0 + 1; s2 < i1; ++s2) if ((*keep)[(size_t)s2]) { i1 = s2; break; }
         const bool cloning = K > 1 && S > 1 && keep && be.clone && i0 >= 2;
         const size_t Krec = cloning ? 1 : K;
+        const bool listed = S > 1 && keep && be.recordOps && be.captureOps && i0 >= 2 && (K == 1 || cloning);
+        std::string listKey;
+        if (listed) {
+            listKey = "euler " + std::to_string(i0) + " " + std::to_string(i1) + " of " + std::to_string(n) + " keep ";
+            for (int s2 = i0 + 1; s2 < i1; ++s2) listKey += (*keep)[(size_t)s2] ? '1' : '0';
+        }
+        auto rootsOf = [&](size_t k) {
+            std::vector<RV> roots;
+            for (int j = i0 + 1; j < n; ++j) roots.push_back(sims[k].libor[(size_t)i1][(size_t)j]);
+            for (int i = i0; i < i1; ++i) roots.push_back(sims[k].numeraire[(size_t)i + 1]);
+            for (int s2 = i0 + 1; s2 < i1; ++s2)
+                if (!keep || (*keep)[(size_t)s2]) for (int j = s2; j < n; ++j) roots.push_back(sims[k].libor[(size_t)s2][(size_t)j]);
+            return roots;
+        };
+        auto leavesOf = [&](size_t k) {
+            std::vector<RV> leaves;
+            for (int j = i0; j < n; ++j) leaves.push_back(sims[k].libor[(size_t)i0][(size_t)j]);
+            leaves.push_back(sims[k].numeraire[(size_t)i0]);
+            return leaves;
+        };
+        auto withIncrements = [&](std::vector<RV> leaves) { for (int i = i0; i < i1; ++i) leaves.push_back(be.brownianMotion->getBrownianIncrement(i, 0)); return leaves; };
+        auto takeRoots = [&](size_t k, const std::vector<RV>& got) {
+            auto& nxt = sims[k].libor[(size_t)i1];
+            nxt.resize((size_t)n);
+            for (int j = 0; j <= i0 && j < n; ++j) nxt[(size_t)j] = sims[k].libor[(size_t)i0][(size_t)j];
+            size_t r = 0;
+            for (int j = i0 + 1; j < n; ++j) nxt[(size_t)j] = got[r++];
+            for (int i = i0; i < i1; ++i) sims[k].numeraire[(size_t)i + 1] = got[r++];
+            for (int s2 = i0 + 1; s2 < i1; ++s2)
+                if (!keep || (*keep)[(size_t)s2]) { auto& mid = sims[k].libor[(size_t)s2]; mid.resize((size_t)n); for (int j = s2; j < n; ++j) mid[(size_t)j] = got[r++]; }
+        };
+        auto scalarsOf = [&](const VolatilityModel& vol) {
+            std::vector<double> sc;
+            for (int i = i0; i < i1; ++i) {
+                const double t = td.getTime(i), dt = td.getTimeStep(i);
+                for (int j = i + 1; j < n; ++j) {
+                    const double lambda = vol.volatility(t, td.getTime(j));
+                    sc.push_back(delta); sc.push_back(1.0); sc.push_back(lambda * delta); sc.push_back(lambda); sc.push_back(dt); sc.push_back(lambda);
+                }
+                sc.push_back(delta);
+            }
+            return sc;
+        };
         if (S > 1) be.hold(true);
+        bool recordedAsList = false;
+        if (listed) {
+            const std::vector<double> sc = scalarsOf(*vols[0]);
+            const std::vector<RV> got = recordListed(be, listKey, &sc, withIncrements(leavesOf(0)));
+            if (!got.empty()) { takeRoots(0, got); recordedAsList = true; }
+        }
+        if (!recordedAsList) {
         for (int i = i0; i < i1; ++i) {
             const double t = td.getTime(i), dt = td.getTimeStep(i);
             const RV dW = be.brownianMotion->getBrownianIncrement(i, 0);
@@ -204,48 +306,19 @@
                 sims[k].numeraire[(size_t)i + 1] = sims[k].numeraire[(size_t)i]->accrue(sims[k].libor[(size_t)i][(size_t)i], delta);
             for (size_t k = 0; k < Krec; ++k) factorSum[k] = nullptr;
         }
+        if (listed) { const std::vector<double> sc = scalarsOf(*vols[0]); captureListed(be, listKey, rootsOf(0), withIncrements(leavesOf(0)), &sc); }
+        }
         if (cloning) {
-            std::vector<RV> roots, leafFrom;
-            for (int j = i0 + 1; j < n; ++j) roots.push_back(sims[0].libor[(size_t)i1][(size_t)j]);
-            for (int i = i0; i < i1; ++i) roots.push_back(sims[0].numeraire[(size_t)i + 1]);
-            for (int s2 = i0 + 1; s2 < i1; ++s2)
-                if (!keep || (*keep)[(size_t)s2]) for (int j = s2; j < n; ++j) roots.push_back(sims[0].libor[(size_t)s2][(size_t)j]);
-            for (int j = i0; j < n; ++j) leafFrom.push_back(sims[0].libor[(size_t)i0][(size_t)j]);
-            leafFrom.push_back(sims[0].numeraire[(size_t)i0]);
-            auto scalarsOf = [&](const VolatilityModel& vol) {
-                std::vector<double> sc;
-                for (int i = i0; i < i1; ++i) {
-                    const double t = td.getTime(i), dt = td.getTimeStep(i);
-                    for (int j = i + 1; j < n; ++j) {
-                        const double lambda = vol.volatility(t, td.getTime(j));
-                        sc.push_back(delta); sc.push_back(1.0); sc.push_back(lambda * delta); sc.push_back(lambda); sc.push_back(dt); sc.push_back(lambda);
-                    }
-                    sc.push_back(delta);
-                }
-                return sc;
-            };
+            const std::vector<RV> roots = rootsOf(0), leafFrom = leavesOf(0);
             if (cloneChecks < 64 && be.recordedScalars) {
                 ++cloneChecks;
                 if (be.recordedScalars(roots) != scalarsOf(*vols[0])) throw std::runtime_error("lmm: the scalar list of the replicated Euler steps does not match the recording");
             }
             std::vector<std::vector<RV>> leafTo(K - 1);
             std::vector<std::vector<double>> scalars(K - 1);
-            for (size_t k = 1; k < K; ++k) {
-                for (int j = i0; j < n; ++j) leafTo[k - 1].push_back(sims[k].libor[(size_t)i0][(size_t)j]);
-                leafTo[k - 1].push_back(sims[k].numeraire[(size_t)i0]);
-                scalars[k - 1] = scalarsOf(*vols[k]);
-            }
+            for (size_t k = 1; k < K; ++k) { leafTo[k - 1] = leavesOf(k); scalars[k - 1] = scalarsOf(*vols[k]); }
             const std::vector<std::vector<RV>> copies = be.clone(roots, leafFrom, leafTo, &scalars);
-            for (size_t k = 1; k < K; ++k) {
-                auto& nxt = sims[k].libor[(size_t)i1];
-                nxt.resize((size_t)n);
-                for (int j = 0; j <= i0 && j < n; ++j) nxt[(size_t)j] = sims[k].libor[(size_t)i0][(size_t)j];
-                size_t r = 0;
-                for (int j = i0 + 1; j < n; ++j) nxt[(size_t)j] = copies[k - 1][r++];
-                for (int i = i0; i < i1; ++i) sims[k].numeraire[(size_t)i + 1] = copies[k - 1][r++];
-                for (int s2 = i0 + 1; s2 < i1; ++s2)
-                    if (!keep || (*keep)[(size_t)s2]) { auto& mid = sims[k].libor[(size_t)s2]; mid.resize((size_t)n); for (int j = s2; j < n; ++j) mid[(size_t)j] = copies[k - 1][r++]; }
-            }
+            for (size_t k = 1; k < K; ++k) takeRoots(k, copies[k - 1]);
         }
         if (keep)
             for (int i = i0; i < i1; ++i)
@@ -310,20 +383,29 @@
     const auto t1 = clk::now();
     const long long l1 = be.launches();
     std::vector<std::vector<RV>> values(K);
+    auto productLeaves = [&](size_t k) {
+        std::vector<RV> leaves;
+        for (int e = 0; e <= lastIndex; ++e) {
+            if (!keep[(size_t)e]) continue;
+            for (int j = e; j < m.numberOfLibors(); ++j) leaves.push_back(sims[k].libor[(size_t)e][(size_t)j]);
+            leaves.push_back(sims[k].numeraire[(size_t)e]);
+        }
+        return leaves;
+    };
+    const bool listed = be.recordOps && be.captureOps && (K == 1 || be.clone);
+    const std::string listKey = "payoffs of " + std::to_string(m.swaptions.size()) + " products";
+    auto recordProducts = [&](size_t k) {
+        if (listed) { values[k] = recordListed(be, listKey, nullptr, productLeaves(k)); if (!values[k].empty()) return; }
+        values[k].reserve(m.swaptions.size());
+        for (const Swaption& s : m.swaptions) values[k].push_back(swaptionValue(m, sims[k], s));
+        if (listed) captureListed(be, listKey, values[k], productLeaves(k), nullptr);
+    };
     if (K > 1 && be.clone) {
         be.hold(true);
-        values[0].reserve(m.swaptions.size());
-        for (const Swaption& s : m.swaptions) values[0].push_back(swaptionValue(m, sims[0], s));
-        std::vector<RV> leafFrom;
+        recordProducts(0);
+        const std::vector<RV> leafFrom = productLeaves(0);
         std::vector<std::vector<RV>> leafTo(K - 1);
-        for (int e = 0; e <= lastIndex; ++e) {
-            if (!keep[(size_t)e]) continue;
-            for (size_t k = 0; k < K; ++k) {
-                std::vector<RV>& dst = k == 0 ? leafFrom : leafTo[k - 1];
-                for (int j = e; j < m.numberOfLibors(); ++j) dst.push_back(sims[k].libor[(size_t)e][(size_t)j]);
-                dst.push_back(sims[k].numeraire[(size_t)e]);
-            }
-        }
+        for (size_t k = 1; k < K; ++k) leafTo[k - 1] = productLeaves(k);
         const std::vector<std::vector<RV>> copies = be.clone(values[0], leafFrom, leafTo, nullptr);
         for (size_t k = 1; k < K; ++k) values[k] = copies[k - 1];
         be.hold(false);
@@ -331,8 +413,7 @@
     } else
     for (size_t k = 0; k < K; ++k) {
         be.hold(true);
-        values[k].reserve(m.swaptions.size());
-        for (const Swaption& s : m.swaptions) values[k].push_back(swaptionValue(m, sims[k], s));
+        recordProducts(k);
         be.hold(false);
         if (!(be.averagesAsync && be.expectationsRunPending)) be.flush();
     }
diff --git a/finmath-lib-cuda-extensions_amd/host/lmm_hip_main.cpp b/finmath-lib-cuda-extensions_amd/host/lmm_hip_main.cpp
--- a/finmath-lib-cuda-extensions_amd/host/lmm_hip_main.cpp
+++ b/finmath-lib-cuda-extensions_amd/host/lmm_hip_main.cpp
@@ -43,6 +43,7 @@
         if (o.finmathLike) {
             be.flush = [] {}; be.hold = [](bool) {}; be.clone = nullptr; be.recordedScalars = nullptr; be.averagesAsync = nullptr; be.expectationsRunPending = false;
             be.averages = [](const std::vector<RV>& v) { std::vector<double> a; for (const RV& x : v) a.push_back(x->getAverage()); return a; };
+            be.captureOps = nullptr; be.recordOps = nullptr;
             be.jacobianBatch = 1; be.stepsPerLaunch = 1; be.chunk = 1 << 30; be.keepAllStates = true;
             if (o.threads > 1) {
                 if (!o.devices.empty() || o.world > 1) throw std::runtime_error("--threads: one device, one process");
@@ -50,7 +51,7 @@
                 be.threads = o.threads;
             }
         } else if (o.threads > 1) throw std::runtime_error("--threads belongs to --finmath-like (the native driver batches its Jacobian columns instead)");
-        if (o.releaseLagMs > 0.0 || o.releaseLagBytes > 0) ReleaseLag::instance().start(o.releaseLagMs, (size_t)o.releaseLagBytes);
+        if (o.releaseLagMs > 0.0 || o.releaseLagBytes > 0) { ReleaseLag::instance().start(o.releaseLagMs, (size_t)o.releaseLagBytes); be.captureOps = nullptr; be.recordOps = nullptr; }
         ncclComm_t comm = nullptr;
         std::vector<std::pair<double*, hipEvent_t>> sparePinned;
         fmhip_vec sums = 0;
@@ -197,7 +198,9 @@
                           (long long)es.interpreter_launches, (long long)es.algorithmic_bytes_written, (long long)es.values_deferred, (long long)es.values_deferred_now,
                           (long long)es.values_demanded, (long long)es.peak_bytes_reserved, (long long)es.late_releases_while_waiting, (long long)es.late_releases_at_once, (double)es.late_release_nanoseconds * 1e-9,
                           (long long)es.merged_launches, (long long)es.merged_chains, (long long)es.common_rows, (long long)es.rolled_launches);
-            return std::string(buf) + prof + lag + eb;
+            char lb2[128];
+            std::snprintf(lb2, sizeof lb2, ", \"recorded_as_lists\": {\"lists\": %lld, \"operations\": %lld}", lmm::opLists().recordings, lmm::opLists().operations);
+            return std::string(buf) + prof + lag + eb + lb2;
         };
         if (o.rank == 0) lmm::runAndReport(o, be, "hip", extra);
         else { lmm::Options quiet = o; quiet.verbose = false; lmm::runAndReport(quiet, be, "hip", extra); }
diff --git a/include/fmhip.h b/include/fmhip.h
--- a/include/fmhip.h
+++ b/include/fmhip.h
@@ -120,6 +120,17 @@
                       const fmhip_vec* leaf_from, const fmhip_vec* leaf_to, int n_map,
                       const double* scalars, int n_scalars, fmhip_vec* out);
 int fmhip_graph_scalars(const fmhip_vec* roots, int n_roots, double* scalars_out, int capacity, int* n_scalars);
+typedef struct fmhip_op {
+    int32_t opcode;
+    int32_t n_in;
+    int32_t in[3];
+    int32_t reserved;
+    double  scalar;
+} fmhip_op;
+int fmhip_record_ops(const fmhip_op* ops, int n_ops, const fmhip_vec* leaves, int n_leaves,
+                     const int32_t* wanted, int n_wanted, fmhip_vec* out);
+int fmhip_graph_ops(const fmhip_vec* roots, int n_roots, fmhip_op* ops_out, int capacity, int* n_ops,
+                    fmhip_vec* leaves_out, int leaf_capacity, int* n_leaves, int32_t* root_entry_out);
 
 #define FMHIP_MATH_EXACT 0
 #define FMHIP_MATH_FAST  1
diff --git a/java/net/finmath/hip/Native.java b/java/net/finmath/hip/Native.java
--- a/java/net/finmath/hip/Native.java
+++ b/java/net/finmath/hip/Native.java
@@ -43,6 +43,8 @@
 	static native int setStepGrouping(int steps, int[] previous);
 	static native int graphClone(long[] roots, int nCopies, long[] leafFrom, long[] leafTo, double[] scalarsOrNull, int nScalars, long[] out);
 	static native int graphScalars(long[] roots, double[] scalarsOutOrNull, int[] count);
+	static native int recordOps(int[] opcodes, int[] operandCounts, int[] operands, double[] scalars, long[] leaves, int[] wanted, long[] out);
+	static native int graphOps(long[] roots, int[] opcodes, int[] operandCounts, int[] operands, double[] scalars, long[] leavesOut, int[] rootEntriesOrNull, int[] counts2);
 	static native int setMathMode(int mode, int[] previous);
 
 	static native int reduceMoments(long vector, double shift, double[] moments4);
diff --git a/src/jni/fmhip_jni.cpp b/src/jni/fmhip_jni.cpp
--- a/src/jni/fmhip_jni.cpp
+++ b/src/jni/fmhip_jni.cpp
@@ -1,4 +1,5 @@
 #include <jni.h>
+#include <algorithm>
 #include <cstdint>
 #include <string>
 #include <vector>
@@ -127,6 +128,28 @@
     if (st == FMHIP_OK) set1(env, count, n);
     return st;
 }
+FMJ(jint, recordOps)(JNIEnv* env, jclass, jintArray opcodes, jintArray operandCounts, jintArray operands, jdoubleArray scalars, jlongArray leaves, jintArray wanted, jlongArray out) {
+    Pin<jint> po(env, opcodes, JNI_ABORT), pc(env, operandCounts, JNI_ABORT), pi(env, operands, JNI_ABORT), pw(env, wanted, JNI_ABORT); Pin<jdouble> ps(env, scalars, JNI_ABORT);
+    Pin<jlong> pl(env, leaves, JNI_ABORT), pout(env, out);
+    const int n = po.length();
+    if (pc.length() < n || ps.length() < n || (int64_t)pi.length() < (int64_t)3 * n || pout.length() < pw.length()) return FMHIP_ERR_INVALID_ARGUMENT;
+    std::vector<fmhip_op> ops((size_t)n);
+    for (int i = 0; i < n; ++i) { fmhip_op& o = ops[(size_t)i]; o.opcode = po.p[i]; o.n_in = pc.p[i]; for (int k = 0; k < 3; ++k) o.in[k] = pi.p[3 * i + k]; o.reserved = 0; o.scalar = ps.p[i]; }
+    return fmhip_record_ops(ops.data(), n, (const fmhip_vec*)pl.p, pl.length(), (const int32_t*)pw.p, pw.length(), (fmhip_vec*)pout.p);
+}
+FMJ(jint, graphOps)(JNIEnv* env, jclass, jlongArray roots, jintArray opcodes, jintArray operandCounts, jintArray operands, jdoubleArray scalars, jlongArray leaves, jintArray rootEntries, jintArray counts2) {
+    int n = 0, nl = 0, st;
+    {
+        Pin<jlong> pr(env, roots, JNI_ABORT), pl(env, leaves); Pin<jint> po(env, opcodes), pc(env, operandCounts), pi(env, operands), pe(env, rootEntries); Pin<jdouble> ps(env, scalars);
+        const int cap = std::min(std::min(po.length(), pc.length()), std::min(pi.length() / 3, ps.length()));
+        if (pe.p && pe.length() < pr.length()) return FMHIP_ERR_INVALID_ARGUMENT;
+        std::vector<fmhip_op> ops((size_t)cap);
+        st = fmhip_graph_ops((const fmhip_vec*)pr.p, pr.length(), ops.data(), cap, &n, (fmhip_vec*)pl.p, pl.length(), &nl, (int32_t*)pe.p);
+        for (int i = 0; st == FMHIP_OK && i < std::min(cap, n); ++i) { po.p[i] = ops[(size_t)i].opcode; pc.p[i] = ops[(size_t)i].n_in; for (int k = 0; k < 3; ++k) pi.p[3 * i + k] = ops[(size_t)i].in[k]; ps.p[i] = ops[(size_t)i].scalar; }
+    }
+    if (st == FMHIP_OK && counts2 && env->GetArrayLength(counts2) >= 2) { const jint both[2] = { n, nl }; env->SetIntArrayRegion(counts2, 0, 2, both); }
+    return st;
+}
 FMJ(jint, setMathMode)(JNIEnv* env, jclass, jint mode, jintArray previous) { int prev = 0; const int st = fmhip_set_math_mode(mode, &prev); if (st == FMHIP_OK) set1(env, previous, prev); return st; }
 
 FMJ(jint, reduceMoments)(JNIEnv* env, jclass, jlong v, jdouble shift, jdoubleArray moments4) {
```

Result: no change. 4249 billion (median of 2 runs) (+0.2%).
